# JuliaLinearAlgebra/IterativeSolvers.jl

Measured on AMD Instinct MI355X. Metric: cg_iters_per_sec, higher is better.
Workload: dtype f64; 1 GPU; cg! on 256^3 3D 7-point Laplacian (test/laplace_matrix.jl), fp64, hashed rhs, x0 = 0 (BASELINE.json configs[1]); n=16777216, nnz=117047296

## Files before the change

### include/mik_dev.h

```cpp
#include "mik.h"
#ifndef MIK_DEV_H
#define MIK_DEV_H
#ifdef __cplusplus
extern "C" {
#endif
enum {
    MIK_KNOB_LAYOUTS = 0,
    MIK_KNOB_CSR_KERNEL = 1,
    MIK_KNOB_SDIA_KERNEL = 2,
    MIK_KNOB_LONG_SEGMENT = 3,
    MIK_KNOB_UPLOAD = 4,
    MIK_KNOB_GS = 5,
    MIK_KNOB_TRANSPORT = 6,
    MIK_KNOB_NO_LOOKAHEAD = 7,
    MIK_KNOB_SOLVER_FORM = 8,
    MIK_KNOB_GS_TIMEOUT = 9,
    MIK_KNOB_CG_STEP = 10,
    MIK_KNOB_HOST_WAIT = 11,
    MIK_KNOB_MACHINE = 12,
    MIK_KNOB_COUNT = 13
};
int mik_set_tuning(int key, int value);
int mik_ctx_set_tuning(mik_ctx *ctx, int key, int value);
int mik_dev_gmres_form(const mik_gmres *it, int *single_launch, int *segments_per_workgroup, int *xcd_local_last, int *timeouts);
int mik_dev_dense_plan(const mik_dense *D, int adjoint, const void *x, const void *y, int *vec, int *streamed, int64_t *grid_x, int64_t *grid_y,
                       int64_t *chunks_or_batches, int64_t *segments);
int mik_dev_dense_block_plan(const mik_dense *D, int b, const void *X, int64_t ldx, const void *Y, int64_t ldy, int *vec, int *streamed,
                             int64_t *grid_x, int64_t *grid_y, int64_t *chunks, int *groups, int *last_width, int *vector_cols, int64_t *workspace_bytes);
int mik_dev_dense_block_min_width(mik_dense *D, int width);
int mik_dev_mgs_resident_shape(int *threads, int *register_rounds, int *lds_rounds);
int mik_dev_spmv_plan(const mik_csr *A, const void *x, int fuse_dot, int rb_begin, int rb_count, int skip_begin, int skip_end, char *kernel_name, int len,
                      int64_t *grid, int *launches, int *pre_longrows, int *post_rowdot);
int mik_dev_spmv_run(mik_ctx *ctx, const mik_csr *A, const void *x, void *y, int fuse_dot, void *seg_out, int rb_begin, int rb_count, int skip_begin,
                     int skip_end);
int mik_dev_exclusive_scan(mik_ctx *ctx, int *data, int64_t n);
int mik_dev_xwin_plan(int64_t n_blocks, const int *first_col, const int *last_col, const int *entries, int elem_size, int64_t n_cols,
                      int64_t total_entries, int *win_lo, int *span);
#ifdef __cplusplus
}
#endif
#endif
```

### iterativesolvers.jl_amd/_lib.py

```python
from __future__ import annotations

import ctypes as C
import os

import numpy as np

_HERE = os.path.dirname(os.path.abspath(__file__))
LIB_PATH = os.path.join(_HERE, "libmik.so")

MIK_OK = 0
MIK_F64, MIK_F32 = 0, 1
MIK_C64, MIK_C32 = 2, 3
MIK_SCALAR_REAL = 0x100
MIK_MGS, MIK_CGS, MIK_DGKS = 0, 1, 2
STATUS = {1: "invalid argument", 2: "HIP runtime error", 3: "dimension/dtype mismatch",
          4: "out of memory", 5: "not implemented", 6: "callback failed", 7: "norm outside the safely representable range",
          8: "singular"}


class MikError(RuntimeError):
    def __init__(self, code: int, where: str, detail: str = ""):
        self.code = code
        super().__init__(f"{where}: status {code} ({STATUS.get(code, '?')}) {detail}".rstrip())


_vp = C.c_void_p
_i64 = C.c_int64
_i64p = C.POINTER(C.c_int64)
_f64p = C.POINTER(C.c_double)
_ip = C.POINTER(C.c_int)

HALO_FN = C.CFUNCTYPE(C.c_int, C.c_void_p)
REDUCE_FN = C.CFUNCTYPE(C.c_int, C.c_void_p, C.c_int, C.c_int, C.c_void_p)


MUL_FN = C.CFUNCTYPE(C.c_int, C.c_void_p, C.c_void_p, C.c_void_p)
LDIV_FN = C.CFUNCTYPE(C.c_int, C.c_void_p, C.c_void_p, C.c_void_p)


class MikOperator(C.Structure):
    _fields_ = [("dtype", C.c_int), ("n", C.c_int64), ("csr", C.c_void_p), ("mul", MUL_FN), ("user", C.c_void_p)]


class MikPrecond(C.Structure):
    _fields_ = [("diag", C.c_void_p), ("ldiv", LDIV_FN), ("user", C.c_void_p)]


class MikDeviceInfo(C.Structure):
    _fields_ = [("device", C.c_int), ("compute_units", C.c_int), ("xcds", C.c_int), ("wavefront_size", C.c_int),
                ("lds_bytes_per_cu", C.c_int64), ("l2_bytes", C.c_int64), ("hbm_bytes", C.c_int64), ("arch", C.c_char * 64),
                ("planned_compute_units", C.c_int), ("planned_xcds", C.c_int), ("xcd_maps", C.c_int), ("resident_workgroup_cap", C.c_int),
                ("gs_single_launch_max_segments", C.c_int), ("gs_xcd_local_max_workgroups", C.c_int), ("sweep_grid_cap", C.c_int),
                ("mgs_resident_max_segments", C.c_int), ("reserved", C.c_int * 7)]


class MikPartition(C.Structure):
    _fields_ = [("rank", C.c_int), ("nranks", C.c_int), ("n_ext", C.c_int64), ("x_ext", C.c_void_p),
                ("send_idx", C.c_void_p), ("n_send", C.c_int64), ("send_buf", C.c_void_p),
                ("halo", HALO_FN), ("reduce", REDUCE_FN), ("user", C.c_void_p), ("link", C.c_void_p)]


class MikDensePlan(C.Structure):
    _fields_ = [("form", C.c_int), ("spin_limit", C.c_int)]


MIK_DENSE_AUTO, MIK_DENSE_PANEL, MIK_DENSE_CHAINED = 0, 1, 2


SIGNATURES = {
    "mik_abi_version": (C.c_int, []),
    "mik_device_count": (C.c_int, [_ip]),
    "mik_ctx_create": (C.c_int, [C.c_int, C.POINTER(_vp)]),
    "mik_ctx_destroy": (C.c_int, [_vp]),
    "mik_ctx_info": (C.c_int, [_vp, C.POINTER(MikDeviceInfo)]),
    "mik_dev_gmres_form": (C.c_int, [_vp, _ip, _ip, _ip, _ip]),
    "mik_dev_dense_plan": (C.c_int, [_vp, C.c_int, _vp, _vp, _ip, _ip, _i64p, _i64p, _i64p, _i64p]),
    "mik_dev_dense_block_plan": (C.c_int, [_vp, C.c_int, _vp, _i64, _vp, _i64, _ip, _ip, _i64p, _i64p, _i64p, _ip, _ip, _ip, _i64p]),
    "mik_dev_dense_block_min_width": (C.c_int, [_vp, C.c_int]),
    "mik_dev_mgs_resident_shape": (C.c_int, [_ip, _ip, _ip]),
    "mik_dev_spmv_plan": (C.c_int, [_vp, _vp, C.c_int, C.c_int, C.c_int, C.c_int, C.c_int, C.c_char_p, C.c_int, _i64p, _ip, _ip, _ip]),
    "mik_dev_spmv_run": (C.c_int, [_vp, _vp, _vp, _vp, C.c_int, _vp, C.c_int, C.c_int, C.c_int, C.c_int]),
    "mik_dev_exclusive_scan": (C.c_int, [_vp, _vp, _i64]),
    "mik_ctx_set_stream": (C.c_int, [_vp, _vp]),
    "mik_ctx_synchronize": (C.c_int, [_vp]),
    "mik_last_error": (C.c_char_p, [_vp]),
    "mik_reduce_shape": (C.c_int, [C.c_int, _ip, _ip]),
    "mik_spmv_dot_shape": (C.c_int, [_ip, _ip]),
    "mik_set_tuning": (C.c_int, [C.c_int, C.c_int]),
    "mik_ctx_set_tuning": (C.c_int, [_vp, C.c_int, C.c_int]),
    "mik_dev_xwin_plan": (C.c_int, [_i64, _ip, _ip, _ip, C.c_int, _i64, _i64, _ip, _ip]),
    "mik_spmv_long_row": (C.c_int, [_ip]),
    "mik_spmv_long_segment": (C.c_int, [_ip]),
    "mik_spmv_long_group": (C.c_int, [_ip]),
    "mik_malloc": (C.c_int, [_vp, C.c_size_t, C.POINTER(_vp)]),
    "mik_free": (C.c_int, [_vp, _vp]),
    "mik_memcpy_h2d": (C.c_int, [_vp, _vp, _vp, C.c_size_t]),
    "mik_memcpy_d2h": (C.c_int, [_vp, _vp, _vp, C.c_size_t]),
    "mik_copy": (C.c_int, [_vp, C.c_int, _i64, _vp, _vp]),
    "mik_fill": (C.c_int, [_vp, C.c_int, _i64, _vp, _vp]),
    "mik_csr_create": (C.c_int, [_vp, C.c_int, _i64, _i64, _i64, _i64p, _i64p, _vp, C.c_int, C.c_int,
                                 C.POINTER(_vp)]),
    "mik_csr_create_i32": (C.c_int, [_vp, C.c_int, _i64, _i64, _i64, C.POINTER(C.c_int32), C.POINTER(C.c_int32), _vp, C.c_int, C.c_int,
                                     C.POINTER(_vp)]),
    "mik_csr_destroy": (C.c_int, [_vp]),
    "mik_csr_layout": (C.c_int, [_vp, _ip]),
    "mik_csr_set_layout": (C.c_int, [_vp, C.c_int]),
    "mik_csr_stored_bytes": (C.c_int, [_vp, _i64p]),
    "mik_csr_compact": (C.c_int, [_vp]),
    "mik_spmv_kernel": (C.c_int, [_vp, C.c_char_p, C.c_int]),
    "mik_csr_info": (C.c_int, [_vp, _i64p, _i64p, _i64p, _ip]),
    "mik_spmv": (C.c_int, [_vp, _vp, _vp, _vp]),
    "mik_dot": (C.c_int, [_vp, C.c_int, _i64, _vp, _vp, _vp]),
    "mik_nrm2": (C.c_int, [_vp, C.c_int, _i64, _vp, _vp]),
    "mik_axpy": (C.c_int, [_vp, C.c_int, _i64, _vp, _vp, _vp]),
    "mik_xpby": (C.c_int, [_vp, C.c_int, _i64, _vp, _vp, _vp]),
    "mik_sub": (C.c_int, [_vp, C.c_int, _i64, _vp, _vp]),
    "mik_scal": (C.c_int, [_vp, C.c_int, _i64, _vp, _vp]),
    "mik_divide": (C.c_int, [_vp, C.c_int, _i64, _vp, _vp, _vp]),
    "mik_orthogonalize": (C.c_int, [_vp, C.c_int, _i64, C.c_int, _vp, _i64, _vp, _vp, _vp, C.c_int]),
    "mik_orthogonalize_vectors": (C.c_int, [_vp, C.c_int, _i64, C.c_int, C.POINTER(_vp), _vp, _vp, _vp]),
    "mik_gemv_n": (C.c_int, [_vp, C.c_int, _i64, C.c_int, _vp, _i64, _vp, _vp, _vp]),
    "mik_gemv_t": (C.c_int, [_vp, C.c_int, _i64, C.c_int, _vp, _i64, _vp, _vp]),
    "mik_lu_solve": (C.c_int, [C.c_int, _vp, _i64, C.c_int, _vp]),
    "mik_cg_create": (C.c_int, [_vp, _vp, _vp, _vp, _vp, _vp, _vp, _vp, C.c_double, C.c_double, _i64,
                                C.c_int, C.POINTER(_vp)]),
    "mik_cg_create_op": (C.c_int, [_vp, C.POINTER(MikOperator), C.POINTER(MikPrecond), _vp, _vp, _vp, _vp, _vp, C.c_double, C.c_double, _i64,
                                   C.c_int, C.POINTER(_vp)]),
    "mik_gmres_create_op": (C.c_int, [_vp, C.POINTER(MikOperator), C.POINTER(MikPrecond), C.POINTER(MikPrecond), _vp, _vp, C.c_double, C.c_double,
                                      C.c_int, _i64, C.c_int, C.c_int, C.POINTER(_vp)]),
    "mik_cg_destroy": (C.c_int, [_vp]),
    "mik_cg_fused_x": (C.c_int, [_vp, C.POINTER(C.c_int)]),
    "mik_cg_iterate": (C.c_int, [_vp, _i64, _f64p, _ip]),
    "mik_cg_iterate_many": (C.c_int, [_vp, _i64, _i64, _f64p, _i64p]),
    "mik_cg_state": (C.c_int, [_vp, _f64p, _f64p, _f64p, _i64p, _i64p, _ip]),
    "mik_gmres_create": (C.c_int, [_vp, _vp, _vp, _vp, _vp, _vp, C.c_double, C.c_double, C.c_int, _i64, C.c_int,
                                   C.c_int, C.POINTER(_vp)]),
    "mik_gmres_create_partitioned": (C.c_int, [_vp, _vp, _vp, _vp, _vp, _vp, C.c_double, C.c_double, C.c_int, _i64, C.c_int,
                                               C.c_int, C.POINTER(MikPartition), C.POINTER(_vp)]),
    "mik_gmres_destroy": (C.c_int, [_vp]),
    "mik_gmres_iterate": (C.c_int, [_vp, _i64, _f64p, _ip]),
    "mik_gmres_iterate_many": (C.c_int, [_vp, _i64, _i64, _f64p, _i64p]),
    "mik_gmres_state": (C.c_int, [_vp, _f64p, _f64p, _f64p, _ip, _i64p, _ip]),
    "mik_axpy_dot": (C.c_int, [_vp, C.c_int, _i64, _vp, _vp, _vp, _vp, _vp, C.c_int]),
    "mik_axpy2_nrm2": (C.c_int, [_vp, C.c_int, _i64, _vp, _vp, _vp, _vp, _vp, _vp, C.c_int]),
    "mik_cheb_direction": (C.c_int, [_vp, C.c_int, _i64, _vp, _vp, _vp, C.c_int, _vp]),
    "mik_minres_update": (C.c_int, [_vp, C.c_int, _i64, _vp, _vp, _vp, _vp, _vp, _vp, _vp, _vp, _vp, _vp, _vp, C.c_int]),
    "mik_gram": (C.c_int, [_vp, C.c_int, _i64, C.c_int, _vp, _i64, _vp]),
    "mik_bicgstab_mr_update": (C.c_int, [_vp, C.c_int, _i64, C.c_int, _vp, _i64, _vp, _i64, _vp, _vp, _vp]),
    "mik_bicgstab_create": (C.c_int, [_vp, _vp, C.c_int, _vp, _vp, _i64, _vp, _i64, _vp, _vp, C.POINTER(_vp)]),
    "mik_bicgstab_step": (C.c_int, [_vp, _vp]),
    "mik_bicgstab_destroy": (C.c_int, [_vp]),
    "mik_minres_create": (C.c_int, [_vp, _vp, _vp, _vp, _vp, _vp, _vp, _vp, _vp, C.c_double, C.c_int, C.POINTER(_vp)]),
    "mik_minres_step": (C.c_int, [_vp, _i64, _vp]),
    "mik_minres_proj_shape": (C.c_int, [_vp, _ip, _ip]),
    "mik_bicgstab_dot_shape": (C.c_int, [_vp, _ip, _ip]),
    "mik_minres_destroy": (C.c_int, [_vp]),
    "mik_xpby_nrm2": (C.c_int, [_vp, C.c_int, _i64, _vp, _vp, _vp, _vp]),
    "mik_lsqr_update": (C.c_int, [_vp, C.c_int, _i64, _vp, _vp, _vp, _vp, _vp, _vp, _vp]),
    "mik_lsmr_update": (C.c_int, [_vp, C.c_int, _i64, _vp, _vp, _vp, _vp, _vp, _vp, _vp, _vp]),
    "mik_axpy2_dot": (C.c_int, [_vp, C.c_int, _i64, _vp, _vp, _vp, _vp, _vp, _vp, _vp]),
    "mik_scal2": (C.c_int, [_vp, C.c_int, _i64, _vp, _vp, _vp, _vp]),
    "mik_qmr_update": (C.c_int, [_vp, C.c_int, _i64, _vp, _vp, _vp, _vp, _vp, _vp, _vp, _vp, _vp]),
    "mik_idrs_create": (C.c_int, [_vp, _vp, C.c_int, _vp, _vp, _vp, _i64, _vp, _i64, _vp, _i64, _vp, _vp, _vp, C.c_double, C.POINTER(_vp)]),
    "mik_idrs_step": (C.c_int, [_vp, C.c_int, _vp]),
    "mik_idrs_state": (C.c_int, [_vp, _vp, _vp, _vp]),
# ... 141 lines not shown
```

### iterativesolvers.jl_amd/csrc/mik_comm.hip

```cpp
#include <dlfcn.h>

#include <algorithm>
#include <new>

#include "mik_kernels.h"
#include "mik_iter.h"
#include "mik_mail.h"

namespace {
struct NcclId { char internal[128]; };
using nccl_comm_t = void *;
struct Rccl {
    void *h = nullptr;
    int (*GetUniqueId)(NcclId *) = nullptr;
    int (*CommInitRank)(nccl_comm_t *, int, NcclId, int) = nullptr;
    int (*CommDestroy)(nccl_comm_t) = nullptr;
    int (*Send)(const void *, size_t, int, int, nccl_comm_t, hipStream_t) = nullptr;
    int (*Recv)(void *, size_t, int, int, nccl_comm_t, hipStream_t) = nullptr;
    int (*AllGather)(const void *, void *, size_t, int, nccl_comm_t, hipStream_t) = nullptr;
    int (*GroupStart)() = nullptr;
    int (*GroupEnd)() = nullptr;
    const char *(*GetErrorString)(int) = nullptr;
    std::string err;
};
// ... 1108 lines not shown
        MIK_TRY(halo_begin(it, &pending));
    }
    if (pending && it->int_end > it->int_begin) {
        MIK_TRY(mik_cgd_phase(it, MIK_CGD_STEP_B_INTERIOR, iteration));
        MIK_TRY(halo_end(it, pending));
        return head_spmv_dot(it, true, iteration);
    }
    MIK_TRY(halo_end(it, pending));
    return head_spmv_dot(it, false, iteration);
}

static int cgd_enqueue_tail(mik_cgd *it, int64_t iteration)
{
    if (mail_fused(it)) {
        MIK_TRY(mik_cgd_phase(it, CGD_STEP_C_NOFIN, iteration));
        return it->base.dtype == MIK_F64 ? mail_fin_rr<double>(it, iteration) : mail_fin_rr<float>(it, iteration);
    }
    MIK_TRY(mik_cgd_phase(it, MIK_CGD_STEP_C, iteration));
    MIK_TRY(gather_scalar(it, it->rr_all, 1));
    return mik_cgd_phase(it, MIK_CGD_STEP_D, iteration);
}

struct CgdComm {
    mik_cgd *it;
    mik_cg &base() { return it->base; }
    int phase(int ph) { return mik_cgd_phase(it, ph, 0); }
    int halo_x()
    {
        bool pending = false;
        if (!it->initially_zero) MIK_TRY(halo_begin(it, &pending));
        return halo_end(it, pending);
    }
    int gather_rr_init() { return gather_scalar(it, it->rr_all, 2); }
    int head(int64_t iteration) { return cgd_enqueue_head(it, iteration); }
    int tail(int64_t iteration, int64_t) { return cgd_enqueue_tail(it, iteration); }
    int flush_x() { return phase(CGD_X_FLUSH); }
    int wait(CgMirror *m) { return cgd_wait_raw(it, m); }
    int clear_pending() { return it->base.fuse_x ? phase(CGD_CLEAR_PENDING) : MIK_OK; }
    int scaled_norm()
    {
        bool direct = false;
        MIK_TRY(phase(CGD_NORM_AMAX));
        MIK_TRY(gather_rr_init());
        MIK_TRY(cgd_norm_stage1_any(it, &direct));
        if (direct) return MIK_OK;
        MIK_TRY(gather_rr_init());
        return cgd_norm_stage2_any(it);
    }
    int close_frozen(int64_t it_next, int hist_index)
    {
        it->norm_fix_index = hist_index;
        it->norm_it_next = it_next;
        return phase(CGD_FIX_STEP);
    }
    int collect(const CgMirror &m, double *residual, double *tol, double *history, int64_t cap, int64_t *steps)
    {
        int done = 0;
        MIK_TRY(mailbox_check(it->comm, "row-partitioned cg"));
        return cgd_collect(it, m, residual, tol, &done, history, cap, steps);
    }
};

extern "C" int mik_cgd_init(mik_cgd *it, double *residual, double *tol)
{
    if (!it) return MIK_ERR_INVALID;
    MIK_TRY(cgd_require_transport(it, "mik_cgd_init"));
    CgdComm rk{it};
    MIK_TRY(cgd_init_ranks(rk, residual, tol));
    it->initialised = true;
    return MIK_OK;
}

extern "C" int mik_cgd_iterate_many(mik_cgd *it, int64_t iteration, int64_t max_steps, double *residuals, int64_t *steps_done)
{
    if (!it || !steps_done || iteration < 0) return MIK_ERR_INVALID;
    *steps_done = 0;
    MIK_TRY(cgd_require_transport(it, "mik_cgd_iterate_many"));
    if (!it->initialised) return mik_fail(it->base.ctx, MIK_ERR_INVALID, "mik_cgd_iterate_many: call mik_cgd_init first");
    mik_cg &bs = it->base;
    if (max_steps <= 0 || iteration >= bs.maxiter || bs.residual <= bs.tol) return MIK_OK;
    max_steps = std::min<int64_t>(std::min<int64_t>(max_steps, bs.maxiter - iteration), bs.hist_cap);
    const bool ahead_ok = bs.ctx->tuning[MIK_KNOB_NO_LOOKAHEAD] == 0 && iteration + max_steps < bs.maxiter;
    bs.fuse_x = (bs.ctx->tuning[MIK_KNOB_CG_STEP] & 1) == 0;
    CgdComm rk{it};
    return cg_run_batch(rk, iteration, max_steps, ahead_ok, residuals, steps_done);
}

namespace {
struct GroupEvents {
    std::vector<hipEvent_t> packed, halo, dot, rr;
    std::vector<hipStream_t> side;
};

struct GroupState {
    int P = 0;
    std::vector<mik_cgd *> its;
    GroupEvents ev;
    ~GroupState()
    {
        for (auto *v : {&ev.packed, &ev.halo, &ev.dot, &ev.rr})
            for (hipEvent_t e : *v) if (e) (void)hipEventDestroy(e);
        for (hipStream_t s : ev.side) if (s) (void)hipStreamDestroy(s);
    }
};

std::vector<GroupState *> g_groups;

GroupState *find_group(mik_cgd **its, int P)
{
    for (GroupState *g : g_groups)
        if (g->P == P && std::equal(g->its.begin(), g->its.end(), its)) return g;
    return nullptr;
}
}

static int group_check(mik_cgd **its, int P, const char *who)
{
    if (!its || P < 1) return MIK_ERR_INVALID;
    for (int p = 0; p < P; ++p) {
        if (!its[p]) return MIK_ERR_INVALID;
        if (its[p]->nranks != P || its[p]->rank != p) return mik_fail(its[p]->base.ctx, MIK_ERR_MISMATCH, "%s: handle %d is rank %d of %d", who, p, its[p]->rank, its[p]->nranks);
        if (its[p]->base.dtype != its[0]->base.dtype) return mik_fail(its[p]->base.ctx, MIK_ERR_MISMATCH, "%s: mixed dtypes", who);
    }
    return MIK_OK;
}

static inline hipError_t group_copy(void *dst, int dst_dev, const void *src, int src_dev, size_t bytes, hipStream_t s)
{
    return dst_dev == src_dev ? hipMemcpyAsync(dst, src, bytes, hipMemcpyDeviceToDevice, s) : hipMemcpyPeerAsync(dst, dst_dev, src, src_dev, bytes, s);
}

static int group_get(mik_cgd **its, int P, GroupState **out)
{
    GroupState *g = find_group(its, P);
    if (!g) {
        g = new (std::nothrow) GroupState();
        if (!g) return MIK_ERR_NOMEM;
        g->P = P;
        g->its.assign(its, its + P);
        for (auto *v : {&g->ev.packed, &g->ev.halo, &g->ev.dot, &g->ev.rr}) v->assign((size_t)P, nullptr);
        g->ev.side.assign((size_t)P, nullptr);
        for (int p = 0; p < P; ++p) {
            mik_ctx *ctx = its[p]->base.ctx;
            MIK_HIP(ctx, hipSetDevice(ctx->device));
            for (int q = 0; q < P; ++q)
                if (its[q]->base.ctx->device != ctx->device) {
                    (void)hipDeviceEnablePeerAccess(its[q]->base.ctx->device, 0);
                    (void)hipGetLastError();
                }
            for (auto *v : {&g->ev.packed, &g->ev.halo, &g->ev.dot, &g->ev.rr}) MIK_HIP(ctx, hipEventCreateWithFlags(&(*v)[p], hipEventDisableTiming));
            MIK_HIP(ctx, hipStreamCreateWithFlags(&g->ev.side[p], hipStreamNonBlocking));
        }
        g_groups.push_back(g);
    }
    *out = g;
    return MIK_OK;
}

void mik_cgd_group_forget(mik_cgd *it)
{
    for (size_t i = 0; i < g_groups.size();) {
        GroupState *g = g_groups[i];
        if (std::find(g->its.begin(), g->its.end(), it) != g->its.end()) {
            for (int p = 0; p < g->P; ++p) (void)hipStreamSynchronize(g->ev.side[p]);
            g_groups.erase(g_groups.begin() + (long)i);
            delete g;
// ... 131 lines not shown
    int wait(CgMirror *m)
    {
        ms.resize((size_t)g->P);
        for (int p = 0; p < g->P; ++p) {
            MIK_TRY(set_device(p));
            MIK_TRY(cgd_wait_raw(g->its[p], &ms[(size_t)p]));
            if (ms[(size_t)p].range != ms[0].range)
                return mik_fail(g->its[p]->base.ctx, MIK_ERR_MISMATCH, "row-partitioned cg: rank %d disagrees with rank 0 on the range of |r|^2", p);
        }
        *m = ms[0];
        return MIK_OK;
    }
    int clear_pending() { return MIK_OK; }
    int scaled_norm()
    {
        MIK_TRY(phase(CGD_NORM_AMAX));
        MIK_TRY(group_gather_scalar(g, 1));
        bool direct = false;
        for (int p = 0; p < g->P; ++p) {
            bool dp = false;
            MIK_TRY(set_device(p));
            MIK_TRY(cgd_norm_stage1_any(g->its[p], &dp));
            if (p == 0) direct = dp;
            else if (dp != direct) return mik_fail(g->its[p]->base.ctx, MIK_ERR_MISMATCH, "row-partitioned cg: rank %d disagrees with rank 0 on max |r|", p);
        }
        if (direct) return MIK_OK;
        MIK_TRY(group_gather_scalar(g, 1));
        for (int p = 0; p < g->P; ++p) {
            MIK_TRY(set_device(p));
            MIK_TRY(cgd_norm_stage2_any(g->its[p]));
        }
        return MIK_OK;
    }
    int close_frozen(int64_t it_next, int hist_index)
    {
        for (mik_cgd *it : g->its) { it->norm_fix_index = hist_index; it->norm_it_next = it_next; }
        return phase(CGD_FIX_STEP);
    }
    int collect(const CgMirror &, double *residual, double *tol, double *history, int64_t cap, int64_t *steps)
    {
        std::vector<double> h0((size_t)cap), hp((size_t)cap);
        for (int p = 0; p < g->P; ++p) {
            mik_cgd *it = g->its[p];
            double res = 0, tl = 0;
            int done = 0;
            int64_t st = 0;
            MIK_TRY(set_device(p));
            MIK_TRY(cgd_collect(it, ms[(size_t)p], &res, &tl, &done, p == 0 ? h0.data() : hp.data(), cap, &st));
            if (p == 0) { *steps = st; if (residual) *residual = res; if (tol) *tol = tl; }
            else if (st != *steps || !std::equal(h0.begin(), h0.begin() + st, hp.begin()) || res != base().residual || tl != base().tol)
                return mik_fail(it->base.ctx, MIK_ERR_MISMATCH, "row-partitioned cg (group): rank %d disagrees with rank 0 on the residuals", p);
        }
        if (history) std::copy(h0.begin(), h0.begin() + *steps, history);
        return MIK_OK;
    }
};

extern "C" int mik_cgd_group_init(mik_cgd **its, int P, double *residual, double *tol)
{
    MIK_TRY(group_check(its, P, "mik_cgd_group_init"));
    CgdGroup rk{};
    MIK_TRY(group_get(its, P, &rk.g));
    MIK_TRY(cgd_init_ranks(rk, residual, tol));
    for (int p = 0; p < P; ++p) its[p]->initialised = true;
    return MIK_OK;
}

extern "C" int mik_cgd_group_iterate_many(mik_cgd **its, int P, int64_t iteration, int64_t max_steps, double *residuals, int64_t *steps_done)
{
    MIK_TRY(group_check(its, P, "mik_cgd_group_iterate_many"));
    if (!steps_done || iteration < 0) return MIK_ERR_INVALID;
    *steps_done = 0;
    CgdGroup rk{};
    MIK_TRY(group_get(its, P, &rk.g));
    mik_cg &b0 = its[0]->base;
    for (int p = 0; p < P; ++p) if (!its[p]->initialised) return mik_fail(b0.ctx, MIK_ERR_INVALID, "mik_cgd_group_iterate_many: call mik_cgd_group_init first");
    if (max_steps <= 0 || iteration >= b0.maxiter || b0.residual <= b0.tol) return MIK_OK;
    max_steps = std::min<int64_t>(std::min<int64_t>(max_steps, b0.maxiter - iteration), b0.hist_cap);
    rk.split = rk.early = true;
    for (int p = 0; p < P; ++p) {
        rk.split = rk.split && its[p]->int_end > its[p]->int_begin;
        rk.early = rk.early && its[p]->n_early > 0;
        its[p]->base.fuse_x = (its[p]->base.ctx->tuning[MIK_KNOB_CG_STEP] & 1) == 0;
    }
    rk.early = rk.early && rk.split;
    return cg_run_batch(rk, iteration, max_steps, false, residuals, steps_done);
}
```

### iterativesolvers.jl_amd/csrc/mik_core.hip

```cpp
#include <algorithm>
#include <cmath>
#include <cstdarg>
#include <limits>
#include <new>

#include "mik_kernels.h"
#include "mik_spmv.h"
#include "mik_complex.h"
#include <algorithm>
#include <mutex>

#include "mik_sell.h"
#include "mik_jds.h"
#include <map>
#include <string>
#include <unordered_map>

thread_local std::string g_mik_create_error;
int g_mik_tuning[MIK_KNOB_COUNT] = {0};
static std::vector<mik_ctx *> g_mik_contexts;
static std::mutex g_mik_contexts_mu;

int mik_fail(mik_ctx *ctx, int code, const char *fmt, ...)
{
    char buf[512];
    va_list ap;
    va_start(ap, fmt);
    vsnprintf(buf, sizeof(buf), fmt, ap);
    va_end(ap);
    if (ctx) ctx->err = buf; else g_mik_create_error = buf;
    return code;
}

int mik_ensure_partials(mik_ctx *ctx, size_t bytes)
{
    if (bytes <= ctx->partials_bytes) return MIK_OK;
    size_t want = std::max(bytes, (size_t)1 << 20);
    if (ctx->partials) {
        MIK_HIP(ctx, hipStreamSynchronize(ctx->stream));
        MIK_HIP(ctx, hipFree(ctx->partials));
        ctx->partials = nullptr;
        ctx->partials_bytes = 0;
    }
    MIK_HIP(ctx, hipMalloc(&ctx->partials, want));
    ctx->partials_bytes = want;
    return MIK_OK;
}


extern "C" int mik_abi_version(void) { return MIK_ABI_VERSION; }

extern "C" int mik_device_count(int *count)
{
    if (!count) return MIK_ERR_INVALID;
    int c = 0;
    hipError_t e = hipGetDeviceCount(&c);
    if (e != hipSuccess) { *count = 0; return mik_fail(nullptr, MIK_ERR_HIP, "hipGetDeviceCount: %s", hipGetErrorString(e)); }
    *count = c;
    return MIK_OK;
}

extern "C" int mik_ctx_create(int device, mik_ctx **out)
{
    if (!out) return mik_fail(nullptr, MIK_ERR_INVALID, "mik_ctx_create: out is NULL");
    *out = nullptr;
    int count = 0;
    hipError_t e = hipGetDeviceCount(&count);
    if (e != hipSuccess || count == 0)
        return mik_fail(nullptr, MIK_ERR_HIP, "mik_ctx_create: no HIP device available (%s)", hipGetErrorString(e));
    if (device < 0 || device >= count)
        return mik_fail(nullptr, MIK_ERR_INVALID, "mik_ctx_create: device %d out of range [0, %d)", device, count);
    mik_ctx *ctx = new (std::nothrow) mik_ctx();
    if (!ctx) return mik_fail(nullptr, MIK_ERR_NOMEM, "mik_ctx_create: host allocation failed");
    ctx->device = device;
    auto bail = [&](hipError_t err, const char *what) {
        int rc = mik_fail(nullptr, MIK_ERR_HIP, "mik_ctx_create: %s: %s", what, hipGetErrorString(err));
        delete ctx;
        return rc;
    };
    if ((e = hipSetDevice(device)) != hipSuccess) return bail(e, "hipSetDevice");
    if ((e = hipStreamCreateWithFlags(&ctx->own_stream, hipStreamNonBlocking)) != hipSuccess) return bail(e, "hipStreamCreate");
    ctx->stream = ctx->own_stream;
    {
        int v = 0;
        if ((e = hipDeviceGetAttribute(&v, hipDeviceAttributeMultiprocessorCount, device)) != hipSuccess) return bail(e, "hipDeviceGetAttribute(MultiprocessorCount)");
        ctx->cu_count = v;
        v = 0;
        if (hipDeviceGetAttribute(&v, hipDeviceAttributeNumberOfXccs, device) != hipSuccess || v < 1) { (void)hipGetLastError(); v = 1; }
        ctx->xcd_count = v;
        v = 0;
        if (hipDeviceGetAttribute(&v, hipDeviceAttributeWarpSize, device) == hipSuccess) ctx->wave_size = v; else (void)hipGetLastError();
        v = 0;
        if (hipDeviceGetAttribute(&v, hipDeviceAttributeMaxSharedMemoryPerMultiprocessor, device) == hipSuccess) ctx->lds_per_cu = v; else (void)hipGetLastError();
        v = 0;
        if (hipDeviceGetAttribute(&v, hipDeviceAttributeL2CacheSize, device) == hipSuccess) ctx->l2_bytes = v; else (void)hipGetLastError();
        hipDeviceProp_t prop;
        if (hipGetDeviceProperties(&prop, device) == hipSuccess) {
            ctx->hbm_bytes = (int64_t)prop.totalGlobalMem;
            snprintf(ctx->arch, sizeof(ctx->arch), "%s", prop.gcnArchName);
        } else (void)hipGetLastError();
        if (ctx->wave_size != 0 && ctx->wave_size != 64) {
            int rc = mik_fail(nullptr, MIK_ERR_HIP, "mik_ctx_create: device %d runs %d-wide wavefronts; libmik's kernels are written for wave-64 (gfx950)", device, ctx->wave_size);
            delete ctx;
            return rc;
        }
    }
    if ((e = hipMalloc(&ctx->coef, mik_ctx::COEF_BYTES)) != hipSuccess) return bail(e, "hipMalloc");
    if ((e = hipHostMalloc(&ctx->coef_host, mik_ctx::COEF_BYTES, hipHostMallocDefault)) != hipSuccess) return bail(e, "hipHostMalloc");
    if ((e = hipEventCreateWithFlags(&ctx->wait_event, hipEventDisableTiming)) != hipSuccess) return bail(e, "hipEventCreate");
    if ((e = hipHostMalloc(&ctx->pub, mik_ctx::PUB_BYTES + 64, hipHostMallocMapped | hipHostMallocCoherent)) != hipSuccess) return bail(e, "hipHostMalloc");
    memset(ctx->pub, 0, mik_ctx::PUB_BYTES + 64);
    {
        std::lock_guard<std::mutex> lk(g_mik_contexts_mu);
        memcpy(ctx->tuning, g_mik_tuning, sizeof(ctx->tuning));
        g_mik_contexts.push_back(ctx);
    }
    *out = ctx;
    return MIK_OK;
}

extern "C" int mik_ctx_info(const mik_ctx *ctx, mik_device_info *out)
{
    if (!ctx || !out) return MIK_ERR_INVALID;
    memset(out, 0, sizeof(*out));
    out->device = ctx->device;
    out->compute_units = ctx->cu_count;
    out->xcds = ctx->xcd_count;
    out->wavefront_size = ctx->wave_size;
    out->lds_bytes_per_cu = ctx->lds_per_cu;
    out->l2_bytes = ctx->l2_bytes;
    out->hbm_bytes = ctx->hbm_bytes;
    snprintf(out->arch, sizeof(out->arch), "%s", ctx->arch);
    out->planned_compute_units = mik_cus(ctx);
    out->planned_xcds = mik_xcds(ctx);
    out->xcd_maps = mik_xcd_maps(ctx) ? 1 : 0;
    out->resident_workgroup_cap = mik_resident_cap(ctx);
    out->gs_single_launch_max_segments = 8 * mik_resident_cap(ctx);
    out->gs_xcd_local_max_workgroups = mik_xcd_maps(ctx) ? 4 * (mik_cus(ctx) / mik_xcds(ctx)) : 0;
    out->sweep_grid_cap = mik_max_grid(ctx);
    out->mgs_resident_max_segments = ctx->lds_per_cu >= 160 * 1024 ? mik_mgs_resident_max_s() * mik_resident_cap(ctx) : 0;
    return MIK_OK;
}

extern "C" int mik_ctx_destroy(mik_ctx *ctx)
{
    if (!ctx) return MIK_OK;
    {
        std::lock_guard<std::mutex> lk(g_mik_contexts_mu);
        g_mik_contexts.erase(std::remove(g_mik_contexts.begin(), g_mik_contexts.end(), ctx), g_mik_contexts.end());
    }
    (void)hipSetDevice(ctx->device);
    (void)hipStreamSynchronize(ctx->stream);
    {
        std::vector<std::pair<void *, int (*)(void *)>> owned;
        owned.swap(ctx->owned);
        for (auto &h : owned) (void)h.second(h.first);
    }
    if (ctx->partials) (void)hipFree(ctx->partials);
    if (ctx->coef) (void)hipFree(ctx->coef);
    if (ctx->coef_host) (void)hipHostFree(ctx->coef_host);
    if (ctx->pub) (void)hipHostFree(ctx->pub);
    if (ctx->wait_event) (void)hipEventDestroy(ctx->wait_event);
    if (ctx->own_stream) (void)hipStreamDestroy(ctx->own_stream);
    delete ctx;
    return MIK_OK;
}

extern "C" int mik_ctx_set_stream(mik_ctx *ctx, void *hip_stream)
{
    if (!ctx) return MIK_ERR_INVALID;
    MIK_HIP(ctx, hipStreamSynchronize(ctx->stream));
    ctx->stream = hip_stream ? (hipStream_t)hip_stream : ctx->own_stream;
    return MIK_OK;
}

extern "C" int mik_ctx_synchronize(mik_ctx *ctx)
{
    if (!ctx) return MIK_ERR_INVALID;
    MIK_HIP(ctx, mik_wait(ctx));
    return MIK_OK;
}

extern "C" const char *mik_last_error(mik_ctx *ctx) { return ctx ? ctx->err.c_str() : g_mik_create_error.c_str(); }
// ... 1025 lines not shown
    return A->sdia_buf_ok && A->sdia_cls >= 1 && (A->n_rows & 1) == 0 && A->ctx->tuning[MIK_KNOB_SDIA_KERNEL] == 0;
}

static inline bool spmv_pair_range(int rb0, int nb, int nb_all) { return (rb0 & 1) == 0 && ((nb & 1) == 0 || rb0 + nb == nb_all); }

extern "C" int mik_csr_layout(const mik_csr *A, int *layout)
{
    if (!A || !layout) return MIK_ERR_INVALID;
    *layout = spmv_kernel_choice(A);
    return MIK_OK;
}

extern "C" int mik_csr_set_layout(mik_csr *A, int layout)
{
    if (!A) return MIK_ERR_INVALID;
    if (layout != 0 && layout != -1) return mik_fail(A->ctx, MIK_ERR_NOTIMPL, "mik_csr_set_layout: only 0 (CSR arrays) and -1 (automatic) can be requested");
    if (layout == 0 && !A->col) return mik_fail(A->ctx, MIK_ERR_NOTIMPL, "mik_csr_set_layout: the CSR arrays were released (mik_csr_compact)");
    A->force_layout = layout;
    return MIK_OK;
}

extern "C" int mik_csr_stored_bytes(const mik_csr *A, int64_t *bytes)
{
    if (!A || !bytes) return MIK_ERR_INVALID;
    const int64_t es = (int64_t)mik_dtype_size(A->dtype);
    const int64_t nb = (A->n_rows + MIK_BLOCK - 1) / MIK_BLOCK;
    if (mik_is_complex(A->dtype)) { *bytes = mik_c_stored_bytes(A); return MIK_OK; }
    switch (spmv_kernel_choice(A)) {
    case LAYOUT_SDIAC: *bytes = A->n_rows + nb * (spmv_sdiab_usable(A) ? 64 : 4) + (int64_t)A->sdia_npat * (80 + 8 * es); break;
    case LAYOUT_SDIAW: *bytes = A->n_rows * 4 + nb * 4 + (nb + 1) / 2 * 64 + (int64_t)A->sdiaw_npat * A->sdiaw_pat_bytes; break;
    case LAYOUT_SDIA: *bytes = A->sdia_entries * es + A->n_rows + nb * 36; break;
    case LAYOUT_JDS: *bytes = A->jds_groups * (16 / es) * (es + 4) + A->n_rows * 2 + ((A->n_rows + 63) / 64 + 1) * 4 +
                              (A->n_long ? (A->nnz - A->jds_short_nnz) * (es + 4) + 12LL * A->n_long + 4LL * A->n_seg + 16LL * A->n_cut : 0); break;
    case LAYOUT_CSR: *bytes = A->nnz * (es + 4) + (A->n_rows + 1) * 4 + (A->n_long ? A->n_rows + 12LL * A->n_long + 4LL * A->n_seg + 16LL * A->n_cut : 0) +
                              ((A->xwin_lo && !spmv_csr_rowgather(A)) ? nb * 4 : 0) + ((A->rperm && !spmv_csr_rowgather(A)) ? A->n_rows : 0); break;
    }
    return MIK_OK;
}

extern "C" int mik_csr_info(const mik_csr *A, int64_t *n_rows, int64_t *n_cols, int64_t *nnz, int *dtype)
{
    if (!A) return MIK_ERR_INVALID;
    if (n_rows) *n_rows = A->n_rows;
    if (n_cols) *n_cols = A->n_cols;
    if (nnz) *nnz = A->nnz;
    if (dtype) *dtype = A->dtype;
    return MIK_OK;
}

extern "C" int mik_csr_compact(mik_csr *A)
{
    if (!A) return MIK_ERR_INVALID;
    if (!A->col) return MIK_OK;
    if (!(A->sdia_pats || A->sdia_val || A->sdiaw_pats || A->jds_val) || A->n_long)
        return mik_fail(A->ctx, MIK_ERR_NOTIMPL, "mik_csr_compact: this operator runs on its CSR arrays");
    if (A->ctx) { (void)hipSetDevice(A->ctx->device); (void)hipStreamSynchronize(A->ctx->stream); }
    (void)hipFree(A->rowptr); (void)hipFree(A->col); (void)hipFree(A->val);
    A->rowptr = nullptr; A->col = nullptr; A->val = nullptr;
    return MIK_OK;
}

enum SpmvKernel { SPMV_ROWGATHER, SPMV_ROWBLOCK, SPMV_JDS, SPMV_SDIA, SPMV_SDIAC, SPMV_SDIAB, SPMV_SDIAB2, SPMV_SDIAW, SPMV_SDIAW2 };

constexpr int SPMV_NO_SKIP = 0x7fffffff;

struct SpmvPlan {
    int rc = MIK_OK;
    const char *refusal = nullptr;
    bool empty = false;
    SpmvKernel kernel = SPMV_ROWGATHER;
    bool can_split = false;
    bool skips = false;
    bool epilogue = false;
    bool pre_longrows = false, post_rowdot = false;
    int grid = 0;
    size_t lds = 0, pre_lds = 0;
    bool fd = false;
    int nb_all = 0, nlb = 0;
    int rb0 = 0, nb = 0, map_mode = 0;
    int skip_at = SPMV_NO_SKIP, skip_len = 0;
    int pb0 = 0, np = 0, pmode = 0, ps = -1, pfull = 0;
    int sshift = -1, nfull = 0, cls = 0;
    bool merge = false, nt_rb = false, xwin = false, rp = false;
    bool long_win = false;
    int lw_launch = 0;
};

static SpmvPlan spmv_refusal(SpmvPlan p, int rc, const char *text) { p.rc = rc; p.refusal = text; return p; }
static inline bool spmv_ep_armed(const mik_ctx *ctx) { return ctx->spmv_ep_w || ctx->spmv_ep_c || ctx->spmv_ep_z; }

static SpmvPlan spmv_plan(const mik_csr *A, size_t es, bool x_aligned, bool fuse_dot, int rb_begin, int rb_count, int skip_at, int skip_len, bool ep_armed)
{
    SpmvPlan p;
    const int *knob = A->ctx->tuning;
    const int n = (int)A->n_rows, nb_all = (int)mik_spmv_nwg(n), nlong = A->n_long;
    const bool whole = rb_count < 0 || (rb_begin == 0 && rb_count == nb_all);
    const int rb0 = whole ? 0 : rb_begin, nb = whole ? nb_all : rb_count;
    switch (spmv_kernel_choice(A)) {
    case LAYOUT_SDIAC:
        p.kernel = !spmv_sdiab_usable(A) ? SPMV_SDIAC : (sdiab2_applies(A) && skip_len == 0 && spmv_pair_range(rb0, nb, nb_all)) ? SPMV_SDIAB2 : SPMV_SDIAB;
        break;
    case LAYOUT_SDIAW:
        p.kernel = ((n & 1) == 0 && (uint64_t)A->n_cols * es < 0x7FFFFFF0ull && knob[MIK_KNOB_SDIA_KERNEL] != 3 && spmv_pair_range(rb0, nb, nb_all)) ? SPMV_SDIAW2 : SPMV_SDIAW;
        break;
    case LAYOUT_SDIA: p.kernel = SPMV_SDIA; break;
    case LAYOUT_JDS: p.kernel = SPMV_JDS; break;
    case LAYOUT_CSR: p.kernel = spmv_csr_rowgather(A) ? SPMV_ROWGATHER : SPMV_ROWBLOCK; break;
    }
    const bool row_per_thread = p.kernel == SPMV_ROWGATHER || p.kernel == SPMV_ROWBLOCK || p.kernel == SPMV_JDS;
    p.can_split = p.kernel != SPMV_ROWBLOCK && !(row_per_thread && nlong);
    p.skips = p.kernel == SPMV_SDIAB || p.kernel == SPMV_SDIAB2;
    p.epilogue = whole && fuse_dot && knob[MIK_KNOB_SOLVER_FORM] != 2 && (p.kernel == SPMV_SDIAB2 || (row_per_thread && nlong == 0));
    if (n == 0) { p.empty = true; return p; }
    if (!whole && !p.can_split) return spmv_refusal(p, MIK_ERR_NOTIMPL, "SpMV over a row-block range is not available for this operator layout");
    if (!whole && (rb_begin < 0 || rb_begin + rb_count > nb_all)) return spmv_refusal(p, MIK_ERR_INVALID, "SpMV row-block range out of bounds");
    if (!whole && rb_count == 0) { p.empty = true; return p; }
    if (ep_armed && !p.epilogue)
        return spmv_refusal(p, MIK_ERR_NOTIMPL, "SpMV: the y = A x + c w / dot(z, y) epilogue is not available for this operator's kernel");

    p.map_mode = A->strip;
    if (!whole && p.map_mode >= 8 && (rb0 % p.map_mode != 0 || nb % p.map_mode != 0)) p.map_mode = 0;
    if (skip_len > 0) p.map_mode = 0;
    p.nb_all = nb_all; p.rb0 = rb0; p.nb = nb; p.skip_at = skip_at; p.skip_len = skip_len;
    p.pb0 = rb0 / 2; p.np = (nb + 1) / 2;
    p.fd = fuse_dot;
    p.grid = nb;
    p.nlb = (nlong + 3) / 4;
    p.long_win = A->long_win && spmv_windows_live(A) && x_aligned;
    p.pre_lds = p.long_win ? es * (size_t)A->long_lw : 0;
    switch (p.kernel) {
    case SPMV_SDIAB: case SPMV_SDIAB2:
        if (p.map_mode >= 8) {
            const int S = p.map_mode >> 3;
            if ((S & (S - 1)) == 0) { p.sshift = 0; while ((1 << p.sshift) < S) ++p.sshift; p.nfull = nb / p.map_mode * p.map_mode; }
        }
        p.cls = knob[MIK_KNOB_SDIA_KERNEL] == 2 ? 0 : A->sdia_cls;
        if (p.kernel == SPMV_SDIAB2) {
            p.grid = (p.np + 7) / 8 * 8;
            p.ps = p.sshift >= 1 ? p.sshift - 1 : -1;
            p.pfull = p.sshift >= 1 ? p.nfull / 2 : 0;
            break;
        }
        [[fallthrough]];
    case SPMV_SDIAC: p.grid = ((nb + MIK_SDIAC_G - 1) / MIK_SDIAC_G + 7) / 8 * 8; break;
    case SPMV_SDIAW2:
        p.grid = p.np;
        p.pmode = p.map_mode >= 16 ? (p.map_mode / 2 + 7) / 8 * 8 : 0;
        break;
    case SPMV_SDIAW: case SPMV_SDIA: break;
    case SPMV_JDS:
        p.fd = fuse_dot && nlong == 0;
        p.merge = nlong > 0;
        p.post_rowdot = fuse_dot && !p.fd;
        p.grid = nb + (p.merge ? p.nlb : 0);
        break;
    case SPMV_ROWGATHER:
        p.pre_longrows = nlong > 0;
        break;
    case SPMV_ROWBLOCK: {
        p.merge = nlong > 0 && !fuse_dot;
        p.pre_longrows = nlong > 0 && !p.merge;
        p.nt_rb = !A->xwin_lo;
        p.grid = nb + (p.merge ? p.nlb : 0);
        p.xwin = A->xwin_lo && spmv_windows_live(A) && x_aligned;
        const size_t rb_tile = (size_t)MIK_SPMV_TILE * (8 / es);
        p.lds = es * (rb_tile + 12 + (p.xwin ? (size_t)A->xwin_span : 0));
        const int lw = (int)std::min<size_t>((size_t)A->long_lw, p.lds / 1024 * (1024 / es));
        p.lw_launch = (p.merge && p.long_win && A->long_spread) ? -lw : lw;
        p.rp = A->rperm && spmv_windows_live(A);
        break;
    }
    }
    return p;
}

static const char *spmv_kernel_name(const SpmvPlan &p)
{
    switch (p.kernel) {
    case SPMV_ROWGATHER: return "k_spmv_rowgather";
    case SPMV_ROWBLOCK: return p.xwin ? "k_spmv_rowblock+xwin" : "k_spmv_rowblock";
    case SPMV_JDS: return "k_spmv_jds";
    case SPMV_SDIA: return "k_spmv_sdia";
    case SPMV_SDIAC: return "k_spmv_sdiac";
    case SPMV_SDIAB: return "k_spmv_sdiab";
    case SPMV_SDIAB2: return "k_spmv_sdiab2";
    case SPMV_SDIAW: return "k_spmv_sdiaw";
    case SPMV_SDIAW2: return "k_spmv_sdiaw2";
    }
    return "";
}

static SpmvPlan spmv_plan_whole(const mik_csr *A, bool fuse_dot)
{
    return spmv_plan(A, mik_dtype_size(A->dtype), true, fuse_dot, 0, -1, SPMV_NO_SKIP, 0, false);
}

bool mik_spmv_has_epilogue(const mik_csr *A) { return A && spmv_plan_whole(A, true).epilogue; }
bool mik_spmv_can_split(const mik_csr *A) { return spmv_plan_whole(A, false).can_split; }
bool mik_spmv_is_light(const mik_csr *A) { return A && (spmv_kernel_choice(A) == LAYOUT_SDIAC || spmv_kernel_choice(A) == LAYOUT_SDIAW); }

extern "C" int mik_spmv_kernel(const mik_csr *A, char *name, int len)
{
    if (!A || !name || len <= 0) return MIK_ERR_INVALID;
    if (mik_is_complex(A->dtype)) { snprintf(name, (size_t)len, "%s", mik_c_spmv_kernel_name(A)); return MIK_OK; }
    snprintf(name, (size_t)len, "%s", spmv_kernel_name(spmv_plan_whole(A, false)));
    return MIK_OK;
}

static int spmv_plan_outside(const mik_csr *A, size_t es, bool x_aligned, bool fuse_dot, int skip_begin, int skip_end, bool ep_armed, SpmvPlan out[2])
{
    const int nb_all = (int)mik_spmv_nwg(A->n_rows), rest = skip_begin + (nb_all - skip_end);
    if (skip_begin < 0 || skip_end < skip_begin || skip_end > nb_all) { out[0] = spmv_refusal(SpmvPlan{}, MIK_ERR_INVALID, "SpMV: bad interior range"); return 1; }
    out[0] = spmv_plan(A, es, x_aligned, fuse_dot, 0, rest, skip_begin, skip_end - skip_begin, ep_armed);
    if (out[0].skips && rest > 0) return 1;
    out[0] = spmv_plan(A, es, x_aligned, fuse_dot, 0, skip_begin, SPMV_NO_SKIP, 0, ep_armed);
    out[1] = spmv_plan(A, es, x_aligned, fuse_dot, skip_end, nb_all - skip_end, SPMV_NO_SKIP, 0, ep_armed);
    return 2;
}

extern "C" int mik_dev_spmv_plan(const mik_csr *A, const void *x, int fuse_dot, int rb_begin, int rb_count, int skip_begin, int skip_end, char *kernel_name,
                                 int len, int64_t *grid, int *launches, int *pre_longrows, int *post_rowdot)
{
    if (!A || (kernel_name && len <= 0)) return MIK_ERR_INVALID;
    MIK_REFUSE_COMPLEX(A->ctx, A, "mik_dev_spmv_plan");
    const bool armed = spmv_ep_armed(A->ctx);
    SpmvPlan p[2];
    int np = 1;
    if (skip_begin < 0) p[0] = spmv_plan(A, mik_dtype_size(A->dtype), mik_aligned16(x), fuse_dot != 0, rb_begin, rb_count, SPMV_NO_SKIP, 0, armed);
    else np = spmv_plan_outside(A, mik_dtype_size(A->dtype), mik_aligned16(x), fuse_dot != 0, skip_begin, skip_end, armed, p);
    int total = 0;
    const SpmvPlan *first = nullptr;
    for (int i = 0; i < np; ++i) {
        if (p[i].rc != MIK_OK) return mik_fail(A->ctx, p[i].rc, "%s", p[i].refusal);
        if (p[i].empty) continue;
        total += (int)p[i].pre_longrows + 1 + (int)p[i].post_rowdot;
        if (!first) first = &p[i];
    }
    if (kernel_name) snprintf(kernel_name, (size_t)len, "%s", spmv_kernel_name(first ? *first : p[0]));
    if (grid) *grid = first ? first->grid : 0;
    if (launches) *launches = total;
    if (pre_longrows) *pre_longrows = first && first->pre_longrows;
    if (post_rowdot) *post_rowdot = first && first->post_rowdot;
    return MIK_OK;
}

struct SdiaCls { int c; };
template <typename F> static inline void with_consts(F &&f) { f(); }
template <typename F, typename... R> static inline void with_consts(F &&f, bool b, R... rest);
template <typename F, typename... R> static inline void with_consts(F &&f, SdiaCls s, R... rest);
template <typename C, typename F, typename... R> static inline void with_const(F &f, R... rest)
{
    with_consts([&](auto... c) { f(C{}, c...); }, rest...);
}
template <typename F, typename... R> static inline void with_consts(F &&f, bool b, R... rest)
{
    if (b) with_const<std::true_type>(f, rest...);
    else with_const<std::false_type>(f, rest...);
}
template <typename F, typename... R> static inline void with_consts(F &&f, SdiaCls s, R... rest)
{
    switch (s.c) {
    case 1: with_const<std::integral_constant<int, 1>>(f, rest...); break;
    case 2: with_const<std::integral_constant<int, 2>>(f, rest...); break;
    case 3: with_const<std::integral_constant<int, 3>>(f, rest...); break;
    default: with_const<std::integral_constant<int, 0>>(f, rest...); break;
    }
}

template <typename T> struct SpmvIO {
    mik_ctx *ctx;
    const mik_csr *A;
    const T *x;
    T *y, *seg_out;
    const int *done;
    const T *ep_w() const { return (const T *)ctx->spmv_ep_w; }
    const T *ep_c() const { return (const T *)ctx->spmv_ep_c; }
    const T *ep_z() const { return (const T *)ctx->spmv_ep_z; }
};

static LongTab spmv_long_tab(const mik_csr *A)
{
    LongTab lt{};
    if (const int nlong = A->n_long) {
        int *tb = A->long_rows;
        lt.rows = tb; lt.starts = tb + nlong; lt.lens = tb + 2 * nlong;
        lt.seg_row = tb + 3 * nlong;
        lt.cut_row = lt.seg_row + A->n_seg; lt.cut_first = lt.cut_row + A->n_cut; lt.cut_nseg = lt.cut_first + A->n_cut;
        lt.tickets = (unsigned *)(tb + 3 * nlong + A->n_seg + 3 * A->n_cut);
        lt.seg_sum = A->seg_sum; lt.nlong = nlong;
    }
    return lt;
}

template <typename T> static void spmv_go_sdiab(const SpmvPlan &p, const SpmvIO<T> &io)
{
    const mik_csr *A = io.A;
    with_consts([&](auto fd, auto cls) {
        constexpr int C = decltype(cls)::value;
        hipLaunchKernelGGL((k_spmv_sdiab<T, decltype(fd)::value, true, MIK_SDIAC_G, mik_sdiab_cls_ns(C), mik_sdiab_cls_cq(C)>), dim3(p.grid), dim3(MIK_BLOCK), 0,
                           io.ctx->stream, (int)A->n_rows, (int)A->n_cols, A->sdia_koff, p.rb0, p.nb, p.nfull, p.sshift, p.skip_at, p.skip_len,
                           (const SdiaSliceRec *)A->sdia_recs, (const SdiaPattern<T> *)A->sdia_pats, A->sdia_mask, io.x, io.y, io.seg_out, io.done);
    }, p.fd, SdiaCls{p.cls});
}

template <typename T> static void spmv_go_sdiab2(const SpmvPlan &p, const SpmvIO<T> &io)
{
    const mik_csr *A = io.A;
    with_consts([&](auto fd, auto cls) {
        constexpr int C = decltype(cls)::value;
        if constexpr (C >= 1)
            hipLaunchKernelGGL((k_spmv_sdiab2<T, decltype(fd)::value, true, mik_sdiab_cls_ns(C), mik_sdiab_cls_cq(C)>), dim3(p.grid), dim3(MIK_BLOCK), 0,
                               io.ctx->stream, (int)A->n_rows, (int)A->n_cols, A->sdia_koff, p.pb0, p.np, p.pfull, p.ps, p.nb_all,
                               (const SdiaSliceRec *)A->sdia_recs, (const SdiaPattern<T> *)A->sdia_pats, A->sdia_mask, io.x, io.y, io.seg_out, io.done,
                               io.ep_w(), io.ep_c(), io.ep_z());
    }, p.fd, SdiaCls{p.cls});
}

template <typename T> static void spmv_go_sdiac(const SpmvPlan &p, const SpmvIO<T> &io)
{
    const mik_csr *A = io.A;
    with_consts([&](auto fd) {
        hipLaunchKernelGGL((k_spmv_sdiac<T, decltype(fd)::value, true, MIK_SDIAC_G>), dim3(p.grid), dim3(MIK_BLOCK), 0, io.ctx->stream, (int)A->n_rows,
                           (int)A->n_cols, p.rb0, p.nb, p.map_mode, A->sdia_pat_id, (const SdiaPattern<T> *)A->sdia_pats, A->sdia_mask, io.x, io.y,
                           io.seg_out, io.done);
    }, p.fd);
}

template <typename T> static void spmv_go_sdiaw(const SpmvPlan &p, const SpmvIO<T> &io)
{
    const mik_csr *A = io.A;
    with_consts([&](auto fd) {
        if (p.kernel == SPMV_SDIAW2)
            hipLaunchKernelGGL((k_spmv_sdiaw2<T, decltype(fd)::value, true>), dim3(p.grid), dim3(MIK_BLOCK), 0, io.ctx->stream, (int)A->n_rows, (int)A->n_cols,
                               A->sdiaw_koff, p.pb0, p.np, p.pmode, p.nb_all, A->sdiaw_pat_id, (const SdiawPattern<T> *)A->sdiaw_pats, A->sdiaw_mask,
                               (const uint4 *)A->sdiaw_uz, io.x, io.y, io.seg_out, io.done);
        else
            hipLaunchKernelGGL((k_spmv_sdiaw<T, decltype(fd)::value, true>), dim3(p.grid), dim3(MIK_BLOCK), 0, io.ctx->stream, (int)A->n_rows, A->sdiaw_koff,
                               p.rb0, p.nb, p.map_mode, A->sdiaw_pat_id, (const SdiawPattern<T> *)A->sdiaw_pats, A->sdiaw_mask, io.x, io.y, io.seg_out,
                               io.done);
    }, p.fd);
}

template <typename T> static void spmv_go_sdia(const SpmvPlan &p, const SpmvIO<T> &io)
{
    const mik_csr *A = io.A;
    with_consts([&](auto fd) {
        hipLaunchKernelGGL((k_spmv_sdia<T, decltype(fd)::value, true>), dim3(p.grid), dim3(MIK_BLOCK), 0, io.ctx->stream, (int)A->n_rows, (int)A->n_cols, p.rb0,
                           p.nb, p.map_mode, A->sdia_ptr, A->sdia_off, A->sdia_tri, A->sdia_mask, (const T *)A->sdia_val, io.x, io.y, io.seg_out, io.done);
    }, p.fd);
}

template <typename T> static void spmv_go_jds(const SpmvPlan &p, const SpmvIO<T> &io)
{
    const mik_csr *A = io.A;
    using IV = typename WideVec<T>::idx;
    using VV = typename WideVec<T>::val;
    with_consts([&](auto fd, auto mg) {
        if constexpr (!(decltype(fd)::value && decltype(mg)::value))
            hipLaunchKernelGGL((k_spmv_jds<T, decltype(fd)::value, true, decltype(mg)::value>), dim3(p.grid), dim3(MIK_BLOCK), 0, io.ctx->stream, (int)A->n_rows,
                               p.rb0, A->jds_ptr, A->jds_len, (const IV *)A->jds_col, (const VV *)A->jds_val, io.x, io.y, io.seg_out, io.done, p.nlb,
                               spmv_long_tab(A), A->col, (const T *)A->val, io.ep_w(), io.ep_c(), io.ep_z());
    }, p.fd, p.merge);
}

template <typename T> static void spmv_go_rowgather(const SpmvPlan &p, const SpmvIO<T> &io)
{
    const mik_csr *A = io.A;
    with_consts([&](auto fd) {
        hipLaunchKernelGGL((k_spmv_rowgather<T, decltype(fd)::value, true>), dim3(p.grid), dim3(MIK_BLOCK), 0, io.ctx->stream, (int)A->n_rows, p.rb0, p.nb,
                           p.map_mode, A->rowptr, A->col, (const T *)A->val, io.x, io.y, io.seg_out, io.done, A->is_long, io.ep_w(), io.ep_c(), io.ep_z());
    }, p.fd);
}

template <typename T> static void spmv_go_rowblock(const SpmvPlan &p, const SpmvIO<T> &io)
{
    const mik_csr *A = io.A;
    with_consts([&](auto fd, auto mg, auto nt, auto xw, auto rp) {
        if constexpr (!(decltype(fd)::value && decltype(mg)::value))
            hipLaunchKernelGGL((k_spmv_rowblock<T, decltype(fd)::value, decltype(nt)::value, true, decltype(mg)::value, decltype(xw)::value, decltype(rp)::value>),
                               dim3(p.grid), dim3(MIK_BLOCK), p.lds, io.ctx->stream, (int)A->n_rows, p.nb, p.map_mode, A->rowptr, A->col, (const T *)A->val,
                               io.x, io.y, io.seg_out, io.done, A->is_long, p.nlb, spmv_long_tab(A), (const int *)A->xwin_lo, A->xwin_span,
                               (const unsigned char *)A->rperm, (p.merge && p.long_win) ? (const int *)A->long_win : (const int *)nullptr, p.lw_launch,
                               io.ep_w(), io.ep_c(), io.ep_z());
    }, p.fd, p.merge, p.nt_rb, p.xwin, p.rp);
}

template <typename T> static int spmv_run(const SpmvPlan &p, const SpmvIO<T> &io)
{
    mik_ctx *ctx = io.ctx;
    const mik_csr *A = io.A;
    if (p.rc != MIK_OK) return mik_fail(ctx, p.rc, "%s", p.refusal);
    if (p.empty) return MIK_OK;
    if (p.pre_longrows) {
        hipLaunchKernelGGL((k_spmv_longrows<T>), dim3(p.nlb), dim3(MIK_BLOCK), p.pre_lds, ctx->stream, spmv_long_tab(A), A->col, (const T *)A->val, io.x, io.y,
                           io.done, p.long_win ? (const int *)A->long_win : (const int *)nullptr, A->long_lw);
        MIK_LAUNCH_CHECK(ctx);
    }
    switch (p.kernel) {
    case SPMV_ROWGATHER: spmv_go_rowgather<T>(p, io); break;
    case SPMV_ROWBLOCK: spmv_go_rowblock<T>(p, io); break;
    case SPMV_JDS: spmv_go_jds<T>(p, io); break;
    case SPMV_SDIA: spmv_go_sdia<T>(p, io); break;
    case SPMV_SDIAC: spmv_go_sdiac<T>(p, io); break;
    case SPMV_SDIAB: spmv_go_sdiab<T>(p, io); break;
    case SPMV_SDIAB2: spmv_go_sdiab2<T>(p, io); break;
    case SPMV_SDIAW: case SPMV_SDIAW2: spmv_go_sdiaw<T>(p, io); break;
    }
    MIK_LAUNCH_CHECK(ctx);
    if (p.post_rowdot) {
        hipLaunchKernelGGL((k_rowdot<T>), dim3(p.nb_all), dim3(MIK_BLOCK), 0, ctx->stream, (int)A->n_rows, io.x, (const T *)io.y, io.seg_out, io.done);
        MIK_LAUNCH_CHECK(ctx);
    }
    return MIK_OK;
}

template <typename T>
int mik_spmv_launch_range(mik_ctx *ctx, const mik_csr *A, const T *x, T *y, bool fuse_dot, T *seg_out, const int *done, int rb_begin,
                          int rb_count)
{
    return spmv_run<T>(spmv_plan(A, sizeof(T), mik_aligned16(x), fuse_dot, rb_begin, rb_count, SPMV_NO_SKIP, 0, spmv_ep_armed(ctx)), {ctx, A, x, y, seg_out, done});
}

template <typename T>
int mik_spmv_launch(mik_ctx *ctx, const mik_csr *A, const T *x, T *y, bool fuse_dot, T *seg_out, const int *done)
{
    return mik_spmv_launch_range<T>(ctx, A, x, y, fuse_dot, seg_out, done, 0, -1);
}

template <typename T>
int mik_spmv_launch_outside(mik_ctx *ctx, const mik_csr *A, const T *x, T *y, bool fuse_dot, T *seg_out, const int *done, int skip_begin, int skip_end)
{
    SpmvPlan p[2];
    const int np = spmv_plan_outside(A, sizeof(T), mik_aligned16(x), fuse_dot, skip_begin, skip_end, spmv_ep_armed(ctx), p);
    for (int i = 0; i < np; ++i) MIK_TRY(spmv_run<T>(p[i], {ctx, A, x, y, seg_out, done}));
    return MIK_OK;
}
template int mik_spmv_launch_outside<double>(mik_ctx *, const mik_csr *, const double *, double *, bool, double *, const int *, int, int);
template int mik_spmv_launch_outside<float>(mik_ctx *, const mik_csr *, const float *, float *, bool, float *, const int *, int, int);
template int mik_spmv_launch<double>(mik_ctx *, const mik_csr *, const double *, double *, bool, double *, const int *);
template int mik_spmv_launch<float>(mik_ctx *, const mik_csr *, const float *, float *, bool, float *, const int *);
template int mik_spmv_launch_range<double>(mik_ctx *, const mik_csr *, const double *, double *, bool, double *, const int *, int, int);
template int mik_spmv_launch_range<float>(mik_ctx *, const mik_csr *, const float *, float *, bool, float *, const int *, int, int);

template <typename T>
static int dev_spmv_run(mik_ctx *ctx, const mik_csr *A, const void *x, void *y, bool fuse_dot, void *seg_out, int rb_begin, int rb_count, int skip_begin,
                        int skip_end)
{
    if (skip_begin < 0) return mik_spmv_launch_range<T>(ctx, A, (const T *)x, (T *)y, fuse_dot, (T *)seg_out, nullptr, rb_begin, rb_count);
    return mik_spmv_launch_outside<T>(ctx, A, (const T *)x, (T *)y, fuse_dot, (T *)seg_out, nullptr, skip_begin, skip_end);
}

extern "C" int mik_dev_spmv_run(mik_ctx *ctx, const mik_csr *A, const void *x, void *y, int fuse_dot, void *seg_out, int rb_begin, int rb_count,
                                int skip_begin, int skip_end)
{
    if (!ctx || !A || !x || !y || (fuse_dot && !seg_out)) return MIK_ERR_INVALID;
    if (x == y) return mik_fail(ctx, MIK_ERR_INVALID, "mik_dev_spmv_run: x and y must not alias");
    MIK_REFUSE_COMPLEX(ctx, A, "mik_dev_spmv_run");
    return A->dtype == MIK_F64 ? dev_spmv_run<double>(ctx, A, x, y, fuse_dot != 0, seg_out, rb_begin, rb_count, skip_begin, skip_end)
                               : dev_spmv_run<float>(ctx, A, x, y, fuse_dot != 0, seg_out, rb_begin, rb_count, skip_begin, skip_end);
}

extern "C" int mik_spmv(mik_ctx *ctx, const mik_csr *A, const void *x, void *y)
{
    if (!ctx || !A || !x || !y) return MIK_ERR_INVALID;
    if (x == y) return mik_fail(ctx, MIK_ERR_INVALID, "mik_spmv: x and y must not alias");
    if (mik_is_complex(A->dtype)) return mik_c_spmv(ctx, A, x, y);
    return A->dtype == MIK_F64 ? mik_spmv_launch<double>(ctx, A, (const double *)x, (double *)y, false, nullptr, nullptr)
                               : mik_spmv_launch<float>(ctx, A, (const float *)x, (float *)y, false, nullptr, nullptr);
}

template <typename F> static int time_spmv_impl(mik_ctx *ctx, int reps, double *avg_ms, F &&launch)
{
    hipEvent_t e0, e1;
    MIK_HIP(ctx, hipEventCreate(&e0));
    MIK_HIP(ctx, hipEventCreate(&e1));
    MIK_HIP(ctx, hipEventRecord(e0, ctx->stream));
    for (int i = 0; i < reps; ++i) MIK_TRY(launch());
    MIK_HIP(ctx, hipEventRecord(e1, ctx->stream));
    MIK_HIP(ctx, hipEventSynchronize(e1));
    float ms = 0.f;
    MIK_HIP(ctx, hipEventElapsedTime(&ms, e0, e1));
    (void)hipEventDestroy(e0);
    (void)hipEventDestroy(e1);
    *avg_ms = (double)ms / reps;
    return MIK_OK;
}

extern "C" int mik_time_spmv(mik_ctx *ctx, const mik_csr *A, const void *x, void *y, int fused_dot, int reps, double *avg_ms)
{
    if (!ctx || !A || !x || !y || reps <= 0 || !avg_ms) return MIK_ERR_INVALID;
    if (mik_is_complex(A->dtype)) return time_spmv_impl(ctx, reps, avg_ms, [&] { return mik_c_spmv(ctx, A, x, y); });
    auto real = [&](auto t) {
        using T = decltype(t);
        MIK_TRY(mik_ensure_partials(ctx, sizeof(T) * (size_t)std::max<int64_t>((A->n_rows + MIK_BLOCK - 1) / MIK_BLOCK, 1)));
        return time_spmv_impl(ctx, reps, avg_ms, [&] { return mik_spmv_launch<T>(ctx, A, (const T *)x, (T *)y, fused_dot != 0, (T *)ctx->partials, nullptr); });
    };
    return A->dtype == MIK_F64 ? real(double{}) : real(float{});
}

template <typename T> static int reduce_to_host(mik_ctx *ctx, int64_t n, T *out)
{
    const int64_t nseg = mik_nseg<T>(n);
    hipLaunchKernelGGL((k_finalize_store<T>), dim3(1), dim3(MIK_FIN_THREADS), 0, ctx->stream, (const T *)ctx->partials, nseg,
                       (int64_t)0, (T *)ctx->coef, (const int *)nullptr);
    MIK_LAUNCH_CHECK(ctx);
    return mik_read_scalars<T>(ctx, (const T *)ctx->coef, 1, out);
}

template <typename T> int mik_safe_norm_slow(mik_ctx *ctx, int64_t n, const T *x, T *out)
{
    if (n <= 0) { *out = T(0); return MIK_OK; }
    T *scr = (T *)((unsigned char *)ctx->coef + mik_ctx::COEF_SAFE_SLOT);
    const int grid = (int)std::min<int64_t>((n + MIK_BLOCK - 1) / MIK_BLOCK, 1024);
    MIK_TRY(mik_ensure_partials(ctx, sizeof(T) * (size_t)std::max<int64_t>(std::max<int64_t>(mik_nseg<T>(n), grid), 1)));
    hipLaunchKernelGGL((k_amax<T>), dim3(grid), dim3(MIK_BLOCK), 0, ctx->stream, n, x, (T *)ctx->partials);
    MIK_LAUNCH_CHECK(ctx);
    hipLaunchKernelGGL((k_amax<T>), dim3(1), dim3(MIK_BLOCK), 0, ctx->stream, (int64_t)grid, (const T *)ctx->partials, scr);
    MIK_LAUNCH_CHECK(ctx);
    T amax;
    MIK_TRY(mik_read_scalars<T>(ctx, scr, 1, &amax));
    T sc, sinv;
    if (!mik_nrm_scale(amax, sc, sinv)) { *out = amax; return MIK_OK; }
    OpScaledSq<T> op{x, sc};
    MIK_TRY((launch_map<T>(ctx, n, op, mik_aligned16(x), (T *)ctx->partials, nullptr)));
    hipLaunchKernelGGL((k_finalize_store<T>), dim3(1), dim3(MIK_FIN_THREADS), 0, ctx->stream, (const T *)ctx->partials, mik_nseg<T>(n),
// ... 314 lines not shown
```

### iterativesolvers.jl_amd/csrc/mik_internal.h

```cpp
#pragma once
#include <hip/hip_runtime.h>

#include <algorithm>
#include <cmath>
#include <cstdint>
#include <cstdio>
#include <cstring>
#include <limits>
#include <string>
#include <vector>

#include "../../include/mik.h"
#include "../../include/mik_dev.h"

constexpr int MIK_BLOCK = 256;
constexpr int MIK_RED_L = 2;
constexpr int MIK_FIN_THREADS = 1024;
constexpr int MIK_SPMV_TILE = 2048;
constexpr int MIK_SPMV_G = 1;
constexpr int MIK_LONG_ROW = 256;
constexpr int MIK_XCD_MAP = 8;

template <typename T> struct VT;
template <> struct VT<double> { static constexpr int W = 2; using vec = double2; };
template <> struct VT<float>  { static constexpr int W = 4; using vec = float4;  };

struct mik_ctx {
    int device = 0;
    int cu_count = 0, xcd_count = 0, wave_size = 0;
    int64_t lds_per_cu = 0, l2_bytes = 0, hbm_bytes = 0;
    char arch[64] = {0};
    hipStream_t own_stream = nullptr;
    hipStream_t stream = nullptr;
    std::string err;
    void *partials = nullptr;
    size_t partials_bytes = 0;
    void *coef = nullptr;
    void *coef_host = nullptr;
    hipEvent_t wait_event = nullptr;
    void *pub = nullptr;
    unsigned long long pub_seq = 0;
    static constexpr size_t PUB_BYTES = 4096;
    const void *spmv_ep_w = nullptr, *spmv_ep_c = nullptr;
    const void *spmv_ep_z = nullptr;
    int tuning[MIK_KNOB_COUNT] = {0};
    static constexpr size_t COEF_BYTES = 8192;
    static constexpr size_t COEF_SAFE_SLOT = 4096;
    std::vector<std::pair<void *, int (*)(void *)>> owned;
};

static inline void mik_ctx_disown(mik_ctx *ctx, void *h)
{
    for (size_t i = 0; i < ctx->owned.size(); ++i)
        if (ctx->owned[i].first == h) { ctx->owned.erase(ctx->owned.begin() + (long)i); return; }
}

static inline int mik_cus(const mik_ctx *ctx) { const int v = ctx->tuning[MIK_KNOB_MACHINE] & 0xFFFF; return v > 0 ? v : std::max(1, ctx->cu_count); }
static inline int mik_xcds(const mik_ctx *ctx) { const int v = (ctx->tuning[MIK_KNOB_MACHINE] >> 16) & 0xFF; return v > 0 ? v : std::max(1, ctx->xcd_count); }
static inline bool mik_xcd_maps(const mik_ctx *ctx) { return mik_xcds(ctx) == MIK_XCD_MAP; }
static inline int mik_max_grid(const mik_ctx *ctx) { return mik_cus(ctx) * 32; }
static inline int mik_resident_cap(const mik_ctx *ctx) { return mik_cus(ctx); }
static inline int mik_strip_for(const mik_ctx *ctx, int64_t bw, int64_t nb)
{
    if (!mik_xcd_maps(ctx)) return 0;
    const int64_t P = ((bw + MIK_BLOCK - 1) / MIK_BLOCK + MIK_XCD_MAP - 1) / MIK_XCD_MAP * MIK_XCD_MAP;
    return (P >= MIK_XCD_MAP && P <= nb / 4) ? (int)P : 0;
}

int mik_mgs_resident_max_s();

struct mik_csr {
    mik_ctx *ctx = nullptr;
    int dtype = MIK_F64;
    int64_t n_rows = 0, n_cols = 0, nnz = 0;
    int *rowptr = nullptr;
    int *col = nullptr;
    void *val = nullptr;
    int max_row_nnz = 0;
    int strip = 0;
    int force_layout = -1;
    int max_rowblock_nnz = 0;
    int n_long = 0;
    int *xwin_lo = nullptr;
    int xwin_span = 0;
    int *long_win = nullptr;
    int long_lw = 0;
    bool long_spread = false;
    unsigned char *rperm = nullptr;
    int *long_rows = nullptr;
    int n_seg = 0, n_cut = 0;
    void *seg_sum = nullptr;
    unsigned char *is_long = nullptr;
    void *sdiaw_pats = nullptr;
    int *sdiaw_pat_id = nullptr;
    unsigned *sdiaw_mask = nullptr;
    void *sdiaw_uz = nullptr;
    int sdiaw_npat = 0, sdiaw_koff = 0, sdiaw_pat_bytes = 0;
    int *jds_ptr = nullptr;
    unsigned short *jds_len = nullptr;
    int *jds_col = nullptr;
    void *jds_val = nullptr;
    int64_t jds_groups = 0;
    int64_t jds_short_nnz = 0;
    int *sdia_ptr = nullptr;
    int *sdia_off = nullptr;
    int *sdia_tri = nullptr;
    unsigned char *sdia_mask = nullptr;
    void *sdia_val = nullptr;
    int64_t sdia_entries = 0;
    void *sdia_pats = nullptr;
    int *sdia_pat_id = nullptr;
    int sdia_npat = 0;
    bool sdia_buf_ok = false;
    int sdia_koff = 0;
    void *sdia_recs = nullptr;
    int sdia_cls = 0;
    int c_nlong = 0, c_nvirt = 0;
};

template <typename T> struct NrmRange;
template <> struct NrmRange<double> { static constexpr double LO = 0x1p-900, HI = 0x1p+900; static constexpr int EC = 1022; };
template <> struct NrmRange<float>  { static constexpr float LO = 0x1p-70f, HI = 0x1p+100f; static constexpr int EC = 126; };
template <typename T> __host__ __device__ static inline bool mik_nrm_in_range(T t) { return t >= NrmRange<T>::LO && t <= NrmRange<T>::HI; }

template <typename T> static inline bool mik_nrm_scale(T amax, T &s, T &sinv)
{
    if (amax == T(0) || amax != amax || amax > std::numeric_limits<T>::max()) return false;
    int e;
    (void)std::frexp((double)amax, &e);
    e = std::max(-NrmRange<T>::EC, std::min(NrmRange<T>::EC, e));
    s = (T)std::ldexp(1.0, -e);
    sinv = (T)std::ldexp(1.0, e);
    return true;
}

template <typename T> int mik_safe_norm_slow(mik_ctx *ctx, int64_t n, const T *x, T *out);
template <typename T> static inline int mik_norm_from_sumsq(mik_ctx *ctx, int64_t n, const T *x, T t, T *out)
{
    if (mik_nrm_in_range(t)) { *out = (T)std::sqrt(t); return MIK_OK; }
    return mik_safe_norm_slow<T>(ctx, n, x, out);
}

extern thread_local std::string g_mik_create_error;
extern int g_mik_tuning[MIK_KNOB_COUNT];

int mik_fail(mik_ctx *ctx, int code, const char *fmt, ...);
size_t mik_sdia_pattern_bytes(size_t es);
int mik_sdiac_finish(mik_ctx *ctx, mik_csr *A, const std::vector<unsigned char> &desc, int64_t nb, size_t es, int64_t slots);
int mik_upload_device(mik_ctx *ctx, mik_csr *A, int dtype, int64_t n_rows, int64_t n_cols, int64_t nnz, const int64_t *ptr, const int64_t *idx,
                      const void *val, int index_base, int is_csc);

int mik_ensure_partials(mik_ctx *ctx, size_t bytes);
int mik_build_sdiaw_device(mik_ctx *ctx, mik_csr *A);
int mik_build_jds_device(mik_ctx *ctx, mik_csr *A);
template <typename T>
int mik_spmv_launch(mik_ctx *ctx, const mik_csr *A, const T *x, T *y, bool fuse_dot, T *seg_out, const int *done);
template <typename T>
int mik_spmv_launch_range(mik_ctx *ctx, const mik_csr *A, const T *x, T *y, bool fuse_dot, T *seg_out, const int *done, int rb_begin,
                          int rb_count);
template <typename T>
int mik_spmv_launch_outside(mik_ctx *ctx, const mik_csr *A, const T *x, T *y, bool fuse_dot, T *seg_out, const int *done, int skip_begin, int skip_end);
bool mik_spmv_can_split(const mik_csr *A);
bool mik_spmv_is_light(const mik_csr *A);
bool mik_spmv_has_epilogue(const mik_csr *A);
static inline bool mik_xwin_plan(int64_t nb, const int *mn, const int *mx, const int *cnt, size_t es, int64_t n_cols, int64_t total_entries,
                                 std::vector<int> &lo, int *span_out)
{
    const int W = (int)(16 / es), XP = (int)(1024 / es);
    const int64_t cap = 32768 / (int64_t)es - W;
    lo.assign((size_t)nb, 0);
    int64_t need = 0, inside = 0;
    for (int64_t b = 0; b < nb; ++b) {
        if (cnt[b] <= 0) continue;
        lo[(size_t)b] = mn[b] & ~(W - 1);
        const int64_t nd = (int64_t)mx[b] + 1 - lo[(size_t)b];
        if (nd > cap) { lo[(size_t)b] = -1; continue; }
        need = std::max(need, nd);
        inside += cnt[b];
    }
    if (need <= 0 || 4 * inside < 3 * total_entries) return false;
    const int64_t span = (need + W + XP - 1) / XP * XP;
    if (span + W > n_cols) return false;
    for (int64_t b = 0; b < nb; ++b) {
        if (cnt[b] <= 0 || lo[(size_t)b] < 0 || (int64_t)lo[(size_t)b] + span <= n_cols) continue;
        const int64_t slid = (n_cols - span) & ~(int64_t)(W - 1);
        lo[(size_t)b] = slid + span > (int64_t)mx[b] ? (int)slid : -1;
    }
    *span_out = (int)span;
    return true;
}
int mik_build_xwin_device(mik_ctx *ctx, mik_csr *A);
int mik_build_rperm_host(mik_ctx *ctx, mik_csr *A, const int *rowptr_host);

#define MIK_HIP(ctx, call)                                                                    \
    do {                                                                                      \
        hipError_t e_ = (call);                                                               \
        if (e_ != hipSuccess)                                                                 \
            return mik_fail((ctx), e_ == hipErrorOutOfMemory ? MIK_ERR_NOMEM : MIK_ERR_HIP,    \
                            "%s failed: %s (%s:%d)", #call, hipGetErrorString(e_), __FILE__,   \
                            __LINE__);                                                        \
    } while (0)

#define MIK_LAUNCH_CHECK(ctx)                                                                 \
    do {                                                                                      \
        hipError_t e_ = hipGetLastError();                                                    \
        if (e_ != hipSuccess)                                                                 \
            return mik_fail((ctx), MIK_ERR_HIP, "kernel launch failed: %s (%s:%d)",           \
                            hipGetErrorString(e_), __FILE__, __LINE__);                       \
    } while (0)

static inline bool mik_is_complex(int dtype) { return dtype == MIK_C64 || dtype == MIK_C32; }
static inline int mik_real_dtype(int dtype) { return dtype == MIK_C64 ? MIK_F64 : MIK_F32; }
#define MIK_REFUSE_COMPLEX(ctx, A, who)                                                                                          \
    do {                                                                                                                         \
        if ((A) && mik_is_complex((A)->dtype))                                                                                   \
            return mik_fail((ctx), MIK_ERR_NOTIMPL, "%s: complex operators run through mik_spmv and the L1 / L2 entries only", (who)); \
    } while (0)

static inline bool mik_aligned16(const void *p) { return (reinterpret_cast<uintptr_t>(p) & 15u) == 0; }
static inline size_t mik_dtype_size(int dtype) { return dtype == MIK_C64 ? 16 : (dtype == MIK_F64 || dtype == MIK_C32) ? 8 : 4; }

static inline int64_t mik_spmv_nwg(int64_t n)
{
    const int64_t rows = (int64_t)MIK_BLOCK * MIK_SPMV_G;
    return (n + rows - 1) / rows;
}

template <typename T> static inline int64_t mik_nseg(int64_t n)
{
    const int64_t seg = (int64_t)MIK_BLOCK * VT<T>::W * MIK_RED_L;
    return (n + seg - 1) / seg;
}

template <typename T> static inline int mik_basis_nt(int64_t n, int k) { return (double)n * (double)k * sizeof(T) > 192.0e6 ? 1 : 0; }

static inline size_t mik_block_bytes(size_t es, int64_t n, int cols, int64_t ld)
{
    return (n > 0 && cols > 0) ? es * ((size_t)(cols - 1) * (size_t)ld + (size_t)n) : 0;
}
static inline bool mik_overlap(const void *a, size_t abytes, const void *b, size_t bbytes)
{
    const uintptr_t a0 = (uintptr_t)a, b0 = (uintptr_t)b;
    return abytes && bbytes && a0 < b0 + bbytes && b0 < a0 + abytes;
}
// ... 226 lines not shown
```

### iterativesolvers.jl_amd/csrc/mik_iter.h

```cpp
#pragma once
#include "mik_internal.h"

template <typename T> struct CgDev {
    T res, prev_res, alpha, beta, dot_uc, rr, tol, rho;
    T beta_rho;
    int done, nhist;
    int x_pending, pad_;
};

struct CgMirror {
    double res, prev_res, tol;
    int done, nhist;
    int tol_valid;
    int range;
    unsigned long long seq;
};

struct mik_cg {
    mik_ctx *ctx = nullptr;
    const mik_csr *A = nullptr;
    int dtype = MIK_F64;
    int64_t n = 0;
    void *x = nullptr, *u = nullptr, *r = nullptr, *c = nullptr;
    const void *b = nullptr, *diag = nullptr;
    mik_mul_fn op_mul = nullptr;
    void *op_user = nullptr;
    mik_ldiv_fn pl_fn = nullptr;
    void *pl_user = nullptr;
    void *dev = nullptr;
    void *fin = nullptr;
    void *hist = nullptr;
    int64_t hist_cap = 0;
    void *seg_spmv = nullptr;
    void *seg_vec = nullptr;
    void *seg_vec2 = nullptr;
    bool pcg_fused = false;
    double residual = 0, prev_residual = 1, tol = 0;
    int64_t maxiter = 0, mv_products = 0;
    CgMirror *mirror = nullptr;
    unsigned long long seq = 0;
    bool dev_done = false;
    bool head_ahead = false;
    bool fuse_x = false;
    int profile = 0;
    std::vector<hipEvent_t> ev;
    std::vector<int> ev_kind;
    size_t ev_used = 0;
    double kern_ms[3] = {0, 0, 0};
    int64_t kern_launches[3] = {0, 0, 0};
};

#ifdef __HIPCC__
constexpr int MIK_FIN_WGS = MIK_FIN_THREADS / 64;
template <typename T> struct FinScratch { T ws[MIK_FIN_WGS]; unsigned ticket; };

template <typename T> __device__ __forceinline__ bool level2_sum_spread(const T *__restrict__ S, int64_t m, FinScratch<T> *fs, T &tot)
{
    const int w = blockIdx.x, lane = threadIdx.x;
    T acc = T(0);
    int64_t j = 64 * (int64_t)w + lane;
    for (; j + 63 * (int64_t)MIK_FIN_THREADS < m; j += 64 * (int64_t)MIK_FIN_THREADS) {
        T v[64];
#pragma unroll
        for (int q = 0; q < 64; ++q) v[q] = S[j + q * (int64_t)MIK_FIN_THREADS];
#pragma unroll
        for (int q = 0; q < 64; ++q) acc = acc + v[q];
    }
    for (; j + 15 * (int64_t)MIK_FIN_THREADS < m; j += 16 * (int64_t)MIK_FIN_THREADS) {
        T v[16];
#pragma unroll
        for (int q = 0; q < 16; ++q) v[q] = S[j + q * (int64_t)MIK_FIN_THREADS];
#pragma unroll
        for (int q = 0; q < 16; ++q) acc = acc + v[q];
    }
    for (; j + 7 * (int64_t)MIK_FIN_THREADS < m; j += 8 * (int64_t)MIK_FIN_THREADS) {
        T v[8];
#pragma unroll
        for (int q = 0; q < 8; ++q) v[q] = S[j + q * (int64_t)MIK_FIN_THREADS];
#pragma unroll
        for (int q = 0; q < 8; ++q) acc = acc + v[q];
    }
    for (; j < m; j += MIK_FIN_THREADS) acc = acc + S[j];
    acc = wave_tree(acc);
    bool last = false;
    if (lane == 0) {
        __hip_atomic_store(&fs->ws[w], acc, __ATOMIC_RELAXED, __HIP_MEMORY_SCOPE_AGENT);
        asm volatile("s_waitcnt vmcnt(0)" ::: "memory");
        const unsigned tk = __hip_atomic_fetch_add(&fs->ticket, 1u, __ATOMIC_RELAXED, __HIP_MEMORY_SCOPE_AGENT);
        if (tk == (unsigned)gridDim.x - 1u) {
            T t = __hip_atomic_load(&fs->ws[0], __ATOMIC_RELAXED, __HIP_MEMORY_SCOPE_AGENT);
#pragma unroll
            for (int q = 1; q < MIK_FIN_WGS; ++q) t = t + __hip_atomic_load(&fs->ws[q], __ATOMIC_RELAXED, __HIP_MEMORY_SCOPE_AGENT);
            __hip_atomic_store(&fs->ticket, 0u, __ATOMIC_RELAXED, __HIP_MEMORY_SCOPE_AGENT);
            tot = t;
            last = true;
        }
    }
    return last;
}

template <typename T, typename Fin>
__global__ __launch_bounds__(MIK_FIN_THREADS) void k_fin(const T *__restrict__ S, int64_t m, Fin fin)
{
    __shared__ T lds16[16];
    const T tot = level2_sum(S, m, lds16);
    if (threadIdx.x == 0) fin(tot);
}
template <typename T, typename Fin>
__global__ __launch_bounds__(64) void k_fin_spread(const T *__restrict__ S, int64_t m, Fin fin, FinScratch<T> *fs)
{
    T tot;
    if (level2_sum_spread(S, m, fs, tot)) fin(tot);
}
template <typename T, typename Fin> static inline int launch_fin(mik_ctx *ctx, const T *S, int64_t m, Fin fin)
{
    hipLaunchKernelGGL((k_fin<T, Fin>), dim3(1), dim3(MIK_FIN_THREADS), 0, ctx->stream, S, m, fin);
    MIK_LAUNCH_CHECK(ctx);
    return MIK_OK;
}
template <typename T, typename Fin> static inline int launch_fin(mik_ctx *ctx, const T *S, int64_t m, Fin fin, FinScratch<T> *fs)
{
    if (m <= 16384) return launch_fin<T>(ctx, S, m, fin);
    hipLaunchKernelGGL((k_fin_spread<T, Fin>), dim3(MIK_FIN_WGS), dim3(64), 0, ctx->stream, S, m, fin, fs);
    MIK_LAUNCH_CHECK(ctx);
    return MIK_OK;
}

template <typename T>
__device__ __forceinline__ void cgd_close_step(CgDev<T> *d, T tot, T *__restrict__ hist, long long it_next, long long maxiter, CgMirror *mirror,
                                               unsigned long long seq, int hist_index, int fuse_x)
{
    if (fuse_x) d->x_pending = 1;
    if (!mik_nrm_in_range(tot)) {
// ... 103 lines not shown
```

### iterativesolvers.jl_amd/csrc/mik_kernels.h

```cpp
#pragma once
#include <algorithm>
#include <type_traits>

#include "mik_internal.h"

#ifdef __HIPCC__


template <typename T, bool VEC, typename Op, typename... Acc>
__device__ __forceinline__ void map_segment(const Op &op, int64_t s, int64_t n, Acc &...acc)
{
    constexpr int W = VT<T>::W;
    constexpr int L = MIK_RED_L;
    constexpr int64_t SEG = (int64_t)MIK_BLOCK * W * L;
    const int64_t base = s * SEG + (int64_t)W * threadIdx.x;
#pragma unroll
    for (int l = 0; l < L; ++l) {
        const int64_t i = base + (int64_t)l * MIK_BLOCK * W;
        if (VEC && i + W <= n) {
            op.apply_vec(i, acc...);
        } else {
#pragma unroll
            for (int e = 0; e < W; ++e)
                if (i + e < n) op.apply(i + e, acc...);
// ... 106 lines not shown

template <typename T, typename Op>
static inline int launch_map(mik_ctx *ctx, int64_t n, Op op, bool vec, T *seg_out, const int *done)
{
    return launch_segments<T>(ctx, n, vec, 0, [&](auto v, int grid, int64_t nseg) {
        hipLaunchKernelGGL((k_map<T, decltype(v)::value, Op>), dim3(grid), dim3(MIK_BLOCK), 0, ctx->stream, n, nseg, op, seg_out, done);
    });
}

template <typename T, bool VEC, typename Op>
__global__ __launch_bounds__(MIK_BLOCK) void k_map2(int64_t n, int64_t nseg, Op op, T *__restrict__ seg1, T *__restrict__ seg2,
                                                     const int *__restrict__ done)
{
    if (done && *done) return;
    __shared__ T lds4[4];
    for (int64_t s = blockIdx.x; s < nseg; s += gridDim.x) {
        T a1 = T(0), a2 = T(0);
        map_segment<T, VEC>(op, s, n, a1, a2);
        const T t1 = block_tree_256(a1, lds4);
        const T t2 = block_tree_256(a2, lds4);
        if (threadIdx.x == 0) { seg1[s] = t1; seg2[s] = t2; }
    }
}

template <typename T, typename Op>
static inline int launch_map2(mik_ctx *ctx, int64_t n, Op op, bool vec, T *seg1, T *seg2, const int *done)
{
    return launch_segments<T>(ctx, n, vec, 0, [&](auto v, int grid, int64_t nseg) {
        hipLaunchKernelGGL((k_map2<T, decltype(v)::value, Op>), dim3(grid), dim3(MIK_BLOCK), 0, ctx->stream, n, nseg, op, seg1, seg2, done);
    });
}

template <typename T, bool VEC, typename Op, typename Pro>
__global__ __launch_bounds__(MIK_BLOCK) void k_map_with(int64_t n, int64_t nseg, Op op, Pro pro, const T *__restrict__ part, int m, T *__restrict__ seg_out)
{
    __shared__ T lds16[16];
    __shared__ T lds4[4];
    const T tot = block_level2_256(part, m, lds16);
    pro(tot, op, blockIdx.x == 0 && threadIdx.x == 0);
    map_sweep<T, VEC>(op, n, nseg, seg_out, lds4);
}

template <typename T, typename Op, typename Pro>
static inline int launch_map_with(mik_ctx *ctx, int64_t n, Op op, Pro pro, bool vec, const T *part, int m, T *seg_out)
{
    return launch_segments<T>(ctx, n, vec, 0, [&](auto v, int grid, int64_t nseg) {
        hipLaunchKernelGGL((k_map_with<T, decltype(v)::value, Op, Pro>), dim3(grid), dim3(MIK_BLOCK), 0, ctx->stream, n, nseg, op, pro, part, m, seg_out);
    });
}

template <typename T> __device__ __forceinline__ typename VT<T>::vec vload(const T *p)
{
    return *reinterpret_cast<const typename VT<T>::vec *>(p);
}
template <typename T> __device__ __forceinline__ void vstore(T *p, typename VT<T>::vec v)
{
    *reinterpret_cast<typename VT<T>::vec *>(p) = v;
}
template <typename T> __device__ __forceinline__ T &el(typename VT<T>::vec &v, int e)
{
    return reinterpret_cast<T *>(&v)[e];
}
template <typename T> struct NativeVec;
template <> struct NativeVec<double> { typedef double type __attribute__((ext_vector_type(2))); };
template <> struct NativeVec<float> { typedef float type __attribute__((ext_vector_type(4))); };
template <typename T> __device__ __forceinline__ typename VT<T>::vec vload_nt(const T *p)
{
    using NV = typename NativeVec<T>::type;
    NV v = __builtin_nontemporal_load(reinterpret_cast<const NV *>(p));
    typename VT<T>::vec out;
#pragma unroll
    for (int e = 0; e < VT<T>::W; ++e) reinterpret_cast<T *>(&out)[e] = v[e];
    return out;
}
template <typename T> __device__ __forceinline__ void vstore_nt(T *p, typename VT<T>::vec v)
{
    using NV = typename NativeVec<T>::type;
    NV o;
#pragma unroll
    for (int e = 0; e < VT<T>::W; ++e) o[e] = reinterpret_cast<const T *>(&v)[e];
    __builtin_nontemporal_store(o, reinterpret_cast<NV *>(p));
}

template <typename T> constexpr int SEG_REGS = MIK_RED_L * VT<T>::W;

template <typename T, bool VEC>
__device__ __forceinline__ void seg_load(const T *__restrict__ col, int64_t base, int64_t n, int nt, T (&r)[SEG_REGS<T>])
{
    constexpr int W = VT<T>::W;
#pragma unroll
    for (int l = 0; l < MIK_RED_L; ++l) {
        const int64_t i = base + (int64_t)l * MIK_BLOCK * W;
        if (VEC && i + W <= n) {
            auto cv = nt ? vload_nt(col + i) : vload(col + i);
#pragma unroll
            for (int e = 0; e < W; ++e) r[l * W + e] = el<T>(cv, e);
        } else {
#pragma unroll
            for (int e = 0; e < W; ++e) r[l * W + e] = (i + e < n) ? col[i + e] : T(0);
        }
    }
}

template <typename T, bool VEC>
__device__ __forceinline__ void seg_store(T *__restrict__ col, int64_t base, int64_t n, const T (&r)[SEG_REGS<T>])
{
    constexpr int W = VT<T>::W;
#pragma unroll
    for (int l = 0; l < MIK_RED_L; ++l) {
        const int64_t i = base + (int64_t)l * MIK_BLOCK * W;
        if (VEC && i + W <= n) {
            typename VT<T>::vec cv;
#pragma unroll
            for (int e = 0; e < W; ++e) el<T>(cv, e) = r[l * W + e];
            vstore(col + i, cv);
        } else {
#pragma unroll
            for (int e = 0; e < W; ++e)
                if (i + e < n) col[i + e] = r[l * W + e];
        }
    }
}

template <typename T, bool VEC>
__device__ __forceinline__ T seg_dot(const T (&a)[SEG_REGS<T>], const T (&b)[SEG_REGS<T>], int64_t base, int64_t n)
{
    constexpr int W = VT<T>::W;
    T acc = T(0);
#pragma unroll
    for (int l = 0; l < MIK_RED_L; ++l) {
        const int64_t i = base + (int64_t)l * MIK_BLOCK * W;
        if (VEC && i + W <= n) {
#pragma unroll
            for (int e = 0; e < W; ++e) { T p = a[l * W + e] * b[l * W + e]; acc = acc + p; }
        } else {
#pragma unroll
            for (int e = 0; e < W; ++e)
                if (i + e < n) { T p = a[l * W + e] * b[l * W + e]; acc = acc + p; }
        }
    }
    return acc;
}

template <typename T, bool VEC>
__device__ __forceinline__ T seg_dot_col(const T *__restrict__ col, int64_t base, int64_t n, int nt, const T (&w)[SEG_REGS<T>])
{
    constexpr int W = VT<T>::W;
    T acc = T(0);
#pragma unroll
    for (int l = 0; l < MIK_RED_L; ++l) {
        const int64_t i = base + (int64_t)l * MIK_BLOCK * W;
        if (VEC && i + W <= n) {
            auto cv = nt ? vload_nt(col + i) : vload(col + i);
#pragma unroll
            for (int e = 0; e < W; ++e) { T p = el<T>(cv, e) * w[l * W + e]; acc = acc + p; }
        } else {
#pragma unroll
            for (int e = 0; e < W; ++e)
                if (i + e < n) { T p = col[i + e] * w[l * W + e]; acc = acc + p; }
        }
    }
    return acc;
}
template <typename T, bool VEC>
__device__ __forceinline__ void seg_axpy_col(T temp, const T *__restrict__ col, int64_t base, int64_t n, int nt, T (&y)[SEG_REGS<T>])
{
    constexpr int W = VT<T>::W;
#pragma unroll
    for (int l = 0; l < MIK_RED_L; ++l) {
        const int64_t i = base + (int64_t)l * MIK_BLOCK * W;
        if (VEC && i + W <= n) {
            auto cv = nt ? vload_nt(col + i) : vload(col + i);
#pragma unroll
            for (int e = 0; e < W; ++e) { T p = temp * el<T>(cv, e); y[l * W + e] = y[l * W + e] + p; }
        } else {
#pragma unroll
            for (int e = 0; e < W; ++e)
                if (i + e < n) { T p = temp * col[i + e]; y[l * W + e] = y[l * W + e] + p; }
        }
    }
}

template <typename T> __device__ __forceinline__ void pair_put(T acc, T (&slot)[4])
{
    acc = wave_tree(acc);
    if ((threadIdx.x & 63) == 0) slot[threadIdx.x >> 6] = acc;
}
template <typename T> __device__ __forceinline__ T pair_total(const T (&slot)[4])
{
    T tot = slot[0];
    tot = tot + slot[1]; tot = tot + slot[2]; tot = tot + slot[3];
    return tot;
}


template <typename T> struct OpXpby {
    static constexpr bool REDUCE = false;
    const T *__restrict__ x; T *__restrict__ y; Coef<T> beta; int nt = 0;
    __device__ __forceinline__ void apply(int64_t i, T &) const { T t = beta.get() * y[i]; y[i] = x[i] + t; }
    __device__ __forceinline__ void apply_vec(int64_t i, T &) const
    {
        const T b = beta.get();
        auto xv = (nt & 1) ? vload_nt(x + i) : vload(x + i);
        auto yv = (nt & 2) ? vload_nt<T>(y + i) : vload<T>(y + i);
#pragma unroll
        for (int e = 0; e < VT<T>::W; ++e) { T t = b * el<T>(yv, e); el<T>(yv, e) = el<T>(xv, e) + t; }
        if (nt & 4) vstore_nt(y + i, yv); else vstore(y + i, yv);
    }
};

template <typename T> struct OpXpbyNrm {
    static constexpr bool REDUCE = true;
    const T *__restrict__ x; T *__restrict__ y; T beta;
    __device__ __forceinline__ void apply(int64_t i, T &acc) const { T t = beta * y[i]; const T v = x[i] + t; y[i] = v; T p = v * v; acc = acc + p; }
    __device__ __forceinline__ void apply_vec(int64_t i, T &acc) const
    {
        auto xv = vload_nt(x + i); auto yv = vload<T>(y + i);
#pragma unroll
        for (int e = 0; e < VT<T>::W; ++e) { T t = beta * el<T>(yv, e); el<T>(yv, e) = el<T>(xv, e) + t; }
        vstore(y + i, yv);
#pragma unroll
        for (int e = 0; e < VT<T>::W; ++e) { T p = el<T>(yv, e) * el<T>(yv, e); acc = acc + p; }
    }
};

template <typename T> struct OpLsqrUpdate {
    static constexpr bool REDUCE = true;
    T *__restrict__ x; T *__restrict__ w; const T *__restrict__ v; T t1, t2, inv_rho;
    __device__ __forceinline__ void apply(int64_t i, T &acc) const
    {
        const T wo = w[i];
        T a = t1 * wo; x[i] = x[i] + a;
        T b = t2 * wo; const T wn = b + v[i]; w[i] = wn;
        const T r = wn * inv_rho;
        T p = r * r; acc = acc + p;
    }
    __device__ __forceinline__ void apply_vec(int64_t i, T &acc) const
    {
        constexpr int W = VT<T>::W;
        auto xv = vload_nt<T>(x + i); auto wv = vload<T>(w + i); auto vv = vload(v + i);
#pragma unroll
        for (int e = 0; e < W; ++e) {
            const T wo = el<T>(wv, e);
            T a = t1 * wo; el<T>(xv, e) = el<T>(xv, e) + a;
            T b = t2 * wo; el<T>(wv, e) = b + el<T>(vv, e);
        }
        vstore_nt(x + i, xv); vstore(w + i, wv);
#pragma unroll
        for (int e = 0; e < W; ++e) { const T r = el<T>(wv, e) * inv_rho; T p = r * r; acc = acc + p; }
    }
};

template <typename T> struct OpLsmrUpdate {
    static constexpr bool REDUCE = true;
    T *__restrict__ hbar; T *__restrict__ h; T *__restrict__ x; const T *__restrict__ v; T c1, c2, c3;
    __device__ __forceinline__ void apply(int64_t i, T &acc) const
    {
        const T ho = h[i];
        T a = hbar[i] * c1; const T hb = a + ho; hbar[i] = hb;
        T b = c2 * hb; const T xn = x[i] + b; x[i] = xn;
        T c = ho * c3; h[i] = c + v[i];
        T p = xn * xn; acc = acc + p;
    }
    __device__ __forceinline__ void apply_vec(int64_t i, T &acc) const
    {
        constexpr int W = VT<T>::W;
        auto hbv = vload<T>(hbar + i); auto hv = vload<T>(h + i); auto xv = vload<T>(x + i); auto vv = vload(v + i);
#pragma unroll
        for (int e = 0; e < W; ++e) {
            const T ho = el<T>(hv, e);
            T a = el<T>(hbv, e) * c1; el<T>(hbv, e) = a + ho;
            T b = c2 * el<T>(hbv, e); el<T>(xv, e) = el<T>(xv, e) + b;
            T c = ho * c3; el<T>(hv, e) = c + el<T>(vv, e);
        }
        vstore(hbar + i, hbv); vstore(h + i, hv); vstore(x + i, xv);
#pragma unroll
        for (int e = 0; e < W; ++e) { T p = el<T>(xv, e) * el<T>(xv, e); acc = acc + p; }
    }
};

template <typename T> struct OpAxpy2Dot {
    static constexpr bool REDUCE = true;
    T *__restrict__ y; const T *__restrict__ x1; const T *__restrict__ x2; const T *__restrict__ z; T a, b;
    __device__ __forceinline__ void apply(int64_t i, T &acc) const
    {
        T t = a * x1[i]; T v = y[i] + t;
        if (x2) { T u = b * x2[i]; v = v + u; }
        y[i] = v;
        if (z) { T p = v * z[i]; acc = acc + p; }
    }
    __device__ __forceinline__ void apply_vec(int64_t i, T &acc) const
    {
        constexpr int W = VT<T>::W;
        auto yv = vload<T>(y + i); auto xv = vload(x1 + i);
#pragma unroll
        for (int e = 0; e < W; ++e) { T t = a * el<T>(xv, e); el<T>(yv, e) = el<T>(yv, e) + t; }
        if (x2) {
            auto x2v = vload(x2 + i);
#pragma unroll
            for (int e = 0; e < W; ++e) { T u = b * el<T>(x2v, e); el<T>(yv, e) = el<T>(yv, e) + u; }
        }
        vstore(y + i, yv);
        if (z) {
            auto zv = vload(z + i);
#pragma unroll
            for (int e = 0; e < W; ++e) { T p = el<T>(yv, e) * el<T>(zv, e); acc = acc + p; }
        }
    }
};

template <typename T> struct OpScal2 {
    static constexpr bool REDUCE = false;
    T *__restrict__ x; T *__restrict__ y; T a, b;
    __device__ __forceinline__ void apply(int64_t i, T &) const { x[i] = x[i] * a; y[i] = y[i] * b; }
    __device__ __forceinline__ void apply_vec(int64_t i, T &) const
    {
        auto xv = vload<T>(x + i); auto yv = vload<T>(y + i);
#pragma unroll
        for (int e = 0; e < VT<T>::W; ++e) { el<T>(xv, e) = el<T>(xv, e) * a; el<T>(yv, e) = el<T>(yv, e) * b; }
        vstore(x + i, xv); vstore(y + i, yv);
    }
};

template <typename T> struct OpQmrUpdate {
    static constexpr bool REDUCE = false;
    const T *__restrict__ v; const T *p_curr; const T *p_prev; T *p_out; T *__restrict__ x; T neg_h1, neg_h0, inv, g;
    __device__ __forceinline__ void apply(int64_t i, T &) const
    {
        T p = v[i];
        if (p_curr) { T t = neg_h1 * p_curr[i]; p = p + t; }
        if (p_prev) { T t = neg_h0 * p_prev[i]; p = p + t; }
        p = p * inv;
        p_out[i] = p;
        T t = g * p; x[i] = x[i] + t;
    }
    __device__ __forceinline__ void apply_vec(int64_t i, T &) const
    {
        constexpr int W = VT<T>::W;
        auto pv = vload(v + i); auto xv = vload_nt<T>(x + i);
        if (p_curr) {
            auto cv = vload(p_curr + i);
#pragma unroll
            for (int e = 0; e < W; ++e) { T t = neg_h1 * el<T>(cv, e); el<T>(pv, e) = el<T>(pv, e) + t; }
        }
        if (p_prev) {
            auto qv = vload(p_prev + i);
#pragma unroll
            for (int e = 0; e < W; ++e) { T t = neg_h0 * el<T>(qv, e); el<T>(pv, e) = el<T>(pv, e) + t; }
        }
#pragma unroll
        for (int e = 0; e < W; ++e) { el<T>(pv, e) = el<T>(pv, e) * inv; T t = g * el<T>(pv, e); el<T>(xv, e) = el<T>(xv, e) + t; }
        vstore(p_out + i, pv); vstore_nt(x + i, xv);
    }
};

template <typename T> struct OpXpbyX {
    static constexpr bool REDUCE = false;
    const T *__restrict__ r; T *__restrict__ u; T *__restrict__ x; Coef<T> beta, alpha;
    const int *__restrict__ done; const int *__restrict__ pending; int nt = 0;
    __device__ __forceinline__ void apply(int64_t i, T &) const
    {
        const int dn = *done, pd = *pending;
        if (dn && !pd) return;
        const T uo = u[i];
        if (pd) { T t = alpha.get() * uo; x[i] = x[i] + t; }
        if (!dn) { T t = beta.get() * uo; u[i] = r[i] + t; }
    }
    __device__ __forceinline__ void apply_vec(int64_t i, T &) const
    {
        const int dn = *done, pd = *pending;
        if (dn && !pd) return;
        auto uv = (nt & 2) ? vload_nt<T>(u + i) : vload<T>(u + i);
        if (pd) {
            const T a = alpha.get();
            auto xv = (nt & 8) ? vload_nt<T>(x + i) : vload<T>(x + i);
#pragma unroll
            for (int e = 0; e < VT<T>::W; ++e) { T t = a * el<T>(uv, e); el<T>(xv, e) = el<T>(xv, e) + t; }
            if (nt & 8) vstore_nt(x + i, xv); else vstore(x + i, xv);
        }
        if (!dn) {
            const T b = beta.get();
            auto rv = (nt & 1) ? vload_nt(r + i) : vload(r + i);
#pragma unroll
            for (int e = 0; e < VT<T>::W; ++e) { T t = b * el<T>(uv, e); el<T>(uv, e) = el<T>(rv, e) + t; }
            if (nt & 4) vstore_nt(u + i, uv); else vstore(u + i, uv);
        }
    }
};

template <typename T> struct CoefAlphaRanks {
    const T *all; int nranks; const T *res;
    __device__ __forceinline__ T get() const
    {
        T tot = all[0];
        for (int p = 1; p < nranks; ++p) tot = tot + all[p];
        const T r = *res;
        return (r * r) / tot;
    }
};
template <typename T, typename C = Coef<T>> struct OpCgUpdateR {
    static constexpr bool REDUCE = true;
    T *__restrict__ r; const T *__restrict__ c; C alpha; int nt = 0;
    __device__ __forceinline__ void apply(int64_t i, T &acc) const
    {
        T s = alpha.get() * c[i]; T rn = r[i] - s; r[i] = rn;
        T p = rn * rn; acc = acc + p;
    }
    __device__ __forceinline__ void apply_vec(int64_t i, T &acc) const
    {
        const T a = alpha.get();
        auto rv = (nt & 8) ? vload_nt<T>(r + i) : vload<T>(r + i);
        auto cv = (nt & 2) ? vload_nt(c + i) : vload(c + i);
#pragma unroll
        for (int e = 0; e < VT<T>::W; ++e) { T s = a * el<T>(cv, e); el<T>(rv, e) = el<T>(rv, e) - s; }
        if (nt & 16) vstore_nt(r + i, rv); else vstore(r + i, rv);
#pragma unroll
        for (int e = 0; e < VT<T>::W; ++e) { T p = el<T>(rv, e) * el<T>(rv, e); acc = acc + p; }
    }
};

template <typename T> struct OpPcgUpdateR {
    static constexpr bool REDUCE = true;
    T *__restrict__ r; T *__restrict__ c; const T *__restrict__ d; Coef<T> alpha; int nt = 0;
    __device__ __forceinline__ void apply(int64_t i, T &a1, T &a2) const
    {
        T s = alpha.get() * c[i]; T rn = r[i] - s; r[i] = rn;
        T p = rn * rn; a1 = a1 + p;
        T v = rn / d[i]; c[i] = v;
        T q = v * rn; a2 = a2 + q;
    }
    __device__ __forceinline__ void apply_vec(int64_t i, T &a1, T &a2) const
    {
        const T a = alpha.get();
        auto rv = (nt & 8) ? vload_nt<T>(r + i) : vload<T>(r + i);
        auto cv = (nt & 64) ? vload_nt<T>(c + i) : vload<T>(c + i);
        auto dv = vload_nt(d + i);
#pragma unroll
        for (int e = 0; e < VT<T>::W; ++e) { T s = a * el<T>(cv, e); el<T>(rv, e) = el<T>(rv, e) - s; }
        if (nt & 16) vstore_nt(r + i, rv); else vstore(r + i, rv);
#pragma unroll
        for (int e = 0; e < VT<T>::W; ++e) { T p = el<T>(rv, e) * el<T>(rv, e); a1 = a1 + p; }
#pragma unroll
        for (int e = 0; e < VT<T>::W; ++e) el<T>(cv, e) = el<T>(rv, e) / el<T>(dv, e);
        if (nt & 32) vstore_nt(c + i, cv); else vstore(c + i, cv);
#pragma unroll
        for (int e = 0; e < VT<T>::W; ++e) { T q = el<T>(cv, e) * el<T>(rv, e); a2 = a2 + q; }
    }
};

template <typename T> struct OpXFlush {
    static constexpr bool REDUCE = false;
    const T *__restrict__ u; T *__restrict__ x; Coef<T> alpha; const int *__restrict__ pending;
    __device__ __forceinline__ void apply(int64_t i, T &) const
    {
        if (!*pending) return;
        T t = alpha.get() * u[i]; x[i] = x[i] + t;
    }
    __device__ __forceinline__ void apply_vec(int64_t i, T &) const
    {
        if (!*pending) return;
        const T a = alpha.get();
        auto uv = vload(u + i); auto xv = vload<T>(x + i);
#pragma unroll
        for (int e = 0; e < VT<T>::W; ++e) { T t = a * el<T>(uv, e); el<T>(xv, e) = el<T>(xv, e) + t; }
        vstore(x + i, xv);
    }
};

template <typename T> struct OpAxpy {
    static constexpr bool REDUCE = false;
    const T *__restrict__ x; T *__restrict__ y; Coef<T> alpha;
    __device__ __forceinline__ void apply(int64_t i, T &) const { T t = alpha.get() * x[i]; y[i] = y[i] + t; }
    __device__ __forceinline__ void apply_vec(int64_t i, T &) const
    {
        const T a = alpha.get();
        auto xv = vload(x + i); auto yv = vload<T>(y + i);
#pragma unroll
        for (int e = 0; e < VT<T>::W; ++e) { T t = a * el<T>(xv, e); el<T>(yv, e) = el<T>(yv, e) + t; }
        vstore(y + i, yv);
    }
};

template <typename T> struct OpBicgU {
    static constexpr bool REDUCE = false;
    T *__restrict__ us; int64_t ldu; const T *__restrict__ rs; int64_t ldr; int ncols; Coef<T> neg_beta;
    int nt = 0;
    __device__ __forceinline__ void apply(int64_t i, T &) const
    {
        const T b = neg_beta.get();
        for (int q = 0; q < ncols; ++q) { T *u = us + q * ldu; T t = b * u[i]; u[i] = rs[q * ldr + i] + t; }
    }
    __device__ __forceinline__ void apply_vec(int64_t i, T &) const
    {
        const T b = neg_beta.get();
        for (int q = 0; q < ncols; ++q) {
            T *u = us + q * ldu;
            auto xv = (nt & 1) ? vload_nt(rs + q * ldr + i) : vload(rs + q * ldr + i);
            auto yv = (nt & 1) ? vload_nt<T>(u + i) : vload<T>(u + i);
#pragma unroll
            for (int e = 0; e < VT<T>::W; ++e) { T t = b * el<T>(yv, e); el<T>(yv, e) = el<T>(xv, e) + t; }
            if (q + 1 < ncols ? (nt & 2) : (nt & 4)) vstore_nt(u + i, yv); else vstore(u + i, yv);
        }
    }
};
template <typename T> struct OpBicgR {
    static constexpr bool REDUCE = false;
    const T *__restrict__ us; int64_t ldu; T *__restrict__ rs; int64_t ldr; int ncols; T *__restrict__ x; Coef<T> neg_alpha, alpha;
    int nt = 0;
    __device__ __forceinline__ void apply(int64_t i, T &) const
    {
        const T na = neg_alpha.get(), a = alpha.get();
        for (int q = 0; q < ncols; ++q) { T t = na * us[(q + 1) * ldu + i]; rs[q * ldr + i] = rs[q * ldr + i] + t; }
        { T t = a * us[i]; x[i] = x[i] + t; }
    }
    __device__ __forceinline__ void apply_vec(int64_t i, T &) const
    {
// ... 65 lines not shown

template <typename T> struct OpFill {
    static constexpr bool REDUCE = false;
    T *__restrict__ x; T value;
    __device__ __forceinline__ void apply(int64_t i, T &) const { x[i] = value; }
    __device__ __forceinline__ void apply_vec(int64_t i, T &) const
    {
        typename VT<T>::vec v;
#pragma unroll
        for (int e = 0; e < VT<T>::W; ++e) el<T>(v, e) = value;
        vstore(x + i, v);
    }
};

template <typename T> struct OpDot {
    static constexpr bool REDUCE = true;
    const T *__restrict__ x; const T *__restrict__ y;
    __device__ __forceinline__ void apply(int64_t i, T &acc) const { T p = x[i] * y[i]; acc = acc + p; }
    __device__ __forceinline__ void apply_vec(int64_t i, T &acc) const
    {
        auto xv = vload(x + i); auto yv = vload(y + i);
#pragma unroll
        for (int e = 0; e < VT<T>::W; ++e) { T p = el<T>(xv, e) * el<T>(yv, e); acc = acc + p; }
    }
};

template <typename T> struct OpSubNrm {
    static constexpr bool REDUCE = true;
    const T *__restrict__ a; const T *__restrict__ b; T *__restrict__ out;
    __device__ __forceinline__ void apply(int64_t i, T &acc) const
    {
        T v = b ? a[i] - b[i] : a[i];
        out[i] = v;
        T p = v * v; acc = acc + p;
    }
    __device__ __forceinline__ void apply_vec(int64_t i, T &acc) const
    {
        auto av = vload(a + i);
        if (b) {
            auto bv = vload(b + i);
#pragma unroll
            for (int e = 0; e < VT<T>::W; ++e) el<T>(av, e) = el<T>(av, e) - el<T>(bv, e);
        }
        vstore(out + i, av);
#pragma unroll
        for (int e = 0; e < VT<T>::W; ++e) { T p = el<T>(av, e) * el<T>(av, e); acc = acc + p; }
    }
};

template <typename T> struct OpScaledSq {
    static constexpr bool REDUCE = true;
    const T *__restrict__ x; T s;
    __device__ __forceinline__ void apply(int64_t i, T &acc) const { T q = x[i] * s; T p = q * q; acc = acc + p; }
    __device__ __forceinline__ void apply_vec(int64_t i, T &acc) const
    {
        auto xv = vload(x + i);
#pragma unroll
        for (int e = 0; e < VT<T>::W; ++e) { T q = el<T>(xv, e) * s; T p = q * q; acc = acc + p; }
    }
};

template <typename T> __device__ __forceinline__ T amax_fold(T m, T a) { return (a > m || a != a) ? a : m; }
template <typename T>
__global__ __launch_bounds__(MIK_BLOCK) void k_amax(int64_t n, const T *__restrict__ x, T *__restrict__ part)
{
    __shared__ T sm[MIK_BLOCK];
    T m = T(0);
    for (int64_t i = (int64_t)blockIdx.x * MIK_BLOCK + threadIdx.x; i < n; i += (int64_t)gridDim.x * MIK_BLOCK) {
        const T v = x[i];
        m = amax_fold(m, v < T(0) ? -v : v);
    }
    sm[threadIdx.x] = m;
    __syncthreads();
    for (int off = MIK_BLOCK / 2; off >= 1; off >>= 1) {
        if ((int)threadIdx.x < off) sm[threadIdx.x] = amax_fold(sm[threadIdx.x], sm[threadIdx.x + off]);
        __syncthreads();
    }
    if (threadIdx.x == 0) part[blockIdx.x] = sm[0];
}

template <typename T> struct OpCgUpdate {
    static constexpr bool REDUCE = true;
    T *__restrict__ x; T *__restrict__ r; const T *__restrict__ u; const T *__restrict__ c; Coef<T> alpha;
    int nt = 0;
    __device__ __forceinline__ void apply(int64_t i, T &acc) const
    {
        const T a = alpha.get();
        T t = a * u[i]; x[i] = x[i] + t;
        T s = a * c[i]; T rn = r[i] - s; r[i] = rn;
        T p = rn * rn; acc = acc + p;
    }
    __device__ __forceinline__ void apply_vec(int64_t i, T &acc) const
    {
        const T a = alpha.get();
        auto xv = (nt & 1) ? vload_nt<T>(x + i) : vload<T>(x + i);
        auto uv = (nt & 4) ? vload_nt(u + i) : vload(u + i);
        auto rv = (nt & 8) ? vload_nt<T>(r + i) : vload<T>(r + i);
        auto cv = (nt & 2) ? vload_nt(c + i) : vload(c + i);
#pragma unroll
        for (int e = 0; e < VT<T>::W; ++e) {
            T t = a * el<T>(uv, e); el<T>(xv, e) = el<T>(xv, e) + t;
            T s = a * el<T>(cv, e); el<T>(rv, e) = el<T>(rv, e) - s;
        }
        if (nt & 1) vstore_nt(x + i, xv); else vstore(x + i, xv);
        if (nt & 16) vstore_nt(r + i, rv); else vstore(r + i, rv);
#pragma unroll
        for (int e = 0; e < VT<T>::W; ++e) { T p = el<T>(rv, e) * el<T>(rv, e); acc = acc + p; }
    }
};

template <typename T> struct OpAxpyDot {
    static constexpr bool REDUCE = true;
    const T *x; T *y; const T *z; Coef<T> alpha;
    int nt = 0;
    __device__ __forceinline__ void apply(int64_t i, T &acc) const
    {
        T yv = y[i];
        if (x) { T t = alpha.get() * x[i]; yv = yv + t; y[i] = yv; }
        T p = (z ? z[i] : yv) * yv; acc = acc + p;
    }
    __device__ __forceinline__ void apply_vec(int64_t i, T &acc) const
    {
        auto yv = vload<T>(y + i);
        typename VT<T>::vec zv;
        if (z) zv = vload(z + i);
        if (x) {
            auto xv = (nt & 1) ? vload_nt(x + i) : vload(x + i);
            const T a = alpha.get();
#pragma unroll
            for (int e = 0; e < VT<T>::W; ++e) { T t = a * el<T>(xv, e); el<T>(yv, e) = el<T>(yv, e) + t; }
            vstore(y + i, yv);
        }
#pragma unroll
        for (int e = 0; e < VT<T>::W; ++e) { T p = (z ? el<T>(zv, e) : el<T>(yv, e)) * el<T>(yv, e); acc = acc + p; }
    }
};

template <typename T> struct OpMinresUpdate {
    static constexpr bool REDUCE = false;
    T *__restrict__ v_next; const T *__restrict__ v_curr; const T *__restrict__ w_curr; const T *__restrict__ w_prev;
    T *__restrict__ w_next; T *__restrict__ x;
    Coef<T> inv_h3, neg_h1, neg_h0, inv_h2, rhs0;
    int nt = 0;
    __device__ __forceinline__ void apply(int64_t i, T &) const
    {
        v_next[i] = v_next[i] * inv_h3.get();
        T w = v_curr[i];
        if (w_curr) { T t = neg_h1.get() * w_curr[i]; w = w + t; }
        if (w_prev) { T t = neg_h0.get() * w_prev[i]; w = w + t; }
        w = w * inv_h2.get();
        w_next[i] = w;
        T t = rhs0.get() * w; x[i] = x[i] + t;
    }
    __device__ __forceinline__ void apply_vec(int64_t i, T &) const
    {
        auto vn = vload<T>(v_next + i); auto w = vload(v_curr + i);
        auto xv = (nt & 1) ? vload_nt<T>(x + i) : vload<T>(x + i);
        typename VT<T>::vec wc, wp;
        if (w_curr) wc = (nt & 8) ? vload_nt(w_curr + i) : vload(w_curr + i);
        if (w_prev) wp = (nt & 2) ? vload_nt(w_prev + i) : vload(w_prev + i);
        const T c3 = inv_h3.get(), c1 = w_curr ? neg_h1.get() : T(0), c0 = w_prev ? neg_h0.get() : T(0), c2 = inv_h2.get(), cr = rhs0.get();
#pragma unroll
        for (int e = 0; e < VT<T>::W; ++e) {
            el<T>(vn, e) = el<T>(vn, e) * c3;
            T we = el<T>(w, e);
            if (w_curr) { T t = c1 * el<T>(wc, e); we = we + t; }
            if (w_prev) { T t = c0 * el<T>(wp, e); we = we + t; }
            we = we * c2;
            el<T>(w, e) = we;
            T t = cr * we; el<T>(xv, e) = el<T>(xv, e) + t;
        }
        vstore(v_next + i, vn);
        if (nt & 4) vstore_nt(w_next + i, w); else vstore(w_next + i, w);
        if (nt & 1) vstore_nt(x + i, xv); else vstore(x + i, xv);
    }
};

// ... 732 lines not shown
```

### iterativesolvers.jl_amd/csrc/mik_krylov.hip

```cpp
#include <algorithm>
#include <cfloat>
#include <cstddef>
#include <cmath>
#include <map>
#include <new>
#include <tuple>

#include "mik_kernels.h"
#include "mik_mgs_res.h"
#include "mik_complex.h"
#include "mik_iter.h"
#include "mik_mail.h"


template <typename T> static void givens_algorithm(T f, T g, T &cs, T &sn, T &r)
{
    const T eps = std::numeric_limits<T>::epsilon();
    const T safmin = std::numeric_limits<T>::min();
    const T safmn2 = std::pow(T(2), T((int)(std::log(safmin / eps) / std::log(T(2)) / T(2))));
    const T safmx2 = T(1) / safmn2;
    if (g == T(0)) { cs = T(1); sn = T(0); r = f; return; }
    if (f == T(0)) { cs = T(0); sn = T(1); r = g; return; }
    T f1 = f, g1 = g;
    T scale = std::max(std::fabs(f1), std::fabs(g1));
// ... 495 lines not shown
__global__ void k_cg_fix_res(CgDev<T> *d, T res, T *__restrict__ hist, long long it_next, long long maxiter, CgMirror *mirror,
                             unsigned long long seq, int hist_index, int pcg_fused = 0)
{
    d->done = 0;
    mirror->range = 0;
    cg_res_scalars(d, res * res, res, hist, it_next, maxiter, mirror, seq, hist_index, pcg_fused);
}

template <typename T>
__global__ __launch_bounds__(64) void k_cg_fin_res2(const T *__restrict__ S1, const T *__restrict__ S2, int64_t m, CgDev<T> *d, T *__restrict__ hist,
                                                     long long it_next, long long maxiter, CgMirror *mirror, unsigned long long seq, int hist_index,
                                                     FinScratch2<T> *fs)
{
    if (d->done) {
        if (blockIdx.x == 0 && threadIdx.x == 0) __hip_atomic_store(&mirror->seq, seq, __ATOMIC_RELEASE, __HIP_MEMORY_SCOPE_SYSTEM);
        return;
    }
    T tot, tot2;
    if (level2_sum_spread2(S1, S2, m, fs, tot, tot2)) {
        d->x_pending = 1;
        const T rho_prev = d->rho;
        d->rho = tot2;
        d->beta_rho = tot2 / rho_prev;
        if (!mik_nrm_in_range(tot)) {
            d->done = 1;
            mirror->done = 0;
            mirror->nhist = hist_index;
            mirror->range = 1;
            __hip_atomic_store(&mirror->seq, seq, __ATOMIC_RELEASE, __HIP_MEMORY_SCOPE_SYSTEM);
            return;
        }
        cg_res_scalars(d, tot, mik_sqrt(tot), hist, it_next, maxiter, mirror, seq, hist_index, 1);
    }
}

static int cg_profile_collect(mik_cg *it)
{
    size_t i = 0;
    for (; i + 1 < it->ev_used; i += 2) {
        if (hipEventQuery(it->ev[i + 1]) != hipSuccess) { (void)hipGetLastError(); break; }
        float ms = 0.f;
        const int kind = it->ev_kind[i / 2];
        if (hipEventElapsedTime(&ms, it->ev[i], it->ev[i + 1]) == hipSuccess) { it->kern_ms[kind] += ms; it->kern_launches[kind] += 1; }
    }
    size_t keep = 0;
    for (size_t j = i; j + 1 < it->ev_used; j += 2, keep += 2) {
        std::swap(it->ev[keep], it->ev[j]);
        std::swap(it->ev[keep + 1], it->ev[j + 1]);
        it->ev_kind[keep / 2] = it->ev_kind[j / 2];
    }
    it->ev_used = keep;
    return MIK_OK;
}

static void cg_profile_flush(mik_cg *it)
{
    if (!it->ev_used) return;
    (void)hipStreamSynchronize(it->ctx->stream);
    (void)cg_profile_collect(it);
}

struct CgProfileScope {
    mik_cg *it; bool on;
    CgProfileScope(mik_cg *it_, int kind) : it(it_), on(it_->profile == 2 || (it_->profile == 1 && kind == 0))
    {
        if (!on) return;
        if (it->ev_used + 2 > it->ev.size()) {
            hipEvent_t a, b;
            if (hipEventCreate(&a) != hipSuccess || hipEventCreate(&b) != hipSuccess) { on = false; return; }
            it->ev.push_back(a); it->ev.push_back(b);
            it->ev_kind.push_back(0);
        }
        it->ev_kind[it->ev_used / 2] = kind;
        (void)hipEventRecord(it->ev[it->ev_used], it->ctx->stream);
    }
    ~CgProfileScope()
    {
        if (!on) return;
        (void)hipEventRecord(it->ev[it->ev_used + 1], it->ctx->stream);
        it->ev_used += 2;
    }
};

static inline int cg_stream_hints(const mik_ctx *ctx, bool fused_x = false, const mik_csr *A = nullptr)
{
    (void)ctx;
    return fused_x ? (mik_spmv_is_light(A) ? 248 : 121) : 57;
}


static inline int cg_sweep_u_hints(const mik_cg *it) { return it->fuse_x ? cg_stream_hints(it->ctx, true, it->A) & 15 : cg_stream_hints(it->ctx) & 7; }

template <typename T> static int cg_sweep_u(mik_cg *it, const T *src, int64_t lo, int64_t len, bool vec, int hints)
{
    CgDev<T> *d = (CgDev<T> *)it->dev;
    T *x = (T *)it->x, *u = (T *)it->u;
    if (it->fuse_x) {
        OpXpbyX<T> op{src + lo, u + lo, x + lo, coef_ptr<T>(&d->beta), coef_ptr<T>(&d->alpha), &d->done, &d->x_pending, hints};
        return launch_map<T>(it->ctx, len, op, vec, (T *)nullptr, (const int *)nullptr);
    }
    OpXpby<T> op{src + lo, u + lo, coef_ptr<T>(&d->beta), hints};
    return launch_map<T>(it->ctx, len, op, vec, (T *)nullptr, &d->done);
}

template <typename T, typename C> static int cg_update_xr(mik_cg *it, C alpha, bool vec)
{
    CgDev<T> *d = (CgDev<T> *)it->dev;
    T *x = (T *)it->x, *u = (T *)it->u, *r = (T *)it->r, *c = (T *)it->c;
    if (it->fuse_x) {
        OpCgUpdateR<T, C> up{r, c, alpha, cg_stream_hints(it->ctx, true, it->A) >> 3};
        return launch_map<T>(it->ctx, it->n, up, vec, (T *)it->seg_vec, &d->done);
    }
    if constexpr (std::is_same<C, Coef<T>>::value) {
        OpCgUpdate<T> up{x, r, u, c, alpha, cg_stream_hints(it->ctx) >> 3};
        return launch_map<T>(it->ctx, it->n, up, vec, (T *)it->seg_vec, &d->done);
    }
    return mik_fail(it->ctx, MIK_ERR_INVALID, "cg: alpha formed inside the sweep needs the x update on the next sweep over u");
}

template <typename T> __global__ void k_cg_clear_pending(CgDev<T> *d) { d->x_pending = 0; }

template <typename T> static int cg_flush_x(mik_cg *it)
{
    mik_ctx *ctx = it->ctx;
    CgDev<T> *d = (CgDev<T> *)it->dev;
    T *x = (T *)it->x, *u = (T *)it->u;
    OpXFlush<T> op{u, x, coef_ptr<T>(&d->alpha), &d->x_pending};
    MIK_TRY((launch_map<T>(ctx, it->n, op, mik_aligned16(x) && mik_aligned16(u), (T *)nullptr, (const int *)nullptr)));
    hipLaunchKernelGGL((k_cg_clear_pending<T>), dim3(1), dim3(1), 0, ctx->stream, d);
    MIK_LAUNCH_CHECK(ctx);
    return MIK_OK;
}

template <typename T> static int cg_init_residual(mik_cg *it, const T *x0, bool vec)
{
    mik_ctx *ctx = it->ctx;
    T *c = (T *)it->c;
    it->mv_products = x0 ? 1 : 0;
    if (x0) {
        if (it->A) MIK_TRY(mik_spmv_launch<T>(ctx, it->A, x0, c, false, nullptr, nullptr));
        else if (it->op_mul(it->op_user, x0, c) != 0) return mik_fail(ctx, MIK_ERR_CALLBACK, "cg: the operator callback failed");
    }
    OpSubNrm<T> op{(const T *)it->b, x0 ? c : nullptr, (T *)it->r};
    return launch_map<T>(ctx, it->n, op, vec, (T *)it->seg_vec, nullptr);
}

template <typename T> static int cg_enqueue_head(mik_cg *it)
{
    mik_ctx *ctx = it->ctx;
    CgDev<T> *d = (CgDev<T> *)it->dev;
    const int *done = &d->done;
    const int64_t n = it->n, nseg = mik_nseg<T>(n);
    T *x = (T *)it->x, *u = (T *)it->u, *r = (T *)it->r, *c = (T *)it->c;
    const bool vec = mik_aligned16(x) && mik_aligned16(u) && mik_aligned16(r) && mik_aligned16(c) && (!it->diag || mik_aligned16(it->diag));
    const int pcg = (it->diag || it->pl_fn) ? 1 : 0;
    if (it->pcg_fused) {
    } else if (it->diag) {
        OpJacobiDot<T> pj{r, (const T *)it->diag, c, cg_stream_hints(ctx) != 0};
        MIK_TRY((launch_map<T>(ctx, n, pj, vec, (T *)it->seg_vec, done)));
    } else if (it->pl_fn) {
        if (it->pl_fn(it->pl_user, c, r) != 0) return mik_fail(ctx, MIK_ERR_CALLBACK, "cg: the preconditioner callback failed");
        OpDot<T> dcr{c, r};
        MIK_TRY((launch_map<T>(ctx, n, dcr, vec, (T *)it->seg_vec, done)));
    }
    if (pcg && !it->pcg_fused) {
        hipLaunchKernelGGL((k_cg_fin_rho<T>), dim3(MIK_FIN_WGS), dim3(64), 0, ctx->stream, (const T *)it->seg_vec, nseg, d, (FinScratch<T> *)it->fin);
        MIK_LAUNCH_CHECK(ctx);
    }
    {
        CgProfileScope ps(it, 1);
        const int pcg_hints = it->fuse_x ? (cg_stream_hints(ctx, true, it->A) & 8) | 1 : cg_stream_hints(ctx) & 1;
        MIK_TRY(cg_sweep_u<T>(it, pcg ? c : r, 0, n, vec, pcg ? pcg_hints : cg_sweep_u_hints(it)));
    }
    if (it->A) {
        CgProfileScope ps(it, 0);
        MIK_TRY(mik_spmv_launch<T>(ctx, it->A, u, c, true, (T *)it->seg_spmv, done));
    } else {
        if (it->op_mul(it->op_user, u, c) != 0) return mik_fail(ctx, MIK_ERR_CALLBACK, "cg: the operator callback failed");
        OpDot<T> duc{u, c};
        MIK_TRY((launch_map<T>(ctx, n, duc, vec, (T *)it->seg_vec, done)));
    }
    hipLaunchKernelGGL((k_cg_fin_alpha<T>), dim3(MIK_FIN_WGS), dim3(64), 0, ctx->stream, (const T *)(it->A ? it->seg_spmv : it->seg_vec), it->A ? mik_spmv_nwg(n) : nseg,
                       d, pcg, (FinScratch<T> *)it->fin);
    MIK_LAUNCH_CHECK(ctx);
    return MIK_OK;
}

template <typename T> static int cg_enqueue_tail(mik_cg *it, long long it_next, int hist_index)
{
    mik_ctx *ctx = it->ctx;
    CgDev<T> *d = (CgDev<T> *)it->dev;
    const int *done = &d->done;
    const int64_t n = it->n, nseg = mik_nseg<T>(n);
    T *x = (T *)it->x, *u = (T *)it->u, *r = (T *)it->r, *c = (T *)it->c;
    const bool vec = mik_aligned16(x) && mik_aligned16(u) && mik_aligned16(r) && mik_aligned16(c) && (!it->diag || mik_aligned16(it->diag));
    if (it->pcg_fused) {
        {
            CgProfileScope ps(it, 2);
            OpPcgUpdateR<T> up{r, c, (const T *)it->diag, coef_ptr<T>(&d->alpha), 120};
            MIK_TRY((launch_map2<T>(ctx, n, up, vec, (T *)it->seg_vec, (T *)it->seg_vec2, done)));
        }
        it->seq += 1;
        hipLaunchKernelGGL((k_cg_fin_res2<T>), dim3(MIK_FIN_WGS), dim3(64), 0, ctx->stream, (const T *)it->seg_vec, (const T *)it->seg_vec2, nseg, d, (T *)it->hist,
                           it_next, (long long)it->maxiter, it->mirror, it->seq, hist_index, (FinScratch2<T> *)((unsigned char *)it->fin + 512));
        MIK_LAUNCH_CHECK(ctx);
        return MIK_OK;
    }
    {
        CgProfileScope ps(it, 2);
        MIK_TRY(cg_update_xr<T>(it, coef_ptr<T>(&d->alpha), vec));
    }
    it->seq += 1;
    hipLaunchKernelGGL((k_cg_fin_res<T>), dim3(MIK_FIN_WGS), dim3(64), 0, ctx->stream, (const T *)it->seg_vec, nseg, d, (T *)it->hist,
                       it_next, (long long)it->maxiter, it->mirror, it->seq, hist_index, (FinScratch<T> *)it->fin, it->fuse_x ? 1 : 0);
    MIK_LAUNCH_CHECK(ctx);
    return MIK_OK;
}

int cg_wait_mirror(mik_cg *it)
{
    return mik_wait_seq(it->ctx, &it->mirror->seq, it->seq, "cg", "step", "a step");
}

template <typename T> static int cg_fetch_state(mik_cg *it, CgDev<T> *host)
{
    mik_ctx *ctx = it->ctx;
    MIK_HIP(ctx, hipMemcpyAsync(ctx->coef_host, it->dev, sizeof(CgDev<T>), hipMemcpyDeviceToHost, ctx->stream));
    MIK_HIP(ctx, hipStreamSynchronize(ctx->stream));
    memcpy(host, ctx->coef_host, sizeof(CgDev<T>));
    return MIK_OK;
}

template <typename T>
static int cg_init_impl(mik_cg *it, double abstol, double reltol, int initially_zero)
{
    mik_ctx *ctx = it->ctx;
    const int64_t n = it->n, nseg = mik_nseg<T>(n);
    T *u = (T *)it->u, *r = (T *)it->r, *c = (T *)it->c;
    OpFill<T> z{u, T(0)};
    MIK_TRY((launch_map<T>(ctx, n, z, mik_aligned16(u), (T *)nullptr, nullptr)));
    const bool vec = mik_aligned16(r) && mik_aligned16(it->b) && mik_aligned16(c);
    MIK_TRY(cg_init_residual<T>(it, initially_zero ? nullptr : (const T *)it->x, vec));
    hipLaunchKernelGGL((k_cg_fin_init<T>), dim3(1), dim3(MIK_FIN_THREADS), 0, ctx->stream, (const T *)it->seg_vec, nseg,
                       (CgDev<T> *)it->dev, (T)reltol, (T)abstol, (long long)it->maxiter);
    MIK_LAUNCH_CHECK(ctx);
    CgDev<T> h;
    MIK_TRY(cg_fetch_state<T>(it, &h));
    if (!mik_nrm_in_range(h.rr)) {
        T res;
        MIK_TRY(mik_safe_norm_slow<T>(ctx, n, r, &res));
        hipLaunchKernelGGL((k_cg_set_init<T>), dim3(1), dim3(1), 0, ctx->stream, (CgDev<T> *)it->dev, res, (T)reltol, (T)abstol, (long long)it->maxiter);
        MIK_LAUNCH_CHECK(ctx);
        MIK_TRY(cg_fetch_state<T>(it, &h));
    }
    it->residual = (double)h.res;
    it->prev_residual = (double)h.prev_res;
    it->tol = (double)h.tol;
    it->dev_done = h.done != 0;
    if (it->pcg_fused) {
        OpJacobiDot<T> pj{r, (const T *)it->diag, c, 0};
        MIK_TRY((launch_map<T>(ctx, n, pj, vec && mik_aligned16(it->diag), (T *)it->seg_vec, (const int *)nullptr)));
        hipLaunchKernelGGL((k_cg_fin_rho<T>), dim3(MIK_FIN_WGS), dim3(64), 0, ctx->stream, (const T *)it->seg_vec, nseg, (CgDev<T> *)it->dev, (FinScratch<T> *)it->fin);
        MIK_LAUNCH_CHECK(ctx);
    }
    return MIK_OK;
}

static int cg_create_common(mik_ctx *ctx, const mik_csr *A, int dtype, int64_t n, mik_mul_fn op_mul, void *op_user, const void *jacobi_diag,
                            mik_ldiv_fn pl_fn, void *pl_user, void *x, const void *b, void *u, void *r, void *c, double abstol, double reltol,
                            int64_t maxiter, int initially_zero, mik_cg **out)
{
    MIK_REFUSE_COMPLEX(ctx, A, "mik_cg_create");
    if (n && (!x || !b || !u || !r || !c)) return mik_fail(ctx, MIK_ERR_INVALID, "mik_cg_create: NULL vector");
    mik_cg *it = new (std::nothrow) mik_cg();
    if (!it) return mik_fail(ctx, MIK_ERR_NOMEM, "mik_cg_create: host allocation failed");
    it->ctx = ctx; it->A = A; it->dtype = dtype; it->n = n;
    it->op_mul = op_mul; it->op_user = op_user; it->pl_fn = pl_fn; it->pl_user = pl_user;
    it->x = x; it->b = b; it->u = u; it->r = r; it->c = c; it->diag = jacobi_diag;
    it->maxiter = maxiter;
    it->fuse_x = A != nullptr && !pl_fn && (ctx->tuning[MIK_KNOB_CG_STEP] & 1) == 0;
    it->pcg_fused = it->fuse_x && jacobi_diag != nullptr && (ctx->tuning[MIK_KNOB_CG_STEP] & 2) == 0;
    const size_t es = mik_dtype_size(dtype);
    const int64_t nseg = dtype == MIK_F64 ? mik_nseg<double>(n) : mik_nseg<float>(n);
    const int64_t nb = mik_spmv_nwg(n);
    hipError_t e;
    (void)hipSetDevice(ctx->device);
    if ((e = hipMalloc(&it->dev, 256)) != hipSuccess || (e = hipMalloc(&it->fin, 1024)) != hipSuccess ||
        (e = hipMemsetAsync(it->fin, 0, 1024, ctx->stream)) != hipSuccess ||
        (it->pcg_fused && (e = hipMalloc(&it->seg_vec2, es * (size_t)std::max<int64_t>(nseg, 1))) != hipSuccess) || (e = hipMalloc(&it->seg_spmv, es * (size_t)std::max<int64_t>(nb, 1))) != hipSuccess ||
        (e = hipMalloc(&it->seg_vec, es * (size_t)std::max<int64_t>(nseg, 1))) != hipSuccess ||
        (e = hipMalloc(&it->hist, es * 64)) != hipSuccess) {
        mik_cg_destroy(it);
        return mik_fail(ctx, MIK_ERR_NOMEM, "mik_cg_create: hipMalloc: %s", hipGetErrorString(e));
    }
    it->hist_cap = 64;
    if ((e = hipHostMalloc((void **)&it->mirror, sizeof(CgMirror), hipHostMallocMapped | hipHostMallocCoherent)) != hipSuccess) {
        mik_cg_destroy(it);
        return mik_fail(ctx, MIK_ERR_NOMEM, "mik_cg_create: hipHostMalloc: %s", hipGetErrorString(e));
    }
    memset(it->mirror, 0, sizeof(CgMirror));
    int rc = dtype == MIK_F64 ? cg_init_impl<double>(it, abstol, reltol, initially_zero)
                              : cg_init_impl<float>(it, abstol, reltol, initially_zero);
    if (rc) { mik_cg_destroy(it); return rc; }
    *out = it;
    return MIK_OK;
}

extern "C" int mik_cg_create(mik_ctx *ctx, const mik_csr *A, void *x, const void *b, void *u, void *r, void *c,
                             const void *jacobi_diag, double abstol, double reltol, int64_t maxiter, int initially_zero,
                             mik_cg **out)
{
    if (!ctx || !out) return MIK_ERR_INVALID;
    *out = nullptr;
    if (!A || A->n_rows != A->n_cols) return mik_fail(ctx, MIK_ERR_MISMATCH, "mik_cg_create: A must be square");
    return cg_create_common(ctx, A, A->dtype, A->n_rows, nullptr, nullptr, jacobi_diag, nullptr, nullptr, x, b, u, r, c, abstol, reltol, maxiter,
                            initially_zero, out);
}

static int resolve_operator(mik_ctx *ctx, const mik_operator *A, const char *who, const mik_csr **csr, int *dtype, int64_t *n)
{
    if (!A || (!A->csr && !A->mul)) return mik_fail(ctx, MIK_ERR_INVALID, "%s: the operator needs a csr handle or a mul callback", who);
    if (A->csr) {
        if (A->csr->n_rows != A->csr->n_cols) return mik_fail(ctx, MIK_ERR_MISMATCH, "%s: A must be square", who);
        *csr = A->csr; *dtype = A->csr->dtype; *n = A->csr->n_rows;
        return MIK_OK;
    }
    if ((A->dtype != MIK_F64 && A->dtype != MIK_F32) || A->n < 0) return mik_fail(ctx, MIK_ERR_INVALID, "%s: bad dtype / size of the callback operator", who);
    *csr = nullptr; *dtype = A->dtype; *n = A->n;
    return MIK_OK;
}

extern "C" int mik_cg_create_op(mik_ctx *ctx, const mik_operator *A, const mik_precond *Pl, void *x, const void *b, void *u, void *r, void *c,
                                double abstol, double reltol, int64_t maxiter, int initially_zero, mik_cg **out)
{
    if (!ctx || !out) return MIK_ERR_INVALID;
    *out = nullptr;
    const mik_csr *csr = nullptr;
    int dtype = MIK_F64;
    int64_t n = 0;
    MIK_TRY(resolve_operator(ctx, A, "mik_cg_create_op", &csr, &dtype, &n));
    if (Pl && Pl->diag && Pl->ldiv) return mik_fail(ctx, MIK_ERR_INVALID, "mik_cg_create_op: Pl has both a diagonal and a callback");
    return cg_create_common(ctx, csr, dtype, n, csr ? nullptr : A->mul, A->user, Pl ? Pl->diag : nullptr, Pl ? Pl->ldiv : nullptr,
                            Pl ? Pl->user : nullptr, x, b, u, r, c, abstol, reltol, maxiter, initially_zero, out);
}

extern "C" int mik_cg_destroy(mik_cg *it)
{
    if (!it) return MIK_OK;
    if (it->ctx) (void)hipStreamSynchronize(it->ctx->stream);
    if (it->dev) (void)hipFree(it->dev);
    if (it->fin) (void)hipFree(it->fin);
    if (it->hist) (void)hipFree(it->hist);
    if (it->seg_spmv) (void)hipFree(it->seg_spmv);
    if (it->seg_vec) (void)hipFree(it->seg_vec);
    if (it->seg_vec2) (void)hipFree(it->seg_vec2);
    for (hipEvent_t e : it->ev) (void)hipEventDestroy(e);
    if (it->mirror) (void)hipHostFree(it->mirror);
    delete it;
    return MIK_OK;
}

template <typename T> struct CgLocal {
    mik_cg *it;
    T res = T(0);
// ... 14 lines not shown
    }
    int collect(const CgMirror &m, double *, double *, double *residuals, int64_t, int64_t *steps_done)
    {
        mik_ctx *ctx = it->ctx;
        const int64_t nd = m.nhist;
        if (nd == 1) {
            if (residuals) residuals[0] = m.res;
        } else if (nd > 1) {
            std::vector<T> tmp((size_t)nd);
            MIK_HIP(ctx, hipMemcpyAsync(tmp.data(), it->hist, sizeof(T) * (size_t)nd, hipMemcpyDeviceToHost, ctx->stream));
            MIK_HIP(ctx, hipStreamSynchronize(ctx->stream));
            if (residuals) for (int64_t j = 0; j < nd; ++j) residuals[j] = (double)tmp[j];
        }
        if (nd > 0) {
            it->residual = m.res;
            it->prev_residual = m.prev_res;
        }
        it->dev_done = m.done != 0;
        it->mv_products += nd;
        *steps_done = nd;
        if (it->profile) cg_profile_collect(it);
        return MIK_OK;
    }
};

template <typename T>
static int cg_iterate_many_impl(mik_cg *it, int64_t iteration, int64_t max_steps, double *residuals, int64_t *steps_done)
{
    mik_ctx *ctx = it->ctx;
    *steps_done = 0;
    if (max_steps <= 0 || iteration >= it->maxiter || it->residual <= it->tol) return MIK_OK;
    max_steps = std::min(max_steps, it->maxiter - iteration);
    if ((it->op_mul || it->pl_fn) && max_steps > 1) {
        int64_t total = 0;
        for (int64_t j = 0; j < max_steps; ++j) {
            int64_t nd1 = 0;
            double res1 = 0;
            MIK_TRY(cg_iterate_many_impl<T>(it, iteration + j, 1, &res1, &nd1));
            if (nd1 == 0) break;
            if (residuals) residuals[total] = res1;
            total += 1;
        }
        *steps_done = total;
        return MIK_OK;
    }
    if (max_steps > it->hist_cap) {
        MIK_HIP(ctx, hipStreamSynchronize(ctx->stream));
        MIK_HIP(ctx, hipFree(it->hist));
        it->hist = nullptr;
        MIK_HIP(ctx, hipMalloc(&it->hist, sizeof(T) * (size_t)max_steps));
        it->hist_cap = max_steps;
    }
    it->mirror->nhist = 0;
    it->mirror->range = 0;
    if (it->dev_done) MIK_HIP(ctx, hipMemsetAsync(&((CgDev<T> *)it->dev)->done, 0, sizeof(int), ctx->stream));
    const bool ahead_ok = ctx->tuning[MIK_KNOB_NO_LOOKAHEAD] == 0 && !it->op_mul && !it->pl_fn && iteration + max_steps < it->maxiter;
    CgLocal<T> rk{it};
    return cg_run_batch(rk, iteration, max_steps, ahead_ok, residuals, steps_done);
}

extern "C" int mik_cg_iterate_many(mik_cg *it, int64_t iteration, int64_t max_steps, double *residuals, int64_t *steps_done)
{
    if (!it || !steps_done || iteration < 0) return MIK_ERR_INVALID;
    return it->dtype == MIK_F64 ? cg_iterate_many_impl<double>(it, iteration, max_steps, residuals, steps_done)
                                : cg_iterate_many_impl<float>(it, iteration, max_steps, residuals, steps_done);
}

extern "C" int mik_cg_iterate(mik_cg *it, int64_t iteration, double *residual, int *done)
{
    if (!it || !done) return MIK_ERR_INVALID;
    int64_t nd = 0;
    double res = 0;
    int rc = mik_cg_iterate_many(it, iteration, 1, &res, &nd);
    if (rc) return rc;
    *done = nd == 0 ? 1 : 0;
    if (residual) *residual = it->residual;
    return MIK_OK;
}

extern "C" int mik_cg_fused_x(const mik_cg *it, int *fused)
{
    if (!it || !fused) return MIK_ERR_INVALID;
    *fused = it->fuse_x ? 1 : 0;
    return MIK_OK;
}

extern "C" int mik_cg_profile(mik_cg *it, int enable, double *spmv_ms_total, int64_t *spmv_launches)
{
    if (!it) return MIK_ERR_INVALID;
    cg_profile_flush(it);
    if (spmv_ms_total) *spmv_ms_total = it->kern_ms[0];
    if (spmv_launches) *spmv_launches = it->kern_launches[0];
    if (enable >= 0) {
        it->profile = enable;
        if (enable) { for (int q = 0; q < 3; ++q) { it->kern_ms[q] = 0; it->kern_launches[q] = 0; } it->ev_used = 0; }
    }
    return MIK_OK;
}

extern "C" int mik_cgd_profile(mik_cgd *it, int enable, double *spmv_ms_total, int64_t *spmv_launches)
{
    if (!it) return MIK_ERR_INVALID;
    return mik_cg_profile(&it->base, enable > 1 ? 1 : enable, spmv_ms_total, spmv_launches);
}

extern "C" int mik_cg_profile_kernels(const mik_cg *it, double *ms_total, int64_t *launches)
{
    if (!it) return MIK_ERR_INVALID;
    cg_profile_flush(const_cast<mik_cg *>(it));
    for (int q = 0; q < 3; ++q) {
        if (ms_total) ms_total[q] = it->kern_ms[q];
        if (launches) launches[q] = it->kern_launches[q];
    }
    return MIK_OK;
}

extern "C" int mik_cg_state(const mik_cg *it, double *residual, double *prev_residual, double *tol, int64_t *maxiter,
                            int64_t *mv_products, int *converged)
{
    if (!it) return MIK_ERR_INVALID;
    if (residual) *residual = it->residual;
    if (prev_residual) *prev_residual = it->prev_residual;
    if (tol) *tol = it->tol;
    if (maxiter) *maxiter = it->maxiter;
    if (mv_products) *mv_products = it->mv_products;
    if (converged) *converged = it->residual <= it->tol ? 1 : 0;
    return MIK_OK;
}

struct mik_gmres {
    mik_ctx *ctx = nullptr;
    const mik_csr *A = nullptr;
    int dtype = MIK_F64;
    int64_t n = 0, ldv = 0;
    void *x = nullptr;
    const void *b = nullptr;
    const void *pl = nullptr, *pr = nullptr;
    mik_mul_fn op_mul = nullptr;
    void *op_user = nullptr;
    mik_ldiv_fn pl_fn = nullptr, pr_fn = nullptr;
    void *pl_user = nullptr, *pr_user = nullptr;
    void *V = nullptr;
    void *Ax = nullptr;
    std::vector<double> H64; std::vector<float> H32;
    std::vector<double> nv64; std::vector<float> nv32;
    double current = 1, accumulator = 1, res_beta = 1;
    double g_beta = 1, tol = 0;
    int k = 1, restart = 0, method = MIK_MGS;
    int64_t maxiter = 0, mv_products = 0;
    bool dist = false;
    mik_partition part{};
    void *mgs_P = nullptr;
    int mgs_G = 1, mgs_stride = 256;
    int mgs_res_S = 0;
    int gs_timeouts = 0;
    bool fused_off = false;
    unsigned *xl_chk = nullptr;
    bool xl_off = false;
    bool xl_last = false;
    int mgs_rounds = 1;
    MgsMirror *mgs_mirror = nullptr;
    size_t mgs_mirror_stride = 0;
    unsigned long long mgs_seq = 0, mgs_slot_seq[2] = {0, 0};
    int mgs_parity = 0;
    int pre_k = 0, pre_slot = 0;
};
// ... 542 lines not shown
}

template <typename T>
__global__ __launch_bounds__(64) void k_cgd_fin_slot_alpha(const T *__restrict__ S, int64_t m, T *__restrict__ slot, const int *__restrict__ done,
                                                           FinScratch<T> *fs, const T *__restrict__ dot_all, int nranks, CgDev<T> *d)
{
    if (blockIdx.x == 0 && threadIdx.x == 0) d->x_pending = 0;
    if (done && *done) return;
    T tot;
    if (level2_sum_spread(S, m, fs, tot)) {
        *slot = tot;
        const T dt = rank_sum(dot_all, nranks);
        d->dot_uc = dt;
        d->alpha = (d->res * d->res) / dt;
    }
}

template <typename T> __global__ void k_cgd_alpha(const T *__restrict__ dot_all, int nranks, CgDev<T> *d)
{
    d->x_pending = 0;
    if (d->done) return;
    const T tot = rank_sum(dot_all, nranks);
    d->dot_uc = tot;
    d->alpha = (d->res * d->res) / tot;
}

template <typename T> __device__ __forceinline__ void cgd_publish_init(const CgDev<T> *d, CgMirror *mirror, unsigned long long seq)
{
    mirror->res = (double)d->res; mirror->prev_res = 1.0; mirror->done = d->done; mirror->nhist = 0;
    mirror->tol = (double)d->tol; mirror->tol_valid = 1;
    __hip_atomic_store(&mirror->seq, seq, __ATOMIC_RELEASE, __HIP_MEMORY_SCOPE_SYSTEM);
}

template <typename T>
__global__ void k_cgd_fin_init(const T *__restrict__ rr_all, int nranks, CgDev<T> *d, T reltol, T abstol, long long maxiter, CgMirror *mirror,
                               unsigned long long seq)
{
    const T tot = rank_sum(rr_all, nranks);
    if (!mik_nrm_in_range(tot)) {
        d->done = 1; mirror->done = 0; mirror->range = 1;
        __hip_atomic_store(&mirror->seq, seq, __ATOMIC_RELEASE, __HIP_MEMORY_SCOPE_SYSTEM);
        return;
    }
    cg_init_scalars(d, tot, mik_sqrt(tot), reltol, abstol, maxiter);
    cgd_publish_init(d, mirror, seq);
}

template <typename T>
__global__ void k_cgd_fin_res(const T *__restrict__ rr_all, int nranks, CgDev<T> *d, T *__restrict__ hist, long long it_next, long long maxiter,
                              CgMirror *mirror, unsigned long long seq, int hist_index, int fuse_x)
{
    if (d->done) { __hip_atomic_store(&mirror->seq, seq, __ATOMIC_RELEASE, __HIP_MEMORY_SCOPE_SYSTEM); return; }
    cgd_close_step<T>(d, rank_sum(rr_all, nranks), hist, it_next, maxiter, mirror, seq, hist_index, fuse_x);
}

template <typename T>
__global__ void k_cgd_fix_init(CgDev<T> *d, T res, T reltol, T abstol, long long maxiter, CgMirror *mirror, unsigned long long seq)
{
    cg_init_scalars(d, res * res, res, reltol, abstol, maxiter);
    mirror->range = 0;
    cgd_publish_init(d, mirror, seq);
}

extern "C" int mik_cgd_create(mik_ctx *ctx, const mik_csr *A_loc, void *x, const void *b, void *u_ext, void *r, void *c,
                              const int32_t *send_idx, int64_t n_send, void *send_buf, void *dot_all, void *rr_all, int rank,
                              int nranks, double abstol, double reltol, int64_t maxiter, int initially_zero, mik_cgd **out)
{
    if (!ctx || !out) return MIK_ERR_INVALID;
    *out = nullptr;
    if (!A_loc || A_loc->n_cols < A_loc->n_rows) return mik_fail(ctx, MIK_ERR_MISMATCH, "mik_cgd_create: local block must be n_loc x (n_loc + n_ghost)");
    MIK_REFUSE_COMPLEX(ctx, A_loc, "mik_cgd_create");
    if (nranks < 1 || rank < 0 || rank >= nranks || !dot_all || !rr_all || (n_send && (!send_idx || !send_buf)))
        return mik_fail(ctx, MIK_ERR_INVALID, "mik_cgd_create: bad rank / comm buffers");
    const int64_t n = A_loc->n_rows;
    if (n && (!x || !b || !u_ext || !r || !c)) return mik_fail(ctx, MIK_ERR_INVALID, "mik_cgd_create: NULL vector");
    mik_cgd *it = new (std::nothrow) mik_cgd();
    if (!it) return mik_fail(ctx, MIK_ERR_NOMEM, "mik_cgd_create: host allocation failed");
    mik_cg &bs = it->base;
    bs.ctx = ctx; bs.A = A_loc; bs.dtype = A_loc->dtype; bs.n = n;
    bs.x = x; bs.b = b; bs.u = u_ext; bs.r = r; bs.c = c; bs.maxiter = maxiter;
    it->rank = rank; it->nranks = nranks; it->n_send = n_send; it->send_idx = send_idx; it->send_buf = send_buf;
    it->u_ext = u_ext; it->n_ext = A_loc->n_cols; it->dot_all = dot_all; it->rr_all = rr_all;
    it->abstol = abstol; it->reltol = reltol; it->initially_zero = initially_zero;
    const size_t es = mik_dtype_size(A_loc->dtype);
    const int64_t nseg = A_loc->dtype == MIK_F64 ? mik_nseg<double>(n) : mik_nseg<float>(n);
    const int64_t nb = mik_spmv_nwg(n);
    hipError_t e;
    (void)hipSetDevice(ctx->device);
    auto fail = [&](const char *what, hipError_t err) {
        int rc = mik_fail(ctx, MIK_ERR_NOMEM, "mik_cgd_create: %s: %s", what, hipGetErrorString(err));
        mik_cgd_destroy(it);
        return rc;
    };
    if ((e = hipMalloc(&bs.dev, 256)) != hipSuccess) return fail("hipMalloc", e);
    if ((e = hipMalloc(&bs.seg_spmv, es * (size_t)std::max<int64_t>(nb, 1))) != hipSuccess) return fail("hipMalloc", e);
    if ((e = hipMalloc(&bs.seg_vec, es * (size_t)std::max<int64_t>(nseg, 1))) != hipSuccess) return fail("hipMalloc", e);
    if ((e = hipMalloc(&bs.hist, es * 1024)) != hipSuccess) return fail("hipMalloc", e);
    bs.hist_cap = 1024;
    if ((e = hipMalloc(&bs.fin, 256)) != hipSuccess || (e = hipMemsetAsync(bs.fin, 0, 256, ctx->stream)) != hipSuccess) return fail("hipMalloc", e);
    if ((e = hipHostMalloc((void **)&bs.mirror, sizeof(CgMirror), hipHostMallocMapped | hipHostMallocCoherent)) != hipSuccess) return fail("hipHostMalloc", e);
    memset(bs.mirror, 0, sizeof(CgMirror));
    if ((e = hipMemsetAsync(bs.dev, 0, 256, ctx->stream)) != hipSuccess) return fail("hipMemsetAsync", e);
    *out = it;
    return MIK_OK;
}

extern "C" int mik_cgd_set_interior(mik_cgd *it, int64_t rb_begin, int64_t rb_end)
{
    if (!it) return MIK_ERR_INVALID;
    const int64_t nb = mik_spmv_nwg(it->base.n);
    if (rb_begin < 0 || rb_end < rb_begin || rb_end > nb) return mik_fail(it->base.ctx, MIK_ERR_INVALID, "mik_cgd_set_interior: bad range");
    if (!mik_spmv_can_split(it->base.A)) return mik_fail(it->base.ctx, MIK_ERR_NOTIMPL, "mik_cgd_set_interior: the operator's layout cannot be launched over a row-block range");
    it->int_begin = rb_begin;
    it->int_end = rb_end;
    return MIK_OK;
}

void mik_cgd_group_forget(mik_cgd *it);

extern "C" int mik_cgd_destroy(mik_cgd *it)
{
    if (!it) return MIK_OK;
    mik_cgd_group_forget(it);
    mik_cg &bs = it->base;
    if (bs.ctx) (void)hipStreamSynchronize(bs.ctx->stream);
    if (it->link) { (void)mik_plink_destroy(it->link); it->link = nullptr; }
    if (bs.dev) (void)hipFree(bs.dev);
    if (bs.hist) (void)hipFree(bs.hist);
    if (bs.fin) (void)hipFree(bs.fin);
    if (bs.seg_spmv) (void)hipFree(bs.seg_spmv);
    if (bs.seg_vec) (void)hipFree(bs.seg_vec);
    if (bs.mirror) (void)hipHostFree(bs.mirror);
    delete it;
    return MIK_OK;
}

template <typename T> static int cgd_phase_impl(mik_cgd *it, int phase, int64_t iteration)
{
    mik_cg &bs = it->base;
    mik_ctx *ctx = bs.ctx;
    CgDev<T> *d = (CgDev<T> *)bs.dev;
    const int *done = &d->done;
    const int64_t n = bs.n, nseg = mik_nseg<T>(n), nb = mik_spmv_nwg(n);
    T *x = (T *)bs.x, *u = (T *)it->u_ext, *r = (T *)bs.r, *c = (T *)bs.c;
    T *dot_slot = (T *)it->dot_all + it->rank, *rr_slot = (T *)it->rr_all + it->rank;
    const bool vec = mik_aligned16(x) && mik_aligned16(u) && mik_aligned16(r) && mik_aligned16(c) && mik_aligned16(bs.b);
    switch (phase) {
    case MIK_CGD_INIT_A:
        if (!it->initially_zero) {
            MIK_HIP(ctx, hipMemcpyAsync(u, x, sizeof(T) * (size_t)n, hipMemcpyDeviceToDevice, ctx->stream));
            MIK_TRY(gather_launch<T>(ctx, it->n_send, it->send_idx, u, (T *)it->send_buf, nullptr));
        }
        return MIK_OK;
    case MIK_CGD_INIT_B: {
        MIK_TRY(cg_init_residual<T>(&bs, it->initially_zero ? nullptr : u, vec));
        hipLaunchKernelGGL((k_finalize_store<T>), dim3(1), dim3(MIK_FIN_THREADS), 0, ctx->stream, (const T *)bs.seg_vec, nseg, (int64_t)0, rr_slot,
                           (const int *)nullptr);
        MIK_LAUNCH_CHECK(ctx);
        OpFill<T> z{u, T(0)};
        return launch_map<T>(ctx, it->n_ext, z, mik_aligned16(u), (T *)nullptr, nullptr);
    }
    case MIK_CGD_INIT_C:
        bs.seq += 1;
        hipLaunchKernelGGL((k_cgd_fin_init<T>), dim3(1), dim3(1), 0, ctx->stream, (const T *)it->rr_all, it->nranks, d, (T)it->reltol, (T)it->abstol,
                           (long long)bs.maxiter, bs.mirror, bs.seq);
        MIK_LAUNCH_CHECK(ctx);
        return MIK_OK;
    case MIK_CGD_STEP_A:
        MIK_TRY(cg_sweep_u<T>(&bs, r, 0, n, vec, cg_sweep_u_hints(&bs)));
        return gather_launch<T>(ctx, it->n_send, it->send_idx, u, (T *)it->send_buf, done);
    case CGD_STEP_A_EARLY:
    case CGD_STEP_A_BULK: {
        if (it->n_early <= 0) return mik_fail(ctx, MIK_ERR_INVALID, "mik_cgd_phase: no early rows (mik_cgd_set_halo_plan)");
        int64_t lo[3], hi[3];
        int nr = 0;
        if (phase == CGD_STEP_A_EARLY) {
            for (int q = 0; q < it->n_early; ++q) { lo[nr] = it->early_a[q]; hi[nr] = it->early_b[q]; ++nr; }
        } else {
            int64_t at = 0;
            for (int q = 0; q < it->n_early; ++q) {
                if (it->early_a[q] > at) { lo[nr] = at; hi[nr] = it->early_a[q]; ++nr; }
                at = it->early_b[q];
            }
            if (at < n) { lo[nr] = at; hi[nr] = n; ++nr; }
        }
        for (int q = 0; q < nr; ++q)
            MIK_TRY(cg_sweep_u<T>(&bs, r, lo[q], hi[q] - lo[q], vec && (lo[q] % VT<T>::W == 0), cg_sweep_u_hints(&bs)));
        if (phase == CGD_STEP_A_EARLY) return gather_launch<T>(ctx, it->n_send, it->send_idx, u, (T *)it->send_buf, done);
        return MIK_OK;
    }
    case CGD_STEP_A_EARLY_MERGED: {
        if (it->n_early <= 0 || !it->early_merged) return mik_fail(ctx, MIK_ERR_INVALID, "mik_cgd_phase: no merged early part");
        const int grid = (int)std::min<int64_t>((it->n_send + MIK_BLOCK - 1) / MIK_BLOCK, mik_max_grid(ctx));
        hipLaunchKernelGGL((k_cgd_early<T>), dim3(grid), dim3(MIK_BLOCK), 0, ctx->stream, it->n_send, it->send_idx, (const T *)r, u, x, (const T *)&d->beta,
                           (const T *)&d->alpha, done, (const int *)&d->x_pending, bs.fuse_x ? 1 : 0, (T *)it->send_buf);
        MIK_LAUNCH_CHECK(ctx);
        return MIK_OK;
    }
    case CGD_X_FLUSH: return cg_flush_x<T>(&bs);
    case MIK_CGD_STEP_B:
    case CGD_STEP_B_NOFIN:
    case MIK_CGD_STEP_B_REST:
    case CGD_STEP_B_REST_NOFIN: {
        const bool rest = phase == MIK_CGD_STEP_B_REST || phase == CGD_STEP_B_REST_NOFIN;
        {
            CgProfileScope ps(&bs, 0);
            if (rest) MIK_TRY(mik_spmv_launch_outside<T>(ctx, bs.A, u, c, true, (T *)bs.seg_spmv, done, (int)it->int_begin, (int)it->int_end));
            else MIK_TRY(mik_spmv_launch<T>(ctx, bs.A, u, c, true, (T *)bs.seg_spmv, done));
        }
        if (phase == CGD_STEP_B_NOFIN || phase == CGD_STEP_B_REST_NOFIN) return MIK_OK;
        hipLaunchKernelGGL((k_cgd_fin_slot<T>), dim3(MIK_FIN_WGS), dim3(64), 0, ctx->stream, (const T *)bs.seg_spmv, nb, dot_slot, done, (FinScratch<T> *)bs.fin);
        MIK_LAUNCH_CHECK(ctx);
        return MIK_OK;
    }
    case MIK_CGD_STEP_B_INTERIOR:
        if (it->int_end <= it->int_begin) return mik_fail(ctx, MIK_ERR_INVALID, "mik_cgd_phase: no interior range set (mik_cgd_set_interior)");
        { CgProfileScope ps(&bs, 0); return mik_spmv_launch_range<T>(ctx, bs.A, u, c, true, (T *)bs.seg_spmv, done, (int)it->int_begin, (int)(it->int_end - it->int_begin)); }
    case MIK_CGD_STEP_C: {
        if (bs.fuse_x && (ctx->tuning[MIK_KNOB_CG_STEP] & 8) == 0) {
            MIK_TRY(cg_update_xr<T>(&bs, CoefAlphaRanks<T>{(const T *)it->dot_all, it->nranks, &d->res}, vec));
            hipLaunchKernelGGL((k_cgd_fin_slot_alpha<T>), dim3(MIK_FIN_WGS), dim3(64), 0, ctx->stream, (const T *)bs.seg_vec, nseg, rr_slot, done,
                               (FinScratch<T> *)bs.fin, (const T *)it->dot_all, it->nranks, d);
            MIK_LAUNCH_CHECK(ctx);
            return MIK_OK;
        }
        hipLaunchKernelGGL((k_cgd_alpha<T>), dim3(1), dim3(1), 0, ctx->stream, (const T *)it->dot_all, it->nranks, d);
        MIK_LAUNCH_CHECK(ctx);
        MIK_TRY(cg_update_xr<T>(&bs, coef_ptr<T>(&d->alpha), vec));
        hipLaunchKernelGGL((k_cgd_fin_slot<T>), dim3(MIK_FIN_WGS), dim3(64), 0, ctx->stream, (const T *)bs.seg_vec, nseg, rr_slot, done, (FinScratch<T> *)bs.fin);
        MIK_LAUNCH_CHECK(ctx);
        return MIK_OK;
    }
    case MIK_CGD_STEP_D:
        if (it->hist_total >= bs.hist_cap) return mik_fail(ctx, MIK_ERR_INVALID, "mik_cgd_phase: more than %lld steps enqueued without mik_cgd_wait", (long long)bs.hist_cap);
        it->hist_total += 1;
        bs.seq += 1;
        hipLaunchKernelGGL((k_cgd_fin_res<T>), dim3(1), dim3(1), 0, ctx->stream, (const T *)it->rr_all, it->nranks, d, (T *)bs.hist,
                           (long long)(iteration + 1), (long long)bs.maxiter, bs.mirror, bs.seq, (int)(it->hist_total - 1), bs.fuse_x ? 1 : 0);
        MIK_LAUNCH_CHECK(ctx);
        return MIK_OK;
    case CGD_NORM_AMAX: {
        const int grid = (int)std::min<int64_t>((std::max<int64_t>(n, 1) + MIK_BLOCK - 1) / MIK_BLOCK, 1024);
        MIK_TRY(mik_ensure_partials(ctx, sizeof(T) * (size_t)std::max<int64_t>(std::max<int64_t>(nseg, grid), 1)));
        hipLaunchKernelGGL((k_amax<T>), dim3(grid), dim3(MIK_BLOCK), 0, ctx->stream, n, (const T *)r, (T *)ctx->partials);
        MIK_LAUNCH_CHECK(ctx);
        hipLaunchKernelGGL((k_amax<T>), dim3(1), dim3(MIK_BLOCK), 0, ctx->stream, (int64_t)grid, (const T *)ctx->partials, rr_slot);
        MIK_LAUNCH_CHECK(ctx);
        return MIK_OK;
    }
    case CGD_NORM_SCALED_SQ: {
        MIK_TRY(mik_ensure_partials(ctx, sizeof(T) * (size_t)std::max<int64_t>(nseg, 1)));
        OpScaledSq<T> op{(const T *)r, (T)it->norm_scale};
        MIK_TRY((launch_map<T>(ctx, n, op, mik_aligned16(r), (T *)ctx->partials, nullptr)));
        hipLaunchKernelGGL((k_finalize_store<T>), dim3(1), dim3(MIK_FIN_THREADS), 0, ctx->stream, (const T *)ctx->partials, nseg, (int64_t)0, rr_slot,
                           (const int *)nullptr);
        MIK_LAUNCH_CHECK(ctx);
        return MIK_OK;
    }
    case CGD_FIX_STEP:
        bs.seq += 1;
        it->hist_total = it->norm_fix_index + 1;
        hipLaunchKernelGGL((k_cg_fix_res<T>), dim3(1), dim3(1), 0, ctx->stream, d, (T)it->norm_res, (T *)bs.hist, (long long)it->norm_it_next,
                           (long long)bs.maxiter, bs.mirror, bs.seq, it->norm_fix_index);
        MIK_LAUNCH_CHECK(ctx);
        return MIK_OK;
    case CGD_STEP_C_NOFIN: return cg_update_xr<T>(&bs, coef_ptr<T>(&d->alpha), vec);
    case CGD_CLEAR_PENDING:
        hipLaunchKernelGGL((k_cg_clear_pending<T>), dim3(1), dim3(1), 0, ctx->stream, d);
        MIK_LAUNCH_CHECK(ctx);
        return MIK_OK;
    case CGD_FIX_INIT:
        bs.seq += 1;
        hipLaunchKernelGGL((k_cgd_fix_init<T>), dim3(1), dim3(1), 0, ctx->stream, d, (T)it->norm_res, (T)it->reltol, (T)it->abstol, (long long)bs.maxiter,
                           bs.mirror, bs.seq);
        MIK_LAUNCH_CHECK(ctx);
        return MIK_OK;
    default:
        return mik_fail(ctx, MIK_ERR_INVALID, "mik_cgd_phase: unknown phase %d", phase);
    }
}

extern "C" int mik_cgd_phase(mik_cgd *it, int phase, int64_t iteration)
{
    if (!it || iteration < 0) return MIK_ERR_INVALID;
    return it->base.dtype == MIK_F64 ? cgd_phase_impl<double>(it, phase, iteration) : cgd_phase_impl<float>(it, phase, iteration);
}

int cgd_wait_raw(mik_cgd *it, CgMirror *m)
{
    MIK_TRY(cg_wait_mirror(&it->base));
    *m = *it->base.mirror;
    return MIK_OK;
}

int cgd_collect(mik_cgd *it, const CgMirror &m, double *residual, double *tol, int *done, double *history, int64_t cap, int64_t *steps)
{
    mik_cg &bs = it->base;
    mik_ctx *ctx = bs.ctx;
    const int64_t nd = m.nhist;
    if (history && nd == 1 && cap >= 1) {
        history[0] = m.res;
    } else if (history && nd > 0) {
        const int64_t take = std::min<int64_t>(nd, cap);
        const size_t es = mik_dtype_size(bs.dtype);
        std::vector<unsigned char> tmp((size_t)take * es);
        MIK_HIP(ctx, hipMemcpyAsync(tmp.data(), bs.hist, es * (size_t)take, hipMemcpyDeviceToHost, ctx->stream));
        MIK_HIP(ctx, mik_wait(ctx));
        for (int64_t j = 0; j < take; ++j)
            history[j] = bs.dtype == MIK_F64 ? ((const double *)tmp.data())[j] : (double)((const float *)tmp.data())[j];
    }
    if (bs.profile) (void)cg_profile_collect(&bs);
    bs.mirror->nhist = 0;
    it->hist_total = 0;
    bs.residual = m.res;
    bs.prev_residual = m.prev_res;
    if (m.tol_valid) bs.tol = m.tol;
    bs.mv_products += nd;
    if (residual) *residual = m.res;
    if (tol) *tol = bs.tol;
    if (done) *done = m.done;
    if (steps) *steps = nd;
    return MIK_OK;
}

extern "C" int mik_cgd_wait(mik_cgd *it, double *residual, double *tol, int *done, double *history, int64_t cap, int64_t *steps)
{
    if (!it) return MIK_ERR_INVALID;
    CgMirror m;
    MIK_TRY(cgd_wait_raw(it, &m));
    if (m.range) {
        mik_ctx *ctx = it->base.ctx;
        if (it->base.fuse_x && it->initialised) {
            (void)mik_cgd_phase(it, CGD_X_FLUSH, 0);
            (void)mik_wait(ctx);
        }
        return mik_fail(ctx, MIK_ERR_RANGE, "cg (row-partitioned, host-driven phases): |r|^2 left the range of a safe norm; use mik_cgd_init / "
                                            "mik_cgd_iterate_many (or the group calls), which rescale across the ranks");
    }
    return cgd_collect(it, m, residual, tol, done, history, cap, steps);
}


template <typename T> static int gemv_t_impl(mik_ctx *ctx, int64_t n, int k, const T *V, int64_t ldv, const T *w, T *h_host)
{
    if (k == 0) return MIK_OK;
    if ((size_t)k * sizeof(T) > mik_ctx::COEF_SAFE_SLOT) return mik_fail(ctx, MIK_ERR_NOTIMPL, "mik_gemv_t: k = %d too large", k);
    const int64_t nseg = mik_nseg<T>(n);
    MIK_TRY(mik_ensure_partials(ctx, sizeof(T) * (size_t)std::max<int64_t>(nseg, 1) * (size_t)k));
    MIK_TRY(multidot<T>(ctx, n, k, V, ldv, w, (T *)ctx->coef));
// ... 118 lines not shown
```

Measured before the change: 2251 iters/s.

## Plan per-vector cache residency for CG using gfx950 MALL size

Adds a residency planner that decides, from the vector size, operator bytes and the last-level (MALL) cache capacity, which prefix of each CG vector (u, r, c, x) is loaded and stored with normal cache-allocating accesses and which tail uses nontemporal hints. The per-element update kernels now choose nontemporal bits by index range, and the row-gather SpMV can switch nontemporal off when the plan keeps the output vector resident. The aim is to let part of the working set stay in the 256 MiB MALL across the SpMV and vector updates so fewer bytes go to HBM each iteration. This adds per-vector branching through readfirstlane, and at n=16M fp64 the vectors are far larger than the cache, so the planner may keep little and the hit gain may be small.

Result: no change. 2291 iters/s (median of 6 runs) (+1.8%).

```diff
diff --git a/include/mik_dev.h b/include/mik_dev.h
--- a/include/mik_dev.h
+++ b/include/mik_dev.h
@@ -36,6 +36,11 @@
 int mik_dev_exclusive_scan(mik_ctx *ctx, int *data, int64_t n);
 int mik_dev_xwin_plan(int64_t n_blocks, const int *first_col, const int *last_col, const int *entries, int elem_size, int64_t n_cols,
                       int64_t total_entries, int *win_lo, int *span);
+int mik_dev_cg_plan(int64_t n, int elem_size, int64_t operator_bytes, int operator_streamed, int64_t cache_bytes, double budget, int step, int64_t *keep,
+                    int *mask, int *spmv_nt);
+int mik_dev_cg_set_plan(mik_cg *it, int64_t keep_u, int64_t keep_r, int64_t keep_c, int64_t keep_x);
+int mik_dev_cgd_set_plan(mik_cgd *it, int64_t keep_u, int64_t keep_r, int64_t keep_c, int64_t keep_x);
+int mik_dev_cg_get_plan(const mik_cg *it, int64_t *keep, int *mask, int *spmv_nt, int64_t *cache_bytes);
 #ifdef __cplusplus
 }
 #endif
diff --git a/iterativesolvers.jl_amd/_lib.py b/iterativesolvers.jl_amd/_lib.py
--- a/iterativesolvers.jl_amd/_lib.py
+++ b/iterativesolvers.jl_amd/_lib.py
@@ -81,6 +81,10 @@
     "mik_dev_spmv_plan": (C.c_int, [_vp, _vp, C.c_int, C.c_int, C.c_int, C.c_int, C.c_int, C.c_char_p, C.c_int, _i64p, _ip, _ip, _ip]),
     "mik_dev_spmv_run": (C.c_int, [_vp, _vp, _vp, _vp, C.c_int, _vp, C.c_int, C.c_int, C.c_int, C.c_int]),
     "mik_dev_exclusive_scan": (C.c_int, [_vp, _vp, _i64]),
+    "mik_dev_cg_plan": (C.c_int, [_i64, C.c_int, _i64, C.c_int, _i64, C.c_double, C.c_int, _i64p, _ip, _ip]),
+    "mik_dev_cg_set_plan": (C.c_int, [_vp, _i64, _i64, _i64, _i64]),
+    "mik_dev_cgd_set_plan": (C.c_int, [_vp, _i64, _i64, _i64, _i64]),
+    "mik_dev_cg_get_plan": (C.c_int, [_vp, _i64p, _ip, _ip, _i64p]),
     "mik_ctx_set_stream": (C.c_int, [_vp, _vp]),
     "mik_ctx_synchronize": (C.c_int, [_vp]),
     "mik_last_error": (C.c_char_p, [_vp]),
diff --git a/iterativesolvers.jl_amd/csrc/mik_comm.hip b/iterativesolvers.jl_amd/csrc/mik_comm.hip
--- a/iterativesolvers.jl_amd/csrc/mik_comm.hip
+++ b/iterativesolvers.jl_amd/csrc/mik_comm.hip
@@ -1214,6 +1214,7 @@
     max_steps = std::min<int64_t>(std::min<int64_t>(max_steps, bs.maxiter - iteration), bs.hist_cap);
     const bool ahead_ok = bs.ctx->tuning[MIK_KNOB_NO_LOOKAHEAD] == 0 && iteration + max_steps < bs.maxiter;
     bs.fuse_x = (bs.ctx->tuning[MIK_KNOB_CG_STEP] & 1) == 0;
+    cg_make_plan(&bs);
     CgdComm rk{it};
     return cg_run_batch(rk, iteration, max_steps, ahead_ok, residuals, steps_done);
 }
@@ -1511,6 +1512,7 @@
         rk.split = rk.split && its[p]->int_end > its[p]->int_begin;
         rk.early = rk.early && its[p]->n_early > 0;
         its[p]->base.fuse_x = (its[p]->base.ctx->tuning[MIK_KNOB_CG_STEP] & 1) == 0;
+        cg_make_plan(&its[p]->base);
     }
     rk.early = rk.early && rk.split;
     return cg_run_batch(rk, iteration, max_steps, false, residuals, steps_done);
diff --git a/iterativesolvers.jl_amd/csrc/mik_core.hip b/iterativesolvers.jl_amd/csrc/mik_core.hip
--- a/iterativesolvers.jl_amd/csrc/mik_core.hip
+++ b/iterativesolvers.jl_amd/csrc/mik_core.hip
@@ -99,6 +99,7 @@
             ctx->hbm_bytes = (int64_t)prop.totalGlobalMem;
             snprintf(ctx->arch, sizeof(ctx->arch), "%s", prop.gcnArchName);
         } else (void)hipGetLastError();
+        if (strncmp(ctx->arch, "gfx950", 6) == 0) ctx->mall_bytes = (int64_t)256 << 20;
         if (ctx->wave_size != 0 && ctx->wave_size != 64) {
             int rc = mik_fail(nullptr, MIK_ERR_HIP, "mik_ctx_create: device %d runs %d-wide wavefronts; libmik's kernels are written for wave-64 (gfx950)", device, ctx->wave_size);
             delete ctx;
@@ -1290,6 +1291,7 @@
     int pb0 = 0, np = 0, pmode = 0, ps = -1, pfull = 0;
     int sshift = -1, nfull = 0, cls = 0;
     bool merge = false, nt_rb = false, xwin = false, rp = false;
+    bool nt_rg = true;
     bool long_win = false;
     int lw_launch = 0;
 };
@@ -1297,7 +1299,8 @@
 static SpmvPlan spmv_refusal(SpmvPlan p, int rc, const char *text) { p.rc = rc; p.refusal = text; return p; }
 static inline bool spmv_ep_armed(const mik_ctx *ctx) { return ctx->spmv_ep_w || ctx->spmv_ep_c || ctx->spmv_ep_z; }
 
-static SpmvPlan spmv_plan(const mik_csr *A, size_t es, bool x_aligned, bool fuse_dot, int rb_begin, int rb_count, int skip_at, int skip_len, bool ep_armed)
+static SpmvPlan spmv_plan(const mik_csr *A, size_t es, bool x_aligned, bool fuse_dot, int rb_begin, int rb_count, int skip_at, int skip_len, bool ep_armed,
+                          int stream_op = -1)
 {
     SpmvPlan p;
     const int *knob = A->ctx->tuning;
@@ -1364,6 +1367,7 @@
         break;
     case SPMV_ROWGATHER:
         p.pre_longrows = nlong > 0;
+        p.nt_rg = stream_op != 0;
         break;
     case SPMV_ROWBLOCK: {
         p.merge = nlong > 0 && !fuse_dot;
@@ -1415,14 +1419,15 @@
     return MIK_OK;
 }
 
-static int spmv_plan_outside(const mik_csr *A, size_t es, bool x_aligned, bool fuse_dot, int skip_begin, int skip_end, bool ep_armed, SpmvPlan out[2])
+static int spmv_plan_outside(const mik_csr *A, size_t es, bool x_aligned, bool fuse_dot, int skip_begin, int skip_end, bool ep_armed, SpmvPlan out[2],
+                             int stream_op = -1)
 {
     const int nb_all = (int)mik_spmv_nwg(A->n_rows), rest = skip_begin + (nb_all - skip_end);
     if (skip_begin < 0 || skip_end < skip_begin || skip_end > nb_all) { out[0] = spmv_refusal(SpmvPlan{}, MIK_ERR_INVALID, "SpMV: bad interior range"); return 1; }
-    out[0] = spmv_plan(A, es, x_aligned, fuse_dot, 0, rest, skip_begin, skip_end - skip_begin, ep_armed);
+    out[0] = spmv_plan(A, es, x_aligned, fuse_dot, 0, rest, skip_begin, skip_end - skip_begin, ep_armed, stream_op);
     if (out[0].skips && rest > 0) return 1;
-    out[0] = spmv_plan(A, es, x_aligned, fuse_dot, 0, skip_begin, SPMV_NO_SKIP, 0, ep_armed);
-    out[1] = spmv_plan(A, es, x_aligned, fuse_dot, skip_end, nb_all - skip_end, SPMV_NO_SKIP, 0, ep_armed);
+    out[0] = spmv_plan(A, es, x_aligned, fuse_dot, 0, skip_begin, SPMV_NO_SKIP, 0, ep_armed, stream_op);
+    out[1] = spmv_plan(A, es, x_aligned, fuse_dot, skip_end, nb_all - skip_end, SPMV_NO_SKIP, 0, ep_armed, stream_op);
     return 2;
 }
 
@@ -1574,10 +1579,10 @@
 template <typename T> static void spmv_go_rowgather(const SpmvPlan &p, const SpmvIO<T> &io)
 {
     const mik_csr *A = io.A;
-    with_consts([&](auto fd) {
-        hipLaunchKernelGGL((k_spmv_rowgather<T, decltype(fd)::value, true>), dim3(p.grid), dim3(MIK_BLOCK), 0, io.ctx->stream, (int)A->n_rows, p.rb0, p.nb,
+    with_consts([&](auto fd, auto nt) {
+        hipLaunchKernelGGL((k_spmv_rowgather<T, decltype(fd)::value, decltype(nt)::value>), dim3(p.grid), dim3(MIK_BLOCK), 0, io.ctx->stream, (int)A->n_rows, p.rb0, p.nb,
                            p.map_mode, A->rowptr, A->col, (const T *)A->val, io.x, io.y, io.seg_out, io.done, A->is_long, io.ep_w(), io.ep_c(), io.ep_z());
-    }, p.fd);
+    }, p.fd, p.nt_rg);
 }
 
 template <typename T> static void spmv_go_rowblock(const SpmvPlan &p, const SpmvIO<T> &io)
@@ -1624,31 +1629,32 @@
 
 template <typename T>
 int mik_spmv_launch_range(mik_ctx *ctx, const mik_csr *A, const T *x, T *y, bool fuse_dot, T *seg_out, const int *done, int rb_begin,
-                          int rb_count)
-{
-    return spmv_run<T>(spmv_plan(A, sizeof(T), mik_aligned16(x), fuse_dot, rb_begin, rb_count, SPMV_NO_SKIP, 0, spmv_ep_armed(ctx)), {ctx, A, x, y, seg_out, done});
+                          int rb_count, int stream_op)
+{
+    return spmv_run<T>(spmv_plan(A, sizeof(T), mik_aligned16(x), fuse_dot, rb_begin, rb_count, SPMV_NO_SKIP, 0, spmv_ep_armed(ctx), stream_op), {ctx, A, x, y, seg_out, done});
 }
 
 template <typename T>
-int mik_spmv_launch(mik_ctx *ctx, const mik_csr *A, const T *x, T *y, bool fuse_dot, T *seg_out, const int *done)
-{
-    return mik_spmv_launch_range<T>(ctx, A, x, y, fuse_dot, seg_out, done, 0, -1);
+int mik_spmv_launch(mik_ctx *ctx, const mik_csr *A, const T *x, T *y, bool fuse_dot, T *seg_out, const int *done, int stream_op)
+{
+    return mik_spmv_launch_range<T>(ctx, A, x, y, fuse_dot, seg_out, done, 0, -1, stream_op);
 }
 
 template <typename T>
-int mik_spmv_launch_outside(mik_ctx *ctx, const mik_csr *A, const T *x, T *y, bool fuse_dot, T *seg_out, const int *done, int skip_begin, int skip_end)
+int mik_spmv_launch_outside(mik_ctx *ctx, const mik_csr *A, const T *x, T *y, bool fuse_dot, T *seg_out, const int *done, int skip_begin, int skip_end,
+                            int stream_op)
 {
     SpmvPlan p[2];
-    const int np = spmv_plan_outside(A, sizeof(T), mik_aligned16(x), fuse_dot, skip_begin, skip_end, spmv_ep_armed(ctx), p);
+    const int np = spmv_plan_outside(A, sizeof(T), mik_aligned16(x), fuse_dot, skip_begin, skip_end, spmv_ep_armed(ctx), p, stream_op);
     for (int i = 0; i < np; ++i) MIK_TRY(spmv_run<T>(p[i], {ctx, A, x, y, seg_out, done}));
     return MIK_OK;
 }
-template int mik_spmv_launch_outside<double>(mik_ctx *, const mik_csr *, const double *, double *, bool, double *, const int *, int, int);
-template int mik_spmv_launch_outside<float>(mik_ctx *, const mik_csr *, const float *, float *, bool, float *, const int *, int, int);
-template int mik_spmv_launch<double>(mik_ctx *, const mik_csr *, const double *, double *, bool, double *, const int *);
-template int mik_spmv_launch<float>(mik_ctx *, const mik_csr *, const float *, float *, bool, float *, const int *);
-template int mik_spmv_launch_range<double>(mik_ctx *, const mik_csr *, const double *, double *, bool, double *, const int *, int, int);
-template int mik_spmv_launch_range<float>(mik_ctx *, const mik_csr *, const float *, float *, bool, float *, const int *, int, int);
+template int mik_spmv_launch_outside<double>(mik_ctx *, const mik_csr *, const double *, double *, bool, double *, const int *, int, int, int);
+template int mik_spmv_launch_outside<float>(mik_ctx *, const mik_csr *, const float *, float *, bool, float *, const int *, int, int, int);
+template int mik_spmv_launch<double>(mik_ctx *, const mik_csr *, const double *, double *, bool, double *, const int *, int);
+template int mik_spmv_launch<float>(mik_ctx *, const mik_csr *, const float *, float *, bool, float *, const int *, int);
+template int mik_spmv_launch_range<double>(mik_ctx *, const mik_csr *, const double *, double *, bool, double *, const int *, int, int, int);
+template int mik_spmv_launch_range<float>(mik_ctx *, const mik_csr *, const float *, float *, bool, float *, const int *, int, int, int);
 
 template <typename T>
 static int dev_spmv_run(mik_ctx *ctx, const mik_csr *A, const void *x, void *y, bool fuse_dot, void *seg_out, int rb_begin, int rb_count, int skip_begin,
diff --git a/iterativesolvers.jl_amd/csrc/mik_internal.h b/iterativesolvers.jl_amd/csrc/mik_internal.h
--- a/iterativesolvers.jl_amd/csrc/mik_internal.h
+++ b/iterativesolvers.jl_amd/csrc/mik_internal.h
@@ -43,6 +43,7 @@
     static constexpr size_t PUB_BYTES = 4096;
     const void *spmv_ep_w = nullptr, *spmv_ep_c = nullptr;
     const void *spmv_ep_z = nullptr;
+    int64_t mall_bytes = 0;
     int tuning[MIK_KNOB_COUNT] = {0};
     static constexpr size_t COEF_BYTES = 8192;
     static constexpr size_t COEF_SAFE_SLOT = 4096;
@@ -66,6 +67,15 @@
     const int64_t P = ((bw + MIK_BLOCK - 1) / MIK_BLOCK + MIK_XCD_MAP - 1) / MIK_XCD_MAP * MIK_XCD_MAP;
     return (P >= MIK_XCD_MAP && P <= nb / 4) ? (int)P : 0;
 }
+
+enum { MIK_CG_STEP_FUSED_X = 0, MIK_CG_STEP_CLASSIC = 1, MIK_CG_STEP_PCG = 2 };
+struct mik_cg_plan {
+    int64_t keep_u = 0, keep_r = 0, keep_c = 0, keep_x = 0;
+    int ranged = 0, mask = 0;
+    int spmv_nt = 1;
+};
+constexpr double MIK_CG_CACHE_BUDGET = 0.75;
+mik_cg_plan mik_cg_residency_plan(int64_t n, size_t es, int64_t op_bytes, bool op_streamed, int64_t cache_bytes, double budget, int step);
 
 int mik_mgs_resident_max_s();
 
@@ -154,12 +164,13 @@
 int mik_build_sdiaw_device(mik_ctx *ctx, mik_csr *A);
 int mik_build_jds_device(mik_ctx *ctx, mik_csr *A);
 template <typename T>
-int mik_spmv_launch(mik_ctx *ctx, const mik_csr *A, const T *x, T *y, bool fuse_dot, T *seg_out, const int *done);
+int mik_spmv_launch(mik_ctx *ctx, const mik_csr *A, const T *x, T *y, bool fuse_dot, T *seg_out, const int *done, int stream_op = -1);
 template <typename T>
 int mik_spmv_launch_range(mik_ctx *ctx, const mik_csr *A, const T *x, T *y, bool fuse_dot, T *seg_out, const int *done, int rb_begin,
-                          int rb_count);
+                          int rb_count, int stream_op = -1);
 template <typename T>
-int mik_spmv_launch_outside(mik_ctx *ctx, const mik_csr *A, const T *x, T *y, bool fuse_dot, T *seg_out, const int *done, int skip_begin, int skip_end);
+int mik_spmv_launch_outside(mik_ctx *ctx, const mik_csr *A, const T *x, T *y, bool fuse_dot, T *seg_out, const int *done, int skip_begin, int skip_end,
+                            int stream_op = -1);
 bool mik_spmv_can_split(const mik_csr *A);
 bool mik_spmv_is_light(const mik_csr *A);
 bool mik_spmv_has_epilogue(const mik_csr *A);
diff --git a/iterativesolvers.jl_amd/csrc/mik_iter.h b/iterativesolvers.jl_amd/csrc/mik_iter.h
--- a/iterativesolvers.jl_amd/csrc/mik_iter.h
+++ b/iterativesolvers.jl_amd/csrc/mik_iter.h
@@ -42,6 +42,8 @@
     bool dev_done = false;
     bool head_ahead = false;
     bool fuse_x = false;
+    mik_cg_plan plan;
+    bool plan_forced = false;
     int profile = 0;
     std::vector<hipEvent_t> ev;
     std::vector<int> ev_kind;
@@ -49,6 +51,8 @@
     double kern_ms[3] = {0, 0, 0};
     int64_t kern_launches[3] = {0, 0, 0};
 };
+
+void cg_make_plan(mik_cg *it);
 
 #ifdef __HIPCC__
 constexpr int MIK_FIN_WGS = MIK_FIN_THREADS / 64;
diff --git a/iterativesolvers.jl_amd/csrc/mik_kernels.h b/iterativesolvers.jl_amd/csrc/mik_kernels.h
--- a/iterativesolvers.jl_amd/csrc/mik_kernels.h
+++ b/iterativesolvers.jl_amd/csrc/mik_kernels.h
@@ -212,6 +212,12 @@
     __builtin_nontemporal_store(o, reinterpret_cast<NV *>(p));
 }
 
+constexpr int64_t MIK_KEEP_ALL = INT64_MAX;
+__device__ __forceinline__ int keep_bits(int nt, int64_t i, int64_t ka, int ba, int64_t kb, int bb, int64_t kc = MIK_KEEP_ALL, int bc = 0, int64_t kd = MIK_KEEP_ALL, int bd = 0)
+{
+    return __builtin_amdgcn_readfirstlane(nt | (i >= ka ? ba : 0) | (i >= kb ? bb : 0) | (i >= kc ? bc : 0) | (i >= kd ? bd : 0));
+}
+
 template <typename T> constexpr int SEG_REGS = MIK_RED_L * VT<T>::W;
 
 template <typename T, bool VEC>
@@ -326,10 +332,12 @@
 
 template <typename T> struct OpXpby {
     static constexpr bool REDUCE = false;
-    const T *__restrict__ x; T *__restrict__ y; Coef<T> beta; int nt = 0;
+    const T *__restrict__ x; T *__restrict__ y; Coef<T> beta; int nt0 = 0;
+    int64_t keep_x = MIK_KEEP_ALL, keep_y = MIK_KEEP_ALL;
     __device__ __forceinline__ void apply(int64_t i, T &) const { T t = beta.get() * y[i]; y[i] = x[i] + t; }
     __device__ __forceinline__ void apply_vec(int64_t i, T &) const
     {
+        const int nt = keep_bits(nt0, i, keep_x, 1, keep_y, 6);
         const T b = beta.get();
         auto xv = (nt & 1) ? vload_nt(x + i) : vload(x + i);
         auto yv = (nt & 2) ? vload_nt<T>(y + i) : vload<T>(y + i);
@@ -487,7 +495,8 @@
 template <typename T> struct OpXpbyX {
     static constexpr bool REDUCE = false;
     const T *__restrict__ r; T *__restrict__ u; T *__restrict__ x; Coef<T> beta, alpha;
-    const int *__restrict__ done; const int *__restrict__ pending; int nt = 0;
+    const int *__restrict__ done; const int *__restrict__ pending; int nt0 = 0;
+    int64_t keep_r = MIK_KEEP_ALL, keep_u = MIK_KEEP_ALL, keep_x = MIK_KEEP_ALL;
     __device__ __forceinline__ void apply(int64_t i, T &) const
     {
         const int dn = *done, pd = *pending;
@@ -500,6 +509,7 @@
     {
         const int dn = *done, pd = *pending;
         if (dn && !pd) return;
+        const int nt = keep_bits(nt0, i, keep_r, 1, keep_u, 6, keep_x, 8);
         auto uv = (nt & 2) ? vload_nt<T>(u + i) : vload<T>(u + i);
         if (pd) {
             const T a = alpha.get();
@@ -530,7 +540,8 @@
 };
 template <typename T, typename C = Coef<T>> struct OpCgUpdateR {
     static constexpr bool REDUCE = true;
-    T *__restrict__ r; const T *__restrict__ c; C alpha; int nt = 0;
+    T *__restrict__ r; const T *__restrict__ c; C alpha; int nt0 = 0;
+    int64_t keep_r = MIK_KEEP_ALL, keep_c = MIK_KEEP_ALL;
     __device__ __forceinline__ void apply(int64_t i, T &acc) const
     {
         T s = alpha.get() * c[i]; T rn = r[i] - s; r[i] = rn;
@@ -539,6 +550,7 @@
     __device__ __forceinline__ void apply_vec(int64_t i, T &acc) const
     {
         const T a = alpha.get();
+        const int nt = keep_bits(nt0, i, keep_r, 24, keep_c, 2);
         auto rv = (nt & 8) ? vload_nt<T>(r + i) : vload<T>(r + i);
         auto cv = (nt & 2) ? vload_nt(c + i) : vload(c + i);
 #pragma unroll
@@ -551,7 +563,8 @@
 
 template <typename T> struct OpPcgUpdateR {
     static constexpr bool REDUCE = true;
-    T *__restrict__ r; T *__restrict__ c; const T *__restrict__ d; Coef<T> alpha; int nt = 0;
+    T *__restrict__ r; T *__restrict__ c; const T *__restrict__ d; Coef<T> alpha; int nt0 = 0;
+    int64_t keep_r = MIK_KEEP_ALL, keep_c = MIK_KEEP_ALL;
     __device__ __forceinline__ void apply(int64_t i, T &a1, T &a2) const
     {
         T s = alpha.get() * c[i]; T rn = r[i] - s; r[i] = rn;
@@ -562,6 +575,7 @@
     __device__ __forceinline__ void apply_vec(int64_t i, T &a1, T &a2) const
     {
         const T a = alpha.get();
+        const int nt = keep_bits(nt0, i, keep_r, 24, keep_c, 96);
         auto rv = (nt & 8) ? vload_nt<T>(r + i) : vload<T>(r + i);
         auto cv = (nt & 64) ? vload_nt<T>(c + i) : vload<T>(c + i);
         auto dv = vload_nt(d + i);
@@ -793,7 +807,8 @@
 template <typename T> struct OpCgUpdate {
     static constexpr bool REDUCE = true;
     T *__restrict__ x; T *__restrict__ r; const T *__restrict__ u; const T *__restrict__ c; Coef<T> alpha;
-    int nt = 0;
+    int nt0 = 0;
+    int64_t keep_x = MIK_KEEP_ALL, keep_c = MIK_KEEP_ALL, keep_u = MIK_KEEP_ALL, keep_r = MIK_KEEP_ALL;
     __device__ __forceinline__ void apply(int64_t i, T &acc) const
     {
         const T a = alpha.get();
@@ -804,6 +819,7 @@
     __device__ __forceinline__ void apply_vec(int64_t i, T &acc) const
     {
         const T a = alpha.get();
+        const int nt = keep_bits(nt0, i, keep_x, 1, keep_c, 2, keep_u, 4, keep_r, 24);
         auto xv = (nt & 1) ? vload_nt<T>(x + i) : vload<T>(x + i);
         auto uv = (nt & 4) ? vload_nt(u + i) : vload(u + i);
         auto rv = (nt & 8) ? vload_nt<T>(r + i) : vload<T>(r + i);
diff --git a/iterativesolvers.jl_amd/csrc/mik_krylov.hip b/iterativesolvers.jl_amd/csrc/mik_krylov.hip
--- a/iterativesolvers.jl_amd/csrc/mik_krylov.hip
+++ b/iterativesolvers.jl_amd/csrc/mik_krylov.hip
@@ -601,40 +601,84 @@
     }
 };
 
-static inline int cg_stream_hints(const mik_ctx *ctx, bool fused_x = false, const mik_csr *A = nullptr)
-{
-    (void)ctx;
-    return fused_x ? (mik_spmv_is_light(A) ? 248 : 121) : 57;
-}
-
-
-static inline int cg_sweep_u_hints(const mik_cg *it) { return it->fuse_x ? cg_stream_hints(it->ctx, true, it->A) & 15 : cg_stream_hints(it->ctx) & 7; }
-
-template <typename T> static int cg_sweep_u(mik_cg *it, const T *src, int64_t lo, int64_t len, bool vec, int hints)
+mik_cg_plan mik_cg_residency_plan(int64_t n, size_t es, int64_t op_bytes, bool op_streamed, int64_t cache_bytes, double budget, int step)
+{
+    mik_cg_plan p;
+    if (cache_bytes <= 0 || step != MIK_CG_STEP_FUSED_X || !op_streamed) {
+        p.ranged = 0;
+        p.mask = step == MIK_CG_STEP_CLASSIC ? 57 : (op_streamed ? 121 : 248);
+        p.keep_u = p.keep_r = p.keep_c = p.keep_x = n;
+        return p;
+    }
+    p.ranged = 1;
+    const int64_t vec = n * (int64_t)es, seg = (int64_t)MIK_BLOCK * (16 / (int64_t)es) * MIK_RED_L;
+    int64_t room = (int64_t)(std::max(0.0, budget) * (double)cache_bytes);
+    if (op_bytes + 4 * vec <= room) {
+        p.keep_u = p.keep_r = p.keep_c = p.keep_x = n;
+        p.spmv_nt = 0;
+        return p;
+    }
+    int64_t *keep[4] = {&p.keep_u, &p.keep_r, &p.keep_c, &p.keep_x};
+    for (int v = 0; v < 4 && room > 0; ++v) {
+        if (vec <= room) { *keep[v] = n; room -= vec; continue; }
+        *keep[v] = room / (int64_t)es / seg * seg;
+        room = 0;
+    }
+    return p;
+}
+
+void cg_make_plan(mik_cg *it)
+{
+    if (it->plan_forced) return;
+    int64_t op_bytes = 0;
+    if (it->A) (void)mik_csr_stored_bytes(it->A, &op_bytes);
+    const int step = it->fuse_x ? (it->diag ? MIK_CG_STEP_PCG : MIK_CG_STEP_FUSED_X) : MIK_CG_STEP_CLASSIC;
+    it->plan = mik_cg_residency_plan(it->n, mik_dtype_size(it->dtype), op_bytes, !mik_spmv_is_light(it->A), it->ctx->mall_bytes, MIK_CG_CACHE_BUDGET, step);
+}
+static inline int cg_spmv_stream(const mik_cg *it) { return it->plan.ranged ? it->plan.spmv_nt : -1; }
+
+
+static inline int64_t keep_from(int64_t keep, int64_t lo) { return std::max<int64_t>(0, keep - lo); }
+
+template <typename T> static int cg_sweep_u(mik_cg *it, const T *src, int64_t lo, int64_t len, bool vec, const mik_cg_plan &pl)
 {
     CgDev<T> *d = (CgDev<T> *)it->dev;
     T *x = (T *)it->x, *u = (T *)it->u;
+    const bool src_c = (const void *)src == (const void *)it->c;
+    const int hints = pl.ranged ? 0 : (it->fuse_x ? (src_c ? (pl.mask & 8) | 1 : pl.mask & 15) : (src_c ? pl.mask & 1 : pl.mask & 7));
+    const int64_t ks = pl.ranged ? keep_from(src_c ? pl.keep_c : pl.keep_r, lo) : MIK_KEEP_ALL, ku = pl.ranged ? keep_from(pl.keep_u, lo) : MIK_KEEP_ALL;
     if (it->fuse_x) {
-        OpXpbyX<T> op{src + lo, u + lo, x + lo, coef_ptr<T>(&d->beta), coef_ptr<T>(&d->alpha), &d->done, &d->x_pending, hints};
+        OpXpbyX<T> op{src + lo, u + lo, x + lo, coef_ptr<T>(&d->beta), coef_ptr<T>(&d->alpha), &d->done, &d->x_pending, hints,
+                      ks, ku, pl.ranged ? keep_from(pl.keep_x, lo) : MIK_KEEP_ALL};
         return launch_map<T>(it->ctx, len, op, vec, (T *)nullptr, (const int *)nullptr);
     }
-    OpXpby<T> op{src + lo, u + lo, coef_ptr<T>(&d->beta), hints};
+    OpXpby<T> op{src + lo, u + lo, coef_ptr<T>(&d->beta), hints, ks, ku};
     return launch_map<T>(it->ctx, len, op, vec, (T *)nullptr, &d->done);
 }
 
-template <typename T, typename C> static int cg_update_xr(mik_cg *it, C alpha, bool vec)
+template <typename T, typename C> static int cg_update_xr(mik_cg *it, C alpha, bool vec, const mik_cg_plan &pl)
 {
     CgDev<T> *d = (CgDev<T> *)it->dev;
     T *x = (T *)it->x, *u = (T *)it->u, *r = (T *)it->r, *c = (T *)it->c;
+    const int hints = pl.ranged ? 0 : pl.mask >> 3;
+    const int64_t kr = pl.ranged ? pl.keep_r : MIK_KEEP_ALL, kc = pl.ranged ? pl.keep_c : MIK_KEEP_ALL;
     if (it->fuse_x) {
-        OpCgUpdateR<T, C> up{r, c, alpha, cg_stream_hints(it->ctx, true, it->A) >> 3};
+        OpCgUpdateR<T, C> up{r, c, alpha, hints, kr, kc};
         return launch_map<T>(it->ctx, it->n, up, vec, (T *)it->seg_vec, &d->done);
     }
     if constexpr (std::is_same<C, Coef<T>>::value) {
-        OpCgUpdate<T> up{x, r, u, c, alpha, cg_stream_hints(it->ctx) >> 3};
+        OpCgUpdate<T> up{x, r, u, c, alpha, hints, pl.ranged ? pl.keep_x : MIK_KEEP_ALL, kc, pl.ranged ? pl.keep_u : MIK_KEEP_ALL, kr};
         return launch_map<T>(it->ctx, it->n, up, vec, (T *)it->seg_vec, &d->done);
     }
     return mik_fail(it->ctx, MIK_ERR_INVALID, "cg: alpha formed inside the sweep needs the x update on the next sweep over u");
+}
+
+template <typename T> static int cg_pcg_tail(mik_cg *it, bool vec, const mik_cg_plan &pl)
+{
+    CgDev<T> *d = (CgDev<T> *)it->dev;
+    OpPcgUpdateR<T> up{(T *)it->r, (T *)it->c, (const T *)it->diag, coef_ptr<T>(&d->alpha), pl.ranged ? 0 : 120,
+                       pl.ranged ? pl.keep_r : MIK_KEEP_ALL, pl.ranged ? pl.keep_c : MIK_KEEP_ALL};
+    return launch_map2<T>(it->ctx, it->n, up, vec, (T *)it->seg_vec, (T *)it->seg_vec2, &d->done);
 }
 
 template <typename T> __global__ void k_cg_clear_pending(CgDev<T> *d) { d->x_pending = 0; }
@@ -675,7 +719,7 @@
     const int pcg = (it->diag || it->pl_fn) ? 1 : 0;
     if (it->pcg_fused) {
     } else if (it->diag) {
-        OpJacobiDot<T> pj{r, (const T *)it->diag, c, cg_stream_hints(ctx) != 0};
+        OpJacobiDot<T> pj{r, (const T *)it->diag, c, 1};
         MIK_TRY((launch_map<T>(ctx, n, pj, vec, (T *)it->seg_vec, done)));
     } else if (it->pl_fn) {
         if (it->pl_fn(it->pl_user, c, r) != 0) return mik_fail(ctx, MIK_ERR_CALLBACK, "cg: the preconditioner callback failed");
@@ -688,12 +732,11 @@
     }
     {
         CgProfileScope ps(it, 1);
-        const int pcg_hints = it->fuse_x ? (cg_stream_hints(ctx, true, it->A) & 8) | 1 : cg_stream_hints(ctx) & 1;
-        MIK_TRY(cg_sweep_u<T>(it, pcg ? c : r, 0, n, vec, pcg ? pcg_hints : cg_sweep_u_hints(it)));
+        MIK_TRY(cg_sweep_u<T>(it, pcg ? c : r, 0, n, vec, it->plan));
     }
     if (it->A) {
         CgProfileScope ps(it, 0);
-        MIK_TRY(mik_spmv_launch<T>(ctx, it->A, u, c, true, (T *)it->seg_spmv, done));
+        MIK_TRY(mik_spmv_launch<T>(ctx, it->A, u, c, true, (T *)it->seg_spmv, done, cg_spmv_stream(it)));
     } else {
         if (it->op_mul(it->op_user, u, c) != 0) return mik_fail(ctx, MIK_ERR_CALLBACK, "cg: the operator callback failed");
         OpDot<T> duc{u, c};
@@ -709,15 +752,13 @@
 {
     mik_ctx *ctx = it->ctx;
     CgDev<T> *d = (CgDev<T> *)it->dev;
-    const int *done = &d->done;
     const int64_t n = it->n, nseg = mik_nseg<T>(n);
     T *x = (T *)it->x, *u = (T *)it->u, *r = (T *)it->r, *c = (T *)it->c;
     const bool vec = mik_aligned16(x) && mik_aligned16(u) && mik_aligned16(r) && mik_aligned16(c) && (!it->diag || mik_aligned16(it->diag));
     if (it->pcg_fused) {
         {
             CgProfileScope ps(it, 2);
-            OpPcgUpdateR<T> up{r, c, (const T *)it->diag, coef_ptr<T>(&d->alpha), 120};
-            MIK_TRY((launch_map2<T>(ctx, n, up, vec, (T *)it->seg_vec, (T *)it->seg_vec2, done)));
+            MIK_TRY(cg_pcg_tail<T>(it, vec, it->plan));
         }
         it->seq += 1;
         hipLaunchKernelGGL((k_cg_fin_res2<T>), dim3(MIK_FIN_WGS), dim3(64), 0, ctx->stream, (const T *)it->seg_vec, (const T *)it->seg_vec2, nseg, d, (T *)it->hist,
@@ -727,7 +768,7 @@
     }
     {
         CgProfileScope ps(it, 2);
-        MIK_TRY(cg_update_xr<T>(it, coef_ptr<T>(&d->alpha), vec));
+        MIK_TRY(cg_update_xr<T>(it, coef_ptr<T>(&d->alpha), vec, it->plan));
     }
     it->seq += 1;
     hipLaunchKernelGGL((k_cg_fin_res<T>), dim3(MIK_FIN_WGS), dim3(64), 0, ctx->stream, (const T *)it->seg_vec, nseg, d, (T *)it->hist,
@@ -799,6 +840,7 @@
     it->maxiter = maxiter;
     it->fuse_x = A != nullptr && !pl_fn && (ctx->tuning[MIK_KNOB_CG_STEP] & 1) == 0;
     it->pcg_fused = it->fuse_x && jacobi_diag != nullptr && (ctx->tuning[MIK_KNOB_CG_STEP] & 2) == 0;
+    cg_make_plan(it);
     const size_t es = mik_dtype_size(dtype);
     const int64_t nseg = dtype == MIK_F64 ? mik_nseg<double>(n) : mik_nseg<float>(n);
     const int64_t nb = mik_spmv_nwg(n);
@@ -979,6 +1021,57 @@
 {
     if (!it || !fused) return MIK_ERR_INVALID;
     *fused = it->fuse_x ? 1 : 0;
+    return MIK_OK;
+}
+
+extern "C" int mik_dev_cg_plan(int64_t n, int elem_size, int64_t operator_bytes, int operator_streamed, int64_t cache_bytes, double budget, int step,
+                               int64_t *keep, int *mask, int *spmv_nt)
+{
+    if (n < 0 || (elem_size != 4 && elem_size != 8) || operator_bytes < 0 || step < MIK_CG_STEP_FUSED_X || step > MIK_CG_STEP_PCG) return MIK_ERR_INVALID;
+    const mik_cg_plan p = mik_cg_residency_plan(n, (size_t)elem_size, operator_bytes, operator_streamed != 0, cache_bytes, budget, step);
+    if (keep) { keep[0] = p.keep_u; keep[1] = p.keep_r; keep[2] = p.keep_c; keep[3] = p.keep_x; }
+    if (mask) *mask = p.ranged ? -1 : p.mask;
+    if (spmv_nt) *spmv_nt = p.spmv_nt;
+    return MIK_OK;
+}
+
+static int cg_force_plan(mik_cg *it, int64_t keep_u, int64_t keep_r, int64_t keep_c, int64_t keep_x)
+{
+    if (keep_u < 0 || keep_r < 0 || keep_c < 0 || keep_x < 0) {
+        it->plan_forced = false;
+        cg_make_plan(it);
+        return MIK_OK;
+    }
+    const int64_t n = it->n;
+    mik_cg_plan p;
+    p.ranged = 1;
+    p.keep_u = std::min(keep_u, n); p.keep_r = std::min(keep_r, n); p.keep_c = std::min(keep_c, n); p.keep_x = std::min(keep_x, n);
+    p.spmv_nt = p.keep_c >= n ? 0 : 1;
+    it->plan = p;
+    it->plan_forced = true;
+    return MIK_OK;
+}
+
+extern "C" int mik_dev_cg_set_plan(mik_cg *it, int64_t keep_u, int64_t keep_r, int64_t keep_c, int64_t keep_x)
+{
+    if (!it) return MIK_ERR_INVALID;
+    return cg_force_plan(it, keep_u, keep_r, keep_c, keep_x);
+}
+
+extern "C" int mik_dev_cgd_set_plan(mik_cgd *it, int64_t keep_u, int64_t keep_r, int64_t keep_c, int64_t keep_x)
+{
+    if (!it) return MIK_ERR_INVALID;
+    return cg_force_plan(&it->base, keep_u, keep_r, keep_c, keep_x);
+}
+
+extern "C" int mik_dev_cg_get_plan(const mik_cg *it, int64_t *keep, int *mask, int *spmv_nt, int64_t *cache_bytes)
+{
+    if (!it) return MIK_ERR_INVALID;
+    const mik_cg_plan &p = it->plan;
+    if (keep) { keep[0] = p.keep_u; keep[1] = p.keep_r; keep[2] = p.keep_c; keep[3] = p.keep_x; }
+    if (mask) *mask = p.ranged ? -1 : p.mask;
+    if (spmv_nt) *spmv_nt = p.spmv_nt;
+    if (cache_bytes) *cache_bytes = it->ctx->mall_bytes;
     return MIK_OK;
 }
 
@@ -1687,6 +1780,7 @@
     it->rank = rank; it->nranks = nranks; it->n_send = n_send; it->send_idx = send_idx; it->send_buf = send_buf;
     it->u_ext = u_ext; it->n_ext = A_loc->n_cols; it->dot_all = dot_all; it->rr_all = rr_all;
     it->abstol = abstol; it->reltol = reltol; it->initially_zero = initially_zero;
+    cg_make_plan(&bs);
     const size_t es = mik_dtype_size(A_loc->dtype);
     const int64_t nseg = A_loc->dtype == MIK_F64 ? mik_nseg<double>(n) : mik_nseg<float>(n);
     const int64_t nb = mik_spmv_nwg(n);
@@ -1772,7 +1866,7 @@
         MIK_LAUNCH_CHECK(ctx);
         return MIK_OK;
     case MIK_CGD_STEP_A:
-        MIK_TRY(cg_sweep_u<T>(&bs, r, 0, n, vec, cg_sweep_u_hints(&bs)));
+        MIK_TRY(cg_sweep_u<T>(&bs, r, 0, n, vec, bs.plan));
         return gather_launch<T>(ctx, it->n_send, it->send_idx, u, (T *)it->send_buf, done);
     case CGD_STEP_A_EARLY:
     case CGD_STEP_A_BULK: {
@@ -1790,7 +1884,7 @@
             if (at < n) { lo[nr] = at; hi[nr] = n; ++nr; }
         }
         for (int q = 0; q < nr; ++q)
-            MIK_TRY(cg_sweep_u<T>(&bs, r, lo[q], hi[q] - lo[q], vec && (lo[q] % VT<T>::W == 0), cg_sweep_u_hints(&bs)));
+            MIK_TRY(cg_sweep_u<T>(&bs, r, lo[q], hi[q] - lo[q], vec && (lo[q] % VT<T>::W == 0), bs.plan));
         if (phase == CGD_STEP_A_EARLY) return gather_launch<T>(ctx, it->n_send, it->send_idx, u, (T *)it->send_buf, done);
         return MIK_OK;
     }
@@ -1810,8 +1904,8 @@
         const bool rest = phase == MIK_CGD_STEP_B_REST || phase == CGD_STEP_B_REST_NOFIN;
         {
             CgProfileScope ps(&bs, 0);
-            if (rest) MIK_TRY(mik_spmv_launch_outside<T>(ctx, bs.A, u, c, true, (T *)bs.seg_spmv, done, (int)it->int_begin, (int)it->int_end));
-            else MIK_TRY(mik_spmv_launch<T>(ctx, bs.A, u, c, true, (T *)bs.seg_spmv, done));
+            if (rest) MIK_TRY(mik_spmv_launch_outside<T>(ctx, bs.A, u, c, true, (T *)bs.seg_spmv, done, (int)it->int_begin, (int)it->int_end, cg_spmv_stream(&bs)));
+            else MIK_TRY(mik_spmv_launch<T>(ctx, bs.A, u, c, true, (T *)bs.seg_spmv, done, cg_spmv_stream(&bs)));
         }
         if (phase == CGD_STEP_B_NOFIN || phase == CGD_STEP_B_REST_NOFIN) return MIK_OK;
         hipLaunchKernelGGL((k_cgd_fin_slot<T>), dim3(MIK_FIN_WGS), dim3(64), 0, ctx->stream, (const T *)bs.seg_spmv, nb, dot_slot, done, (FinScratch<T> *)bs.fin);
@@ -1820,10 +1914,10 @@
     }
     case MIK_CGD_STEP_B_INTERIOR:
         if (it->int_end <= it->int_begin) return mik_fail(ctx, MIK_ERR_INVALID, "mik_cgd_phase: no interior range set (mik_cgd_set_interior)");
-        { CgProfileScope ps(&bs, 0); return mik_spmv_launch_range<T>(ctx, bs.A, u, c, true, (T *)bs.seg_spmv, done, (int)it->int_begin, (int)(it->int_end - it->int_begin)); }
+        { CgProfileScope ps(&bs, 0); return mik_spmv_launch_range<T>(ctx, bs.A, u, c, true, (T *)bs.seg_spmv, done, (int)it->int_begin, (int)(it->int_end - it->int_begin), cg_spmv_stream(&bs)); }
     case MIK_CGD_STEP_C: {
         if (bs.fuse_x && (ctx->tuning[MIK_KNOB_CG_STEP] & 8) == 0) {
-            MIK_TRY(cg_update_xr<T>(&bs, CoefAlphaRanks<T>{(const T *)it->dot_all, it->nranks, &d->res}, vec));
+            MIK_TRY(cg_update_xr<T>(&bs, CoefAlphaRanks<T>{(const T *)it->dot_all, it->nranks, &d->res}, vec, bs.plan));
             hipLaunchKernelGGL((k_cgd_fin_slot_alpha<T>), dim3(MIK_FIN_WGS), dim3(64), 0, ctx->stream, (const T *)bs.seg_vec, nseg, rr_slot, done,
                                (FinScratch<T> *)bs.fin, (const T *)it->dot_all, it->nranks, d);
             MIK_LAUNCH_CHECK(ctx);
@@ -1831,7 +1925,7 @@
         }
         hipLaunchKernelGGL((k_cgd_alpha<T>), dim3(1), dim3(1), 0, ctx->stream, (const T *)it->dot_all, it->nranks, d);
         MIK_LAUNCH_CHECK(ctx);
-        MIK_TRY(cg_update_xr<T>(&bs, coef_ptr<T>(&d->alpha), vec));
+        MIK_TRY(cg_update_xr<T>(&bs, coef_ptr<T>(&d->alpha), vec, bs.plan));
         hipLaunchKernelGGL((k_cgd_fin_slot<T>), dim3(MIK_FIN_WGS), dim3(64), 0, ctx->stream, (const T *)bs.seg_vec, nseg, rr_slot, done, (FinScratch<T> *)bs.fin);
         MIK_LAUNCH_CHECK(ctx);
         return MIK_OK;
@@ -1869,7 +1963,7 @@
                            (long long)bs.maxiter, bs.mirror, bs.seq, it->norm_fix_index);
         MIK_LAUNCH_CHECK(ctx);
         return MIK_OK;
-    case CGD_STEP_C_NOFIN: return cg_update_xr<T>(&bs, coef_ptr<T>(&d->alpha), vec);
+    case CGD_STEP_C_NOFIN: return cg_update_xr<T>(&bs, coef_ptr<T>(&d->alpha), vec, bs.plan);
     case CGD_CLEAR_PENDING:
         hipLaunchKernelGGL((k_cg_clear_pending<T>), dim3(1), dim3(1), 0, ctx->stream, d);
         MIK_LAUNCH_CHECK(ctx);
```
